# forestagostinelli/DeepCubeA

Hardware: AMD Instinct MI355X
Metric: A* nodes expanded/sec on cube3, batch 20k (higher is better)
Workload: dtype u8 states / f64 cost keys / f32 heuristic

## Files before the change

deepcubea_amd/csrc/dca_engine.hip:

```cpp
#include <string.h>

#include <new>
#include <vector>

#include "dca_common.h"
#include "dca_tile.h"

namespace dca {

constexpr int NBIN = 4096;
constexpr int kBinsPerThread = NBIN / 1024;
constexpr int kLgNbin = 12;
constexpr int kSub = 2048;
constexpr int kScanBlocks = 256;
constexpr int kCollectBlocks = 512;
constexpr int kRankBlocks = 256;
constexpr uint32_t kTinyBin = 512;
constexpr int kSortCap = 8192;
constexpr int RT = 512;
constexpr int kRegEnt = 16;
constexpr uint32_t kLdsEnt = RT * kRegEnt;
constexpr int kStash = 2560;
constexpr int kSegs = NBIN + 1 + kSub;
constexpr uint32_t kGiantBin = 8192;
constexpr int kMaxLevels = 9;
constexpr unsigned long long kBarrierTimeout = 200000000ull;
constexpr unsigned long long kBarrierTimeoutFirst = 25000000ull;
constexpr uint32_t GBAR_BROKEN = 0x80000000u;
constexpr uint32_t NIL = 0xFFFFFFFFu;
constexpr uint32_t ID_MASK = 0x7FFFFFFFu, ID_SOLVED = 0x80000000u;
constexpr uint64_t EMPTY = ~0ull;
constexpr uint64_t DEAD = ~0ull;
constexpr uint32_t GINF = 0xFFFFFFFFu;
constexpr int kMaxMoves = 4096;

struct Slot {
    uint64_t entry;
    uint32_t g;
    uint32_t head;
};

struct alignas(128) Cnt {
    uint32_t v;
    uint32_t pad[31];
};
struct alignas(128) GRange {
    uint64_t kmin, kmax;
    uint32_t imin, imax;
    uint32_t pad[26];
};
struct alignas(128) Rng {
    uint64_t kmin, kmax;
    uint64_t pad[14];
};
struct IterState {
    uint32_t pool_n;
    uint32_t npop, m, base;
    uint32_t best_id;
    int32_t has_best;
    float best_cost;
};
struct Ctl {
    int32_t done, failed, stop_after, pad0;
    int64_t iters, gen, expanded;
    IterState S[2];
    uint32_t cur_f;
    uint32_t hbin;
    uint32_t front_above;
    uint32_t cur_b;
    uint64_t T;
    uint32_t refill, compact, r_bstar, spill_bin, r_move;
    uint64_t r_kmin;
    uint32_t r_shift;
    uint32_t want, bstar, shift, n_big, n_ord;
    uint32_t giant;
    uint32_t tseg;
    uint32_t pre_b, cn_star;
    uint64_t sel_kmin;
    uint32_t goal_id;
    uint32_t dbg_nord, dbg_maxbin, dbg_giant, dbg_giant_seen, dbg_maxsub;
    Cnt open_n[4];
    Cnt closed_n, back_dead, front_dead, ret_n, ticket_a;
    Cnt gbar;
    GRange grange;
    Rng rng[4];
    alignas(128) unsigned long long goal_best;
    alignas(128) uint32_t first_solved;
};

__device__ __forceinline__ uint64_t key_of_cost(double c) {
    uint64_t b = (uint64_t)__double_as_longlong(c);
    return (b & 0x8000000000000000ull) ? ~b : (b | 0x8000000000000000ull);
}
__device__ __forceinline__ double cost_of_key(uint64_t k) {
    uint64_t b = (k & 0x8000000000000000ull) ? (k & 0x7FFFFFFFFFFFFFFFull) : ~k;
    return __longlong_as_double((long long)b);
}
__device__ __forceinline__ uint32_t select_shift(uint64_t kmin, uint64_t kmax) {
    uint64_t range = kmax - kmin;
    int bits = range ? 64 - __clzll((long long)range) : 0;
    return bits > kLgNbin ? (uint32_t)(bits - kLgNbin) : 0u;
}
__device__ __forceinline__ uint32_t bin_of(uint64_t k, uint64_t kmin, uint32_t shift) {
    if (k <= kmin) return 0u;
    const uint64_t f = (k - kmin) >> shift;
    return f < (uint64_t)NBIN ? (uint32_t)f : (uint32_t)(NBIN - 1);
}
__device__ __forceinline__ bool pair_less(uint64_t ka, uint32_t ia, uint64_t kb, uint32_t ib) {
    return ka < kb || (ka == kb && (ia & ID_MASK) < (ib & ID_MASK));
}

enum {
    P_REFILL_HIST = 0, P_REFILL_SCAN, P_REFILL_MOVE, P_SEL_HIST, P_SEL_SCAN, P_SEL_COLLECT, P_RANK, P_EXPAND,
    P_PROBE,
    P_DECIDE, P_PACK, P_COMMIT, P_RANK_SMALL, P_RANK_BIG, P_RB_LOAD, P_RB_COUNT, P_RB_SCATTER, P_RB_ORDER, P_COUNT
};
constexpr int kProfSlots = 1024;
__device__ int g_back_squeeze_mark;
__device__ int g_first_barrier_gives_up;
__device__ __forceinline__ uint32_t rank_shares(uint32_t cn) {
    return cn <= (uint32_t)(512 * 16) ? (cn + 1023u) / 1024u : 1u;
}

struct Eng {
    int env, dim, D, A, B, sem, oh_dtype, depth;
    double w;
    float wf;
    uint32_t max_nodes, M, tab_cap, tab_mask;
    uint32_t front_cap;
    uint8_t* state;
    int32_t* g;
    uint32_t* parent;
    uint8_t* move;
    uint8_t* solved;
    Slot* tab;
    uint32_t* closed_slots;
    uint64_t* open_key[4];
    uint32_t* open_id[4];
    uint32_t f_keep, f_max;
    uint32_t *hist, *pre, *fill;
    uint32_t* rhist;
    uint32_t* subhist;
    int coop;
    uint32_t* coop_off;
    uint64_t* part;
    uint64_t* tmp_key;
    uint32_t* tmp_id;
    uint16_t* tmp_f;
    uint32_t* tmp_idx;
    uint64_t* ord_key;
    uint32_t* ord_id;
    uint32_t* big_list;
    uint64_t* pop_key;
    uint32_t *pop_id, *pop_g;
    uint32_t *child_slot, *child_next, *child_v0;
    uint8_t *child_flags, *child_multi;
    float* child_h;
    uint8_t* nnet_in;
    uint8_t* onehot;
    uint8_t* root_nnet;
    int32_t* d_moves;
    Ctl* ctl;
    unsigned long long* prof;
    uint32_t* kept_pos;
    uint32_t* pk_n;
    uint32_t* pk_src;
    uint8_t* pk_nnet;
    uint8_t* pk_onehot;
    const float* pk_h;
    uint32_t pk_stride, inst;
    int pk_dtype;
};

__device__ __forceinline__ const IterState& st_cur(const Ctl* c) { return c->S[c->iters & 1]; }
__device__ __forceinline__ const IterState& st_next(const Ctl* c) { return c->S[(c->iters + 1) & 1]; }

__device__ __forceinline__ void fresh_binning(const Ctl* c, uint32_t buf, uint64_t& kmin, uint32_t& shift) {
    kmin = c->rng[buf].kmin;
    uint64_t kmax = c->rng[buf].kmax;
    const uint64_t T = c->T;
    if (T != ~0ull && T > kmax) kmax = T;
    shift = kmax > kmin ? select_shift(kmin, kmax) : 0u;
}

struct Stamp {
    unsigned long long* p;
    unsigned long long t0;
    __device__ __forceinline__ Stamp(const Eng& E, int kid) : p(nullptr), t0(0) {
        if (E.prof != nullptr && threadIdx.x == 0) {
            p = E.prof + ((size_t)kid * kProfSlots + (blockIdx.x & (kProfSlots - 1))) * 2;
            t0 = wall_clock64();
        }
    }
    __device__ __forceinline__ ~Stamp() {
        if (p) {
            atomicMin(p, t0);
            atomicMax(p + 1, (unsigned long long)wall_clock64());
        }
    }
};

__device__ __forceinline__ void prof_begin(const Eng& E, int kid) {
    if (E.prof != nullptr && threadIdx.x == 0)
        atomicMin(E.prof + ((size_t)kid * kProfSlots + (blockIdx.x & (kProfSlots - 1))) * 2, (unsigned long long)wall_clock64());
}
__device__ __forceinline__ void prof_end(const Eng& E, int kid) {
    if (E.prof != nullptr && threadIdx.x == 0)
        atomicMax(E.prof + ((size_t)kid * kProfSlots + (blockIdx.x & (kProfSlots - 1))) * 2 + 1, (unsigned long long)wall_clock64());
}

__device__ __forceinline__ void open_append(const Eng& E, Ctl* c, uint32_t buf, bool pred, uint64_t key, uint32_t id) {
    unsigned long long mask = __ballot(pred);
    if (mask == 0) return;
    int lane = threadIdx.x & 63;
    int leader = __ffsll((long long)mask) - 1;
    uint32_t cnt = (uint32_t)__popcll(mask);
    uint32_t basep = 0;
    uint64_t kmn = pred ? key : ~0ull, kmx = pred ? key : 0ull;
    for (int o = 32; o > 0; o >>= 1) {
        uint64_t a = __shfl_xor(kmn, o), b = __shfl_xor(kmx, o);
        kmn = a < kmn ? a : kmn;
        kmx = b > kmx ? b : kmx;
    }
    if (lane == leader) {
        basep = atomicAdd(&c->open_n[buf].v, cnt);
        atomicMin((unsigned long long*)&c->rng[buf].kmin, (unsigned long long)kmn);
        atomicMax((unsigned long long*)&c->rng[buf].kmax, (unsigned long long)kmx);
    }
    basep = __shfl(basep, leader);
    if (pred) {
        uint32_t pos = basep + (uint32_t)__popcll(mask & ((1ull << lane) - 1ull));
        if (pos < (buf < 2 ? E.front_cap : E.max_nodes)) {
            E.open_key[buf][pos] = key;
            E.open_id[buf][pos] = id;
        } else {
            c->failed = 1;
        }
    }
}

struct Pos2 {
    uint32_t a, b;
};
template <int NT>
__device__ __forceinline__ Pos2 block_reserve2(uint32_t cntA, uint32_t cntB, uint32_t* ctrA, uint32_t* ctrB,
                                               uint32_t* sh) {
    constexpr int NW = NT / 64;
    const int lane = threadIdx.x & 63, wv = threadIdx.x >> 6;
    uint32_t ia = cntA, ib = cntB;
    for (int o = 1; o < 64; o <<= 1) {
        uint32_t va = __shfl_up(ia, o), vb = __shfl_up(ib, o);
        if (lane >= o) {
            ia += va;
            ib += vb;
        }
    }
    if (lane == 63) {
        sh[wv] = ia;
        sh[NW + wv] = ib;
    }
    __syncthreads();
    if (threadIdx.x == 0) {
        uint32_t aa = 0, ab = 0;
        for (int w = 0; w < NW; w++) {
            uint32_t ta = sh[w], tb = sh[NW + w];
            sh[w] = aa;
            sh[NW + w] = ab;
            aa += ta;
            ab += tb;
        }
        sh[2 * NW] = aa ? atomicAdd(ctrA, aa) : 0u;
        sh[2 * NW + 1] = ab ? atomicAdd(ctrB, ab) : 0u;
    }
    __syncthreads();
    Pos2 p{sh[2 * NW] + sh[wv] + ia - cntA, sh[2 * NW + 1] + sh[NW + wv] + ib - cntB};
    __syncthreads();
    return p;
}

struct Pos3 {
    uint32_t a, b, c;
};
template <int NT>
__device__ __forceinline__ Pos3 block_reserve3(uint32_t cntA, uint32_t cntB, uint32_t cntC, uint32_t* ctrA,
                                               uint32_t* ctrB, uint32_t* ctrC, uint32_t* sh ) {
    constexpr int NW = NT / 64;
    const int lane = threadIdx.x & 63, wv = threadIdx.x >> 6;
    uint32_t ia = cntA, ib = cntB, ic = cntC;
    for (int o = 1; o < 64; o <<= 1) {
        uint32_t va = __shfl_up(ia, o), vb = __shfl_up(ib, o), vc = __shfl_up(ic, o);
        if (lane >= o) {
            ia += va;
            ib += vb;
            ic += vc;
        }
    }
    if (lane == 63) {
        sh[wv] = ia;
        sh[NW + wv] = ib;
        sh[2 * NW + wv] = ic;
    }
    __syncthreads();
    if (threadIdx.x == 0) {
        uint32_t aa = 0, ab = 0, ac = 0;
        for (int w = 0; w < NW; w++) {
            uint32_t ta = sh[w], tb = sh[NW + w], tc = sh[2 * NW + w];
            sh[w] = aa;
            sh[NW + w] = ab;
            sh[2 * NW + w] = ac;
            aa += ta;
            ab += tb;
            ac += tc;
        }
        sh[3 * NW] = aa ? atomicAdd(ctrA, aa) : 0u;
        sh[3 * NW + 1] = ab ? atomicAdd(ctrB, ab) : 0u;
        sh[3 * NW + 2] = ac ? atomicAdd(ctrC, ac) : 0u;
    }
    __syncthreads();
    Pos3 p{sh[3 * NW] + sh[wv] + ia - cntA, sh[3 * NW + 1] + sh[NW + wv] + ib - cntB,
           sh[3 * NW + 2] + sh[2 * NW + wv] + ic - cntC};
    __syncthreads();
    return p;
}

template <int NT, int K>
__device__ __forceinline__ void block_reserveK(const uint32_t (&cnt)[K], uint32_t* const (&ctr)[K], uint32_t (&pos)[K],
                                               uint32_t* sh ) {
    constexpr int NW = NT / 64;
    const int lane = threadIdx.x & 63, wv = threadIdx.x >> 6;
    uint32_t inc[K];
#pragma unroll
    for (int k = 0; k < K; k++) inc[k] = cnt[k];
    for (int o = 1; o < 64; o <<= 1) {
#pragma unroll
        for (int k = 0; k < K; k++) {
            uint32_t v = __shfl_up(inc[k], o);
            if (lane >= o) inc[k] += v;
        }
    }
    if (lane == 63) {
#pragma unroll
        for (int k = 0; k < K; k++) sh[k * NW + wv] = inc[k];
    }
    __syncthreads();
    if (threadIdx.x < K) {
        const int k = threadIdx.x;
        uint32_t acc = 0;
        for (int w = 0; w < NW; w++) {
            uint32_t tv = sh[k * NW + w];
            sh[k * NW + w] = acc;
            acc += tv;
        }
        sh[K * NW + k] = acc ? atomicAdd(ctr[k], acc) : 0u;
    }
    __syncthreads();
#pragma unroll
    for (int k = 0; k < K; k++) pos[k] = sh[K * NW + k] + sh[k * NW + wv] + inc[k] - cnt[k];
    __syncthreads();
}

__device__ __forceinline__ void fold_range(Ctl* c, uint32_t buf, uint64_t kmn, uint64_t kmx) {
    for (int o = 32; o > 0; o >>= 1) {
        uint64_t a = __shfl_xor(kmn, o), b = __shfl_xor(kmx, o);
        kmn = a < kmn ? a : kmn;
        kmx = b > kmx ? b : kmx;
    }
    if ((threadIdx.x & 63) == 0) {
        if (kmn < c->rng[buf].kmin) atomicMin((unsigned long long*)&c->rng[buf].kmin, (unsigned long long)kmn);
        if (kmx > c->rng[buf].kmax) atomicMax((unsigned long long*)&c->rng[buf].kmax, (unsigned long long)kmx);
    }
}

__device__ __forceinline__ bool clear_by_list(const Ctl* c, uint32_t cap, int force) {
    return !force && (uint64_t)c->closed_n.v * 8ull < (uint64_t)cap;
}
__global__ void k_init_table(Slot* tab, uint32_t cap, const Ctl* c, int force) {
    if (clear_by_list(c, cap, force)) return;
    uint32_t i = blockIdx.x * blockDim.x + threadIdx.x;
    uint32_t stride = gridDim.x * blockDim.x;
    for (; i < cap; i += stride) {
        tab[i].entry = EMPTY;
        tab[i].g = GINF;
        tab[i].head = 0;
    }
}
__global__ void k_clear_table_list(Slot* tab, uint32_t cap, const uint32_t* __restrict__ slots, const Ctl* c, int force) {
    if (!clear_by_list(c, cap, force)) return;
    const uint32_t n = c->closed_n.v;
    for (uint32_t i = blockIdx.x * blockDim.x + threadIdx.x; i < n; i += gridDim.x * blockDim.x) {
        const uint32_t sl = slots[i];
        if (sl < cap) {
            tab[sl].entry = EMPTY;
            tab[sl].g = GINF;
            tab[sl].head = 0;
        }
    }
}

__global__ void k_reset(Eng E) {
    if (threadIdx.x != 0 || blockIdx.x != 0) return;
    Ctl* c = E.ctl;
    memset(c, 0, sizeof(Ctl));
    const uint8_t* s = E.state;
    uint64_t h = hash_init(E.D);
    bool ok = true;
    for (int k = 0; k < E.D; k += 8) {
        uint64_t w = 0;
        for (int j = 0; j < 8 && k + j < E.D; j++) {
            uint32_t b = s[k + j];
            uint32_t goal = goal_byte(E.env, E.D, k + j);
            ok &= (b == goal);
            w |= (uint64_t)b << (8 * j);
            E.root_nnet[k + j] = (uint8_t)(E.env == DCA_ENV_CUBE3 ? (b * 57u) >> 9 : b);
        }
        h = hash_word(h, w);
    }
    h = hash_final(h);
    E.g[0] = 0;
    E.parent[0] = NIL;
    E.move[0] = 0xFF;
    E.solved[0] = ok ? 1 : 0;
    for (int p = 0; p < 2; p++) c->S[p].pool_n = 1;
    c->cur_f = 0;
    c->goal_best = ~0ull;
    c->first_solved = NIL;
    for (int b = 0; b < 4; b++) {
        c->rng[b].kmin = ~0ull;
        c->rng[b].kmax = 0;
    }
    c->cur_b = 2;
    c->T = ~0ull;
    if (E.sem == DCA_SEM_CPP) {
        uint32_t slot = (uint32_t)h & E.tab_mask;
        E.tab[slot].entry = ((h >> 32) << 32) | 0u;
        E.tab[slot].g = 0;
        E.closed_slots[0] = slot;
        c->closed_n.v = 1;
        c->gen = 1;
        uint64_t key = key_of_cost(0.0);
        E.open_key[0][0] = key;
        E.open_id[0][0] = ok ? ID_SOLVED : 0u;
        c->open_n[0].v = 1;
        c->rng[0].kmin = c->rng[0].kmax = key;
    }
}

__global__ void k_root_commit(Eng E, const float* h_root) {
    if (threadIdx.x != 0 || blockIdx.x != 0) return;
    Ctl* c = E.ctl;
    if (E.sem != DCA_SEM_PY || c->open_n[c->cur_f].v != 0) return;
    double hv = fmax((double)h_root[0], 0.0);
    double cost = __dadd_rn(__dmul_rn(E.w, 0.0), __dmul_rn(hv, E.solved[0] ? 0.0 : 1.0));
    uint64_t key = key_of_cost(cost);
    uint32_t b = c->cur_f;
    E.open_key[b][0] = key;
    E.open_id[b][0] = E.solved[0] ? ID_SOLVED : 0u;
    c->open_n[b].v = 1;
    c->rng[b].kmin = c->rng[b].kmax = key;
}

constexpr int kRefillPeriod = 16;
__device__ __forceinline__ uint32_t front_keep(const Eng& E) {
    const uint32_t floor_ = (uint32_t)(kRefillPeriod + 1) * (uint32_t)E.B;
    return E.f_keep > floor_ ? E.f_keep : floor_;
}
__device__ __forceinline__ bool need_refill(const Eng& E, const Ctl* c) {
    return c->open_n[c->cur_b].v != c->back_dead.v &&
           c->open_n[c->cur_f].v - c->front_dead.v - c->front_above < (uint32_t)(kRefillPeriod + 1) * (uint32_t)E.B;
}

__global__ __launch_bounds__(256) void k_refill_hist(const Eng* __restrict__ engs) {
    const Eng& E = engs[blockIdx.y];
    Ctl* c = E.ctl;
    if (c->done || !need_refill(E, c)) return;
    Stamp stamp(E, P_REFILL_HIST);
    __shared__ uint32_t lh[NBIN];
    for (int i = threadIdx.x; i < NBIN; i += 256) lh[i] = 0;
    __syncthreads();
    const uint32_t b = c->cur_b, n = c->open_n[b].v;
    const uint64_t kmin = c->rng[b].kmin;
    const uint32_t shift = select_shift(kmin, c->rng[b].kmax);
    const uint64_t* __restrict__ keys = E.open_key[b];
    for (uint32_t i = blockIdx.x * 256 + threadIdx.x; i < n; i += gridDim.x * 256) {
        uint64_t k = keys[i];
        if (k == DEAD) continue;
        uint64_t f = (k - kmin) >> shift;
        atomicAdd(&lh[f < NBIN ? (uint32_t)f : NBIN - 1], 1u);
    }
    __syncthreads();
    for (int i = threadIdx.x; i < NBIN; i += 256)
        if (lh[i]) atomicAdd(&E.rhist[i], lh[i]);
}

__device__ __forceinline__ void scan_vals(const uint32_t (&v)[kBinsPerThread], uint32_t* pre, uint32_t* wsum) {
    const int t = threadIdx.x, lane = t & 63, wv = t >> 6;
    uint32_t s = 0;
#pragma unroll
    for (int k = 0; k < kBinsPerThread; k++) s += v[k];
    uint32_t incl = s;
    for (int o = 1; o < 64; o <<= 1) {
        uint32_t u = __shfl_up(incl, o);
        if (lane >= o) incl += u;
    }
    if (lane == 63) wsum[wv] = incl;
    __syncthreads();
    if (t < 16) {
        uint32_t u = wsum[t], acc = u;
        for (int o = 1; o < 16; o <<= 1) {
            uint32_t x = __shfl_up(acc, o, 16);
            if (t >= o) acc += x;
        }
        wsum[t] = acc - u;
    }
    __syncthreads();
    uint32_t run = incl - s + wsum[wv];
#pragma unroll
    for (int k = 0; k < kBinsPerThread; k++) {
        pre[kBinsPerThread * t + k] = run;
        run += v[k];
    }
    if (t == 1023) pre[NBIN] = run;
    __syncthreads();
}

__device__ __forceinline__ void scan_bins(uint32_t* __restrict__ hist, bool zero, uint32_t* pre, uint32_t* wsum) {
    const int t = threadIdx.x, lane = t & 63, wv = t >> 6;
    uint32_t v[kBinsPerThread], s = 0;
#pragma unroll
    for (int k = 0; k < kBinsPerThread; k++) {
        v[k] = hist[kBinsPerThread * t + k];
        if (zero) hist[kBinsPerThread * t + k] = 0;
        s += v[k];
    }
    uint32_t incl = s;
    for (int o = 1; o < 64; o <<= 1) {
        uint32_t u = __shfl_up(incl, o);
        if (lane >= o) incl += u;
    }
    if (lane == 63) wsum[wv] = incl;
    __syncthreads();
    if (t < 16) {
        uint32_t u = wsum[t], acc = u;
        for (int o = 1; o < 16; o <<= 1) {
            uint32_t x = __shfl_up(acc, o, 16);
            if (t >= o) acc += x;
        }
        wsum[t] = acc - u;
    }
    __syncthreads();
    uint32_t run = incl - s + wsum[wv];
#pragma unroll
    for (int k = 0; k < kBinsPerThread; k++) {
        pre[kBinsPerThread * t + k] = run;
        run += v[k];
    }
    if (t == 1023) pre[NBIN] = run;
    __syncthreads();
}

__global__ __launch_bounds__(1024) void k_refill_scan(const Eng* __restrict__ engs) {
    const Eng& E = engs[blockIdx.y];
    Ctl* c = E.ctl;
    if (c->done) return;
    Stamp stamp(E, P_REFILL_SCAN);
    for (int k = 0; k < kBinsPerThread; k++) E.hist[kBinsPerThread * threadIdx.x + k] = 0;
    if (threadIdx.x == 0) c->open_n[c->cur_f ^ 1].v = 0;
    if (!need_refill(E, c)) {
        if (threadIdx.x == 0) {
            const uint32_t b = c->cur_b, phys = c->open_n[b].v, dead = c->back_dead.v;
            const uint32_t mark = g_back_squeeze_mark > 0 ? (uint32_t)(((uint64_t)E.max_nodes * (uint32_t)g_back_squeeze_mark) >> 10)
                                                          : (E.max_nodes / 8) * 7;
            const bool squeeze = dead != 0 && phys > mark;
            c->refill = squeeze ? 1u : 0u;
            c->compact = squeeze ? 1u : 0u;
            c->r_move = 0;
            if (squeeze) {
                c->open_n[b ^ 1].v = 0;
                c->rng[b ^ 1].kmin = c->rng[b].kmin;
                c->rng[b ^ 1].kmax = c->rng[b].kmax;
            }
        }
        return;
    }
    __shared__ uint32_t pre[NBIN + 1];
    __shared__ uint32_t wsum[16];
    scan_bins(E.rhist, true, pre, wsum);
    const int t = threadIdx.x;
    const uint32_t b = c->cur_b, n = c->open_n[b].v - c->back_dead.v;
    const uint32_t target = n < front_keep(E) ? n : front_keep(E);
    for (int k = 0; k < kBinsPerThread; k++) {
        int bin = kBinsPerThread * t + k;
        if (pre[bin] < target && target <= pre[bin + 1]) c->r_bstar = (uint32_t)bin;
    }
    __syncthreads();
    if (t == 0) {
        const uint64_t kmin = c->rng[b].kmin;
        const uint32_t shift = select_shift(kmin, c->rng[b].kmax);
        c->refill = 1;
        c->r_move = 1;
        c->r_kmin = kmin;
        c->r_shift = shift;
        uint64_t top = (c->r_bstar >= NBIN - 1) ? ~0ull : kmin + (((uint64_t)c->r_bstar + 1) << shift) - 1;
        if (top < kmin) top = ~0ull;
        c->T = top;
        if (top != ~0ull) c->rng[b].kmin = top + 1;
        const uint32_t phys = c->open_n[b].v, dead = c->back_dead.v;
        c->compact = ((dead > phys / 2 && phys > 4096) || (dead != 0 && phys > (E.max_nodes / 8) * 7)) ? 1u : 0u;
        if (c->compact) {
            c->open_n[b ^ 1].v = 0;
            c->rng[b ^ 1].kmin = c->rng[b].kmin;
            c->rng[b ^ 1].kmax = c->rng[b].kmax;
        }
    }
}

__global__ __launch_bounds__(256) void k_refill_move(const Eng* __restrict__ engs) {
    const Eng& E = engs[blockIdx.y];
    Ctl* c = E.ctl;
    if (c->done || !c->refill) return;
    Stamp stamp(E, P_REFILL_MOVE);
    __shared__ uint32_t sh[2 * 4 + 2];
    const uint32_t sb = c->cur_b, fb = c->cur_f, db = sb ^ 1;
    const bool compact = c->compact != 0;
    const uint32_t n = c->open_n[sb].v;
    const uint64_t kmin = c->r_kmin;
    const uint32_t shift = c->r_shift, bstar = c->r_bstar;
    const bool move = c->r_move != 0;
    uint64_t* __restrict__ keys = E.open_key[sb];
    const uint32_t* __restrict__ ids = E.open_id[sb];
    constexpr uint32_t ITEMS = 8, TILE = 256 * ITEMS;
    uint64_t fmn = ~0ull, fmx = 0;
    uint32_t moved = 0;
    const uint32_t ntiles = (n + TILE - 1) / TILE;
    for (uint32_t tile = blockIdx.x; tile < ntiles; tile += gridDim.x) {
        uint64_t k[ITEMS];
        uint32_t tof = 0, stay = 0, cf = 0, cs = 0;
#pragma unroll
        for (uint32_t i = 0; i < ITEMS; i++) {
            uint32_t idx = tile * TILE + i * 256 + threadIdx.x;
            k[i] = keys[idx < n ? idx : n - 1];
            if (idx >= n) k[i] = DEAD;
            uint64_t f = (k[i] - kmin) >> shift;
            bool alive = k[i] != DEAD;
            bool front = alive && move && (f < NBIN ? (uint32_t)f : NBIN - 1) <= bstar;
            tof |= (front ? 1u : 0u) << i;
            stay |= ((alive && !front && compact) ? 1u : 0u) << i;
            cf += front ? 1u : 0u;
            cs += (alive && !front && compact) ? 1u : 0u;
        }
        Pos2 p = block_reserve2<256>(cf, cs, &c->open_n[fb].v, &c->open_n[db].v, sh);
#pragma unroll
        for (uint32_t i = 0; i < ITEMS; i++) {
            uint32_t idx = tile * TILE + i * 256 + threadIdx.x;
            if ((tof >> i) & 1u) {
                if (p.a < E.front_cap) {
                    E.open_key[fb][p.a] = k[i];
                    E.open_id[fb][p.a] = ids[idx];
                }
                if (!compact) keys[idx] = DEAD;
                p.a++;
                moved++;
                fmn = k[i] < fmn ? k[i] : fmn;
                fmx = k[i] > fmx ? k[i] : fmx;
            } else if ((stay >> i) & 1u) {
                E.open_key[db][p.b] = k[i];
                E.open_id[db][p.b] = ids[idx];
                p.b++;
            }
        }
    }
    fold_range(c, fb, fmn, fmx);
    if (!compact) {
        for (int o = 32; o > 0; o >>= 1) moved += __shfl_xor(moved, o);
        if ((threadIdx.x & 63) == 0 && moved) atomicAdd(&c->back_dead.v, moved);
    }
}

__global__ __launch_bounds__(256) void k_front_rebase(const Eng* __restrict__ engs) {
    const Eng& E = engs[blockIdx.y];
    Ctl* c = E.ctl;
    if (c->done) return;
    Stamp stamp(E, P_SEL_HIST);
    __shared__ uint32_t lh[NBIN];
    __shared__ uint32_t sh[2 * 4 + 2];
    for (int i = threadIdx.x; i < NBIN; i += 256) lh[i] = 0;
    __syncthreads();
    const uint32_t b = c->cur_f, nb = b ^ 1, n = c->open_n[b].v;
    const uint32_t bb = (c->refill && c->compact) ? c->cur_b ^ 1u : c->cur_b;
    const uint64_t T = c->T;
    uint64_t kmin;
    uint32_t shift;
    fresh_binning(c, b, kmin, shift);
    const uint64_t* __restrict__ keys = E.open_key[b];
    const uint32_t* __restrict__ ids = E.open_id[b];
    constexpr uint32_t ITEMS = 8, TILE = 256 * ITEMS;
    uint64_t fmn = ~0ull, fmx = 0, bmn = ~0ull, bmx = 0;
    const uint32_t ntiles = (n + TILE - 1) / TILE;
    for (uint32_t tile = blockIdx.x; tile < ntiles; tile += gridDim.x) {
        uint64_t k[ITEMS];
        uint32_t id[ITEMS];
        uint32_t cl = 0, ce = 0;
#pragma unroll
        for (uint32_t i = 0; i < ITEMS; i++) {
            const uint32_t idx = tile * TILE + i * 256 + threadIdx.x, ic = idx < n ? idx : n - 1;
            k[i] = keys[ic];
            id[i] = ids[ic];
            if (idx >= n) k[i] = DEAD;
            cl += (k[i] != DEAD && k[i] <= T) ? 1u : 0u;
            ce += (k[i] != DEAD && k[i] > T) ? 1u : 0u;
        }
        Pos2 p = block_reserve2<256>(cl, ce, &c->open_n[nb].v, &c->open_n[bb].v, sh);
#pragma unroll
        for (uint32_t i = 0; i < ITEMS; i++) {
            if (k[i] != DEAD && k[i] > T) {
                if (p.b < E.max_nodes) {
                    E.open_key[bb][p.b] = k[i];
                    E.open_id[bb][p.b] = id[i];
                } else {
                    c->failed = 1;
                }
                p.b++;
                bmn = k[i] < bmn ? k[i] : bmn;
                bmx = k[i] > bmx ? k[i] : bmx;
                continue;
            }
            const bool lv = k[i] != DEAD;
            if (lv) atomicAdd(&lh[bin_of(k[i], kmin, shift)], 1u);
            if (!lv) continue;
            if (p.a < E.front_cap) {
                E.open_key[nb][p.a] = k[i];
                E.open_id[nb][p.a] = id[i];
            } else {
                c->failed = 1;
            }
            p.a++;
            fmn = k[i] < fmn ? k[i] : fmn;
            fmx = k[i] > fmx ? k[i] : fmx;
        }
    }
    __syncthreads();
    for (int i = threadIdx.x; i < NBIN; i += 256)
        if (lh[i]) atomicAdd(&E.hist[i], lh[i]);
    if (T != ~0ull) fold_range(c, bb, bmn, bmx);
    {
        __shared__ uint64_t red[2][4];
        const int lane = threadIdx.x & 63, wv = threadIdx.x >> 6;
        for (int o = 32; o > 0; o >>= 1) {
            const uint64_t a = __shfl_xor(fmn, o), z = __shfl_xor(fmx, o);
            fmn = a < fmn ? a : fmn;
            fmx = z > fmx ? z : fmx;
        }
        if (lane == 0) {
            red[0][wv] = fmn;
            red[1][wv] = fmx;
        }
        __syncthreads();
        if (threadIdx.x == 0) {
            uint64_t mn = red[0][0], mx = red[1][0];
            for (int w = 1; w < 4; w++) {
                mn = red[0][w] < mn ? red[0][w] : mn;
                mx = red[1][w] > mx ? red[1][w] : mx;
            }
            E.part[blockIdx.x] = mn;
            E.part[kCollectBlocks + blockIdx.x] = mx;
        }
    }
}

__global__ __launch_bounds__(1024) void k_sel_scan(const Eng* __restrict__ engs, int rebased) {
    const Eng& E = engs[blockIdx.y];
    Ctl* c = E.ctl;
    __shared__ uint32_t pre[NBIN + 1];
    __shared__ uint32_t wsum[16];
    __shared__ uint32_t s_spill, s_bstar, s_maxbin, s_giant, s_nbig, s_sp, s_hbin;
    __shared__ uint64_t s_red[2][16];
    const int t = threadIdx.x;
    const uint32_t done = c->done;
    const uint32_t cur0 = c->cur_f, old_shift = c->shift, refill = c->refill, compact = c->compact;
    const uint64_t old_kmin = c->sel_kmin, T0 = c->T;
    const uint32_t on0 = c->open_n[0].v, on1 = c->open_n[1].v, dead0 = c->front_dead.v, above0 = c->front_above;
    const uint64_t r0min = c->rng[0].kmin, r0max = c->rng[0].kmax, r1min = c->rng[1].kmin, r1max = c->rng[1].kmax;
    const uint32_t giant_seen = c->dbg_giant_seen;
    uint32_t hv[kBinsPerThread];
#pragma unroll
    for (int k = 0; k < kBinsPerThread; k++) hv[k] = E.hist[kBinsPerThread * t + k];
    uint64_t mn = ~0ull, mx = 0;
    if (rebased && t < kCollectBlocks) {
        mn = E.part[t];
        mx = E.part[kCollectBlocks + t];
    }
    if (done) return;
    Stamp stamp(E, P_SEL_SCAN);
    uint32_t cb = cur0;
    uint64_t new_kmin = old_kmin;
    uint32_t new_shift = old_shift;
    if (rebased) {
        new_kmin = cur0 ? r1min : r0min;
        uint64_t kmax = cur0 ? r1max : r0max;
        if (T0 != ~0ull && T0 > kmax) kmax = T0;
        new_shift = kmax > new_kmin ? select_shift(new_kmin, kmax) : 0u;
        for (int o = 32; o > 0; o >>= 1) {
            const uint64_t a = __shfl_xor(mn, o), z = __shfl_xor(mx, o);
            mn = a < mn ? a : mn;
            mx = z > mx ? z : mx;
        }
        if ((t & 63) == 0) {
            s_red[0][t >> 6] = mn;
            s_red[1][t >> 6] = mx;
        }
        cb ^= 1;
    }
    if (t == 0) {
        s_maxbin = 0;
        s_giant = 0;
        s_nbig = 0;
        s_spill = NBIN;
        s_bstar = 0;
        s_hbin = NBIN;
    }
    scan_vals(hv, pre, wsum);
    const uint32_t n = rebased ? (cb ? on1 : on0) : (cb ? on1 : on0) - dead0 - above0;
    const uint32_t want = n < (uint32_t)E.B ? n : (uint32_t)E.B;
    const uint32_t hwant = (uint32_t)(kRefillPeriod + 2) * (uint32_t)E.B;
    for (int k = 0; k < kBinsPerThread; k++) {
        int bin = kBinsPerThread * t + k;
        if (pre[bin] < want && want <= pre[bin + 1]) s_bstar = (uint32_t)bin;
        if (rebased && n > E.f_max) {
            const uint32_t keepn = want + front_keep(E);
            if (pre[bin] < keepn && keepn <= pre[bin + 1]) s_spill = (uint32_t)bin;
        }
        if (rebased && pre[bin] < hwant && hwant <= pre[bin + 1]) s_hbin = (uint32_t)bin + 1u;
        E.pre[bin] = pre[bin];
        E.fill[bin] = 0;
    }
    for (int i = NBIN + t; i < kSegs; i += 1024) E.fill[i] = 0;
    if (t == 1023) E.pre[NBIN] = pre[NBIN];
    __syncthreads();
    const bool giant = E.coop && !*E.coop_off && want != 0 && pre[s_bstar + 1] - pre[s_bstar] > kGiantBin;
    if (giant)
        for (int i = t; i < kMaxLevels * kSub; i += 1024) E.subhist[i] = 0;
    for (int k = 0; k < kBinsPerThread; k++) {
        const uint32_t bin = kBinsPerThread * t + k;
        if (bin <= s_bstar && want != 0) {
            const uint32_t cn = pre[bin + 1] - pre[bin];
            if (cn > 256) atomicMax(&s_maxbin, cn);
            if (cn > (uint32_t)kSortCap) atomicAdd(&s_giant, 1u);
            if (cn > kTinyBin && !(giant && bin == s_bstar)) {
                uint32_t G = rank_shares(cn);
                G = G > 8u ? 8u : G;
                const uint32_t at = atomicAdd(&s_nbig, G);
                for (uint32_t g = 0; g < G; g++) E.big_list[at + g] = bin | (g << 16) | (G << 20);
            }
        }
    }
    __syncthreads();
    if (t == 0) {
        if (rebased) {
            uint64_t fmn = ~0ull, fmx = 0;
            for (int w = 0; w < 16; w++) {
                fmn = s_red[0][w] < fmn ? s_red[0][w] : fmn;
                fmx = s_red[1][w] > fmx ? s_red[1][w] : fmx;
            }
            c->cur_f = cb;
            c->rng[cb].kmin = fmn;
            c->rng[cb].kmax = fmx;
            c->hbin = s_hbin;
        }
        if (refill) {
            if (compact) {
                c->cur_b ^= 1;
                c->back_dead.v = 0;
                c->compact = 0;
            }
            c->refill = 0;
        }
        c->want = want;
        c->bstar = s_bstar;
        c->tseg = s_bstar;
        c->pre_b = pre[s_bstar];
        c->cn_star = pre[s_bstar + 1] - pre[s_bstar];
        c->giant = giant ? 1u : 0u;
        c->gbar.v = 0;
        c->grange.kmin = ~0ull;
        c->grange.kmax = 0;
        c->grange.imin = ~0u;
        c->grange.imax = 0;
        c->sel_kmin = new_kmin;
        c->shift = new_shift;
        uint32_t sp = s_spill;
        if (sp < NBIN - 1) {
            const uint64_t top = new_kmin + (((uint64_t)sp + 1) << new_shift) - 1;
            if (top >= new_kmin && top < T0) c->T = top;  else sp = NBIN;
        } else {
            sp = NBIN;
        }
        if (rebased) c->front_above = sp < NBIN ? pre[NBIN] - pre[sp + 1] : 0u;
        c->spill_bin = sp;
        s_sp = sp;
        c->goal_best = ~0ull;
        c->first_solved = NIL;
        if (want == 0) {
            c->failed = 1;
            c->done = 1;
        }
        c->n_big = s_nbig;
        c->n_ord = want ? pre[s_bstar + 1] : 0;
        c->ret_n.v = 0;
        c->dbg_maxsub = 0;
        c->front_dead.v = (rebased ? 0u : dead0) + want;
        c->dbg_nord = want ? pre[s_bstar + 1] : 0;
        c->dbg_maxbin = s_maxbin;
        c->dbg_giant = s_giant;
        c->dbg_giant_seen = giant_seen + s_giant;
    }
    __syncthreads();
    {
        const uint32_t bstar = s_bstar, sp = s_sp;
        for (int k = 0; k < kBinsPerThread; k++) {
            const uint32_t bin = kBinsPerThread * t + k;
            if (want == 0) break;
            if (bin < bstar || bin > sp)
                E.hist[bin] = 0;
            else if (bin == bstar)
                E.hist[bin] = pre[bin + 1] - want;
        }
    }
}

typedef unsigned __int128 u128;
__device__ __forceinline__ u128 comp_of(uint64_t key, uint32_t id) { return ((u128)key << 32) | (u128)(id & ID_MASK); }
__device__ __forceinline__ int clz128(u128 v) {
    uint64_t hi = (uint64_t)(v >> 64), lo = (uint64_t)v;
    return hi ? __clzll((long long)hi) : 64 + (lo ? __clzll((long long)lo) : 64);
}

constexpr int kStashG = 1536;
struct CollectLds {
    uint32_t pre[NBIN + 4];
    uint32_t lcnt[NBIN];
    union {
        struct {
            uint64_t st_key[kStash];
            uint32_t st_idx[kStash];
            uint16_t st_f[kStash];
            uint16_t nzf[kStash];
        } n;
        struct {
            uint32_t lcnt_ext[kSegs - NBIN + 3];
            uint32_t subpre[kSub + 4];
            uint64_t st_key[kStashG];
            uint32_t st_idx[kStashG];
            uint16_t st_f[kStashG];
            uint16_t nzf[kStashG];
        } g;
    } u;
    uint64_t red64[2][4];
    uint32_t red32[2][4];
    uint32_t wsum[4];
    uint32_t st_n, nz_n, ok, tsub, nb, bstar;
};
static_assert(sizeof(CollectLds) <= 80 * 1024, "two workgroups of k_sel_collect must fit one CU's LDS");
static_assert(offsetof(CollectLds, u) == offsetof(CollectLds, lcnt) + sizeof(uint32_t) * NBIN, "lcnt must run on into lcnt_ext");
static_assert(sizeof(uint64_t) * kStashG >= sizeof(uint32_t) * kSub, "sub-bin counters alias the giant stash");

struct SelParams {
    uint32_t b, n;
    uint64_t kmin;
    uint32_t shift;
    uint32_t want, bstar, pre_b, cn_star;
    bool giant;
};

enum { BAR_FAIL = 0, BAR_PASS = 1, BAR_BROKEN = 2 };
__device__ __forceinline__ int collect_grid_barrier(const Eng& E, Ctl* c, CollectLds& L, uint32_t target, bool first) {
    asm volatile("s_waitcnt vmcnt(0)" ::: "memory");
    __syncthreads();
    if (threadIdx.x == 0) {
        __builtin_amdgcn_fence(__ATOMIC_RELEASE, "agent");
        asm volatile("s_waitcnt vmcnt(0)" ::: "memory");
        uint32_t v = __hip_atomic_fetch_add(&c->gbar.v, 1u, __ATOMIC_RELAXED, __HIP_MEMORY_SCOPE_AGENT) + 1u;
        int res = BAR_PASS;
        const unsigned long long t0 = wall_clock64();
        const unsigned long long limit = first ? (g_first_barrier_gives_up ? 0ull : kBarrierTimeoutFirst) : kBarrierTimeout;
        for (;;) {
            if (v & GBAR_BROKEN) {
                res = first ? BAR_BROKEN : BAR_FAIL;
                break;
            }
            if (v >= target) break;
            __builtin_amdgcn_s_sleep(4);
            if (__hip_atomic_load(&c->failed, __ATOMIC_RELAXED, __HIP_MEMORY_SCOPE_AGENT) != 0) {
                res = BAR_FAIL;
                break;
            }
            if (wall_clock64() - t0 > limit) {
                if (!first) {
                    res = BAR_FAIL;
                    break;
                }
                uint32_t expect = v;
                if (__hip_atomic_compare_exchange_strong(&c->gbar.v, &expect, v | GBAR_BROKEN, __ATOMIC_RELAXED, __ATOMIC_RELAXED,
                                                         __HIP_MEMORY_SCOPE_AGENT)) {
                    res = BAR_BROKEN;
                    break;
                }
                v = expect;
                continue;
            }
            v = __hip_atomic_load(&c->gbar.v, __ATOMIC_RELAXED, __HIP_MEMORY_SCOPE_AGENT);
        }
        __builtin_amdgcn_fence(__ATOMIC_ACQUIRE, "agent");
        if (res == BAR_FAIL) {
            __hip_atomic_store(&c->failed, 1, __ATOMIC_RELAXED, __HIP_MEMORY_SCOPE_AGENT);
            __hip_atomic_store(&c->done, 1, __ATOMIC_RELAXED, __HIP_MEMORY_SCOPE_AGENT);
        } else if (res == BAR_BROKEN) {
            __hip_atomic_store(E.coop_off, 1u, __ATOMIC_RELAXED, __HIP_MEMORY_SCOPE_AGENT);
        }
        L.ok = (uint32_t)res;
    }
    __syncthreads();
    return (int)L.ok;
}

__device__ __noinline__ int collect_giant(const Eng& E, Ctl* c, CollectLds& L, const SelParams P) {
    const uint32_t t = threadIdx.x, lane = t & 63, wv = t >> 6;
    const uint32_t n = P.n;
    const uint64_t bkmin = P.kmin;
    const uint32_t shift = P.shift, bstar = P.bstar, want = P.want;
    const uint32_t pre_b = P.pre_b;
    uint64_t* __restrict__ keys = E.open_key[P.b];
    const uint32_t* __restrict__ ids = E.open_id[P.b];
    constexpr uint32_t ITEMS = 8, TILE = 256 * ITEMS;
    const uint32_t ntiles = (n + TILE - 1) / TILE;
    uint32_t phase = 0;
    {
        uint64_t kmn = ~0ull, kmx = 0;
        uint32_t imn = ~0u, imx = 0;
        for (uint32_t tile = blockIdx.x; tile < ntiles; tile += gridDim.x) {
            uint64_t k[ITEMS];
            uint32_t id[ITEMS];
#pragma unroll
            for (uint32_t i = 0; i < ITEMS; i++) {
                const uint32_t idx = tile * TILE + i * 256 + t, ic = idx < n ? idx : n - 1;
                k[i] = keys[ic];
                id[i] = ids[ic] & ID_MASK;
                if (idx >= n) k[i] = DEAD;
            }
#pragma unroll
            for (uint32_t i = 0; i < ITEMS; i++) {
                const bool in = k[i] != DEAD && bin_of(k[i], bkmin, shift) == bstar;
                kmn = in && k[i] < kmn ? k[i] : kmn;
                kmx = in && k[i] > kmx ? k[i] : kmx;
                imn = in && id[i] < imn ? id[i] : imn;
                imx = in && id[i] > imx ? id[i] : imx;
            }
        }
        for (int o = 32; o > 0; o >>= 1) {
            const uint64_t a = __shfl_xor(kmn, o), z = __shfl_xor(kmx, o);
            const uint32_t x = __shfl_xor(imn, o), y = __shfl_xor(imx, o);
            kmn = a < kmn ? a : kmn;
            kmx = z > kmx ? z : kmx;
            imn = x < imn ? x : imn;
            imx = y > imx ? y : imx;
        }
        if (lane == 0) {
            L.red64[0][wv] = kmn;
            L.red64[1][wv] = kmx;
            L.red32[0][wv] = imn;
            L.red32[1][wv] = imx;
        }
        __syncthreads();
        if (t == 0) {
            for (int w = 1; w < 4; w++) {
                kmn = L.red64[0][w] < kmn ? L.red64[0][w] : kmn;
                kmx = L.red64[1][w] > kmx ? L.red64[1][w] : kmx;
                imn = L.red32[0][w] < imn ? L.red32[0][w] : imn;
                imx = L.red32[1][w] > imx ? L.red32[1][w] : imx;
            }
            if (kmn <= kmx) {
                atomicMin((unsigned long long*)&c->grange.kmin, (unsigned long long)kmn);
                atomicMax((unsigned long long*)&c->grange.kmax, (unsigned long long)kmx);
                atomicMin(&c->grange.imin, imn);
                atomicMax(&c->grange.imax, imx);
            }
        }
    }
    if (const int r = collect_grid_barrier(E, c, L, ++phase * gridDim.x, true); r != BAR_PASS) return r;
    const uint64_t gkmin = __hip_atomic_load(&c->grange.kmin, __ATOMIC_RELAXED, __HIP_MEMORY_SCOPE_AGENT);
    const uint64_t gkmax = __hip_atomic_load(&c->grange.kmax, __ATOMIC_RELAXED, __HIP_MEMORY_SCOPE_AGENT);
    const uint32_t gimin = __hip_atomic_load(&c->grange.imin, __ATOMIC_RELAXED, __HIP_MEMORY_SCOPE_AGENT);
    const uint32_t gimax = __hip_atomic_load(&c->grange.imax, __ATOMIC_RELAXED, __HIP_MEMORY_SCOPE_AGENT);
    u128 V0 = ((u128)gkmin << 32) + (u128)gimin;
    u128 span = ((u128)(gkmax - gkmin) << 32) + (u128)(gimax - gimin);
    uint32_t need = want - pre_b, below = 0, shc = 0, tsub = 0;
    uint32_t* lh = reinterpret_cast<uint32_t*>(L.u.g.st_key);
    uint32_t* subpre = L.u.g.subpre;
    for (int lvl = 0;; lvl++) {
        const uint32_t bits = span ? (uint32_t)(128 - clz128(span)) : 0u;
        shc = bits > 11u ? bits - 11u : 0u;
        for (uint32_t i = t; i < (uint32_t)kSub; i += 256) lh[i] = 0;
        __syncthreads();
        for (uint32_t tile = blockIdx.x; tile < ntiles; tile += gridDim.x) {
            uint64_t k[ITEMS];
            uint32_t id[ITEMS];
#pragma unroll
            for (uint32_t i = 0; i < ITEMS; i++) {
                const uint32_t idx = tile * TILE + i * 256 + t, ic = idx < n ? idx : n - 1;
                k[i] = keys[ic];
                id[i] = ids[ic];
                if (idx >= n) k[i] = DEAD;
            }
#pragma unroll
            for (uint32_t i = 0; i < ITEMS; i++) {
                if (k[i] == DEAD || bin_of(k[i], bkmin, shift) != bstar) continue;
                const u128 v = comp_of(k[i], id[i]);
                if (v < V0 || v - V0 > span) continue;
                atomicAdd(&lh[(uint32_t)((v - V0) >> shc)], 1u);
            }
        }
        __syncthreads();
        uint32_t* gh = E.subhist + (size_t)lvl * kSub;
        for (uint32_t i = t; i < (uint32_t)kSub; i += 256)
            if (lh[i]) atomicAdd(&gh[i], lh[i]);
        if (collect_grid_barrier(E, c, L, ++phase * gridDim.x, false) != BAR_PASS) return BAR_FAIL;
        constexpr int PER = kSub / 256;
        uint32_t v[PER], sum = 0;
#pragma unroll
        for (int k = 0; k < PER; k++) {
            v[k] = __hip_atomic_load(&gh[PER * t + k], __ATOMIC_RELAXED, __HIP_MEMORY_SCOPE_AGENT);
            sum += v[k];
        }
        uint32_t incl = sum;
        for (int o = 1; o < 64; o <<= 1) {
            const uint32_t u = __shfl_up(incl, o);
            if (lane >= (uint32_t)o) incl += u;
        }
        if (lane == 63) L.wsum[wv] = incl;
        if (t == 0) L.tsub = ~0u;
        __syncthreads();
        uint32_t run = incl - sum;
        for (uint32_t w = 0; w < wv; w++) run += L.wsum[w];
#pragma unroll
        for (int k = 0; k < PER; k++) {
            subpre[PER * t + k] = run;
            if (run < need && need <= run + v[k]) L.tsub = PER * t + k;
            run += v[k];
        }
        if (t == 255) subpre[kSub] = run;
        __syncthreads();
        tsub = L.tsub;
        if (tsub == ~0u) {
            if (t == 0) c->failed = 1, c->done = 1;
            return BAR_FAIL;
        }
        const uint32_t cn = subpre[tsub + 1] - subpre[tsub];
        if (cn <= kGiantBin || shc == 0 || lvl + 1 >= kMaxLevels) break;
        below += subpre[tsub];
        need -= subpre[tsub];
        V0 += (u128)tsub << shc;
        span = ((u128)1 << shc) - 1;
        __syncthreads();
    }
    const uint32_t seg0 = bstar + 1u;
    if (blockIdx.x == 0) {
        if (t == 0) {
            L.nb = c->n_big;
            E.pre[bstar + 1] = pre_b + below;
            c->tseg = seg0 + tsub;
            c->n_ord = pre_b + below + subpre[tsub + 1];
            c->dbg_nord = pre_b + below + subpre[tsub + 1];
        }
        __syncthreads();
        for (uint32_t sg = t; sg <= tsub + 1u; sg += 256) {
            const uint32_t cn = sg == 0 ? below : subpre[sg] - subpre[sg - 1];
            if (sg > 0) E.pre[seg0 + sg] = pre_b + below + subpre[sg];
            if (cn > kTinyBin) {
                uint32_t G = rank_shares(cn);
                G = G > 8u ? 8u : G;
                const uint32_t at = atomicAdd(&L.nb, G);
                for (uint32_t g = 0; g < G; g++) E.big_list[at + g] = (bstar + sg) | (g << 16) | (G << 20);
            }
        }
        __syncthreads();
        if (t == 0) c->n_big = L.nb;
    }
    uint32_t* lcnt = L.lcnt;
    for (uint32_t i = t; i < (uint32_t)(kSegs + 3); i += 256) lcnt[i] = 0;
    if (t == 0) {
        L.st_n = 0;
        L.nz_n = 0;
    }
    __syncthreads();
    uint64_t* st_key = L.u.g.st_key;
    uint32_t* st_idx = L.u.g.st_idx;
    uint16_t *st_f = L.u.g.st_f, *nzf = L.u.g.nzf;
    auto seg_base = [&](uint32_t f) -> uint32_t {
        return f < bstar ? L.pre[f] : f == bstar ? pre_b : pre_b + below + subpre[f - seg0];
    };
    auto seg_end = [&](uint32_t f) -> uint32_t {
        return f < bstar ? L.pre[f + 1] : f == bstar ? pre_b + below : pre_b + below + subpre[f - seg0 + 1];
    };
    auto flush = [&]() {
        const uint32_t ns = L.st_n < (uint32_t)kStashG ? L.st_n : (uint32_t)kStashG;
        const uint32_t nz = L.nz_n;
        for (uint32_t i = t; i < nz; i += 256) {
            const uint32_t f = nzf[i];
            lcnt[f] = atomicAdd(&E.fill[f], lcnt[f]);
        }
        __syncthreads();
        for (uint32_t p = t; p < ns; p += 256) {
            const uint32_t f = st_f[p];
            const uint32_t id = ids[st_idx[p]];
            const uint32_t pos = seg_base(f) + atomicAdd(&lcnt[f], 1u);
            if (pos < seg_end(f)) {
                E.tmp_key[pos] = st_key[p];
                E.tmp_id[pos] = id;
                E.tmp_f[pos] = (uint16_t)f;
                E.tmp_idx[pos] = st_idx[p];
            } else {
                c->failed = 1;
            }
        }
        __syncthreads();
        for (uint32_t i = t; i < nz; i += 256) lcnt[nzf[i]] = 0;
        __syncthreads();
        if (t == 0) {
            L.st_n = 0;
            L.nz_n = 0;
        }
        __syncthreads();
    };
    constexpr uint32_t ITEMS_D = 4, TILE_D = 256 * ITEMS_D;
    const uint32_t ntiles_d = (n + TILE_D - 1) / TILE_D;
    for (uint32_t tile2 = blockIdx.x; tile2 < ntiles; tile2 += gridDim.x) {
        for (uint32_t half = 0; half < 2; half++) {
            const uint32_t tile = tile2 * 2 + half;
            if (tile < ntiles_d) {
                uint64_t k[ITEMS_D];
                uint32_t id[ITEMS_D];
#pragma unroll
                for (uint32_t i = 0; i < ITEMS_D; i++) {
                    const uint32_t idx = tile * TILE_D + i * 256 + t, ic = idx < n ? idx : n - 1;
                    k[i] = keys[ic];
                    id[i] = ids[ic];
                    if (idx >= n) k[i] = DEAD;
                }
#pragma unroll
                for (uint32_t i = 0; i < ITEMS_D; i++) {
                    if (k[i] == DEAD) continue;
                    uint32_t f = bin_of(k[i], bkmin, shift);
                    if (f > bstar) continue;
                    if (f == bstar) {
                        const u128 v = comp_of(k[i], id[i]);
                        if (v >= V0) {
                            if (v - V0 > span) continue;
                            const uint32_t sub = (uint32_t)((v - V0) >> shc);
                            if (sub > tsub) continue;
                            f = seg0 + sub;
                        }
                    }
                    const uint32_t idx = tile * TILE_D + i * 256 + t;
                    const uint32_t p = atomicAdd(&L.st_n, 1u);
                    keys[idx] = DEAD;
                    if (p < (uint32_t)kStashG) {
                        st_key[p] = k[i];
                        st_idx[p] = idx;
                        st_f[p] = (uint16_t)f;
                        if (atomicAdd(&lcnt[f], 1u) == 0u) nzf[atomicAdd(&L.nz_n, 1u)] = (uint16_t)f;
                    } else {
                        const uint32_t pos = seg_base(f) + atomicAdd(&E.fill[f], 1u);
                        if (pos < seg_end(f)) {
                            E.tmp_key[pos] = k[i];
                            E.tmp_id[pos] = id[i];
                            E.tmp_f[pos] = (uint16_t)f;
                            E.tmp_idx[pos] = idx;
                        } else {
                            c->failed = 1;
                        }
                    }
                }
            }
            __syncthreads();
            if (L.st_n + TILE_D > (uint32_t)kStashG) flush();
        }
    }
    __syncthreads();
    flush();
    return BAR_PASS;
}

template <bool FUSED>
__global__ __launch_bounds__(256) void k_sel_collect(const Eng* __restrict__ engs) {
    const Eng& E = engs[blockIdx.y];
    Ctl* c = E.ctl;
    if (c->done) return;
    Stamp stamp(E, P_SEL_COLLECT);
    extern __shared__ __attribute__((aligned(16))) uint8_t collect_lds[];
    CollectLds& L = *reinterpret_cast<CollectLds*>(collect_lds);
    const uint32_t t = threadIdx.x;
    SelParams P;
    {
        const uint32_t b = c->cur_f, on0 = c->open_n[0].v, on1 = c->open_n[1].v;
        P.b = b;
        P.n = b ? on1 : on0;
        P.kmin = c->sel_kmin;
        P.shift = c->shift;
        P.want = c->want;
    }
    if constexpr (FUSED) {
        constexpr int PER = NBIN / 256;
        const uint32_t lane = t & 63, wv = t >> 6;
        uint32_t v[PER], sum = 0;
        {
            const uint4* h4 = reinterpret_cast<const uint4*>(E.hist + PER * t);
#pragma unroll
            for (int q = 0; q < PER / 4; q++) {
                const uint4 x = h4[q];
                v[4 * q] = x.x;
                v[4 * q + 1] = x.y;
                v[4 * q + 2] = x.z;
                v[4 * q + 3] = x.w;
            }
#pragma unroll
            for (int k = 0; k < PER; k++) sum += v[k];
        }
        uint32_t incl = sum;
        for (int o = 1; o < 64; o <<= 1) {
            const uint32_t u = __shfl_up(incl, o);
            if (lane >= (uint32_t)o) incl += u;
        }
        if (lane == 63) L.wsum[wv] = incl;
        if (t == 0) L.bstar = 0;
        __syncthreads();
        uint32_t run = incl - sum;
        for (uint32_t w = 0; w < wv; w++) run += L.wsum[w];
        const uint32_t want = P.want;
#pragma unroll
        for (int k = 0; k < PER; k++) {
            L.pre[PER * t + k] = run;
            if (run < want && want <= run + v[k]) L.bstar = PER * t + k;
            run += v[k];
        }
        if (t == 255) L.pre[NBIN] = run;
        __syncthreads();
        if (want == 0) {
            if (blockIdx.x == 0 && t == 0) {
                c->failed = 1;
                c->done = 1;
            }
            return;
        }
        P.bstar = L.bstar;
        P.pre_b = L.pre[P.bstar];
        P.cn_star = L.pre[P.bstar + 1] - P.pre_b;
        P.giant = E.coop && !*E.coop_off && P.cn_star > kGiantBin;
        if (blockIdx.x == 0) {
            for (uint32_t i = t; i <= (uint32_t)NBIN; i += 256) E.pre[i] = L.pre[i];
            if (t == 0) {
                L.nb = 0;
                L.st_n = 0;
                L.nz_n = 0;
            }
            __syncthreads();
            for (uint32_t bin = t; bin <= P.bstar; bin += 256) {
                const uint32_t cn = L.pre[bin + 1] - L.pre[bin];
                if (cn > 256) atomicMax(&L.st_n, cn);
                if (cn > (uint32_t)kSortCap) atomicAdd(&L.nz_n, 1u);
                if (cn > kTinyBin && !(P.giant && bin == P.bstar)) {
                    uint32_t G = rank_shares(cn);
                    G = G > 8u ? 8u : G;
                    const uint32_t at = atomicAdd(&L.nb, G);
                    for (uint32_t g = 0; g < G; g++) E.big_list[at + g] = bin | (g << 16) | (G << 20);
                }
            }
            __syncthreads();
            if (t == 0) {
                c->bstar = P.bstar;
                c->tseg = P.bstar;
                c->giant = P.giant ? 1u : 0u;
                c->pre_b = P.pre_b;
                c->cn_star = P.cn_star;
                c->spill_bin = NBIN;
                c->n_big = L.nb;
                c->n_ord = L.pre[P.bstar + 1];
                c->front_dead.v += want;
                c->dbg_nord = L.pre[P.bstar + 1];
                c->dbg_maxbin = L.st_n;
                c->dbg_giant = L.nz_n;
                c->dbg_giant_seen += L.nz_n;
                c->dbg_maxsub = 0;
            }
            __syncthreads();
        }
    } else {
        P.bstar = c->bstar;
        P.giant = c->giant != 0;
        P.pre_b = c->pre_b;
        P.cn_star = c->cn_star;
        if (P.want == 0) return;
        for (uint32_t i = t; i <= P.bstar + 1u; i += 256) L.pre[i] = E.pre[i];
        __syncthreads();
    }
    if (P.giant) {
        if (collect_giant(E, c, L, P) != BAR_BROKEN) return;
        if (blockIdx.x == 0 && t == 0) {
            const uint32_t cn = P.cn_star;
            uint32_t G = rank_shares(cn);
            G = G > 8u ? 8u : G;
            const uint32_t at = c->n_big;
            if (cn > kTinyBin) {
                for (uint32_t g = 0; g < G; g++) E.big_list[at + g] = P.bstar | (g << 16) | (G << 20);
                c->n_big = at + G;
            }
            c->giant = 0;
        }
        P.giant = false;
        __syncthreads();
    }
    const uint32_t n = P.n;
    const uint64_t kmin = P.kmin;
    const uint32_t shift = P.shift, bstar = P.bstar;
    uint64_t* __restrict__ keys = E.open_key[P.b];
    const uint32_t* __restrict__ ids = E.open_id[P.b];
    constexpr uint32_t ITEMS = 8, TILE = 256 * ITEMS;
    const uint32_t ntiles = (n + TILE - 1) / TILE;
    uint64_t* st_key = L.u.n.st_key;
    uint32_t* st_idx = L.u.n.st_idx;
    uint16_t *st_f = L.u.n.st_f, *nzf = L.u.n.nzf;
    for (int i = t; i < NBIN; i += 256) L.lcnt[i] = 0;
    if (t == 0) {
        L.st_n = 0;
        L.nz_n = 0;
    }
    __syncthreads();
    auto flush = [&]() {
        const uint32_t ns = L.st_n < (uint32_t)kStash ? L.st_n : (uint32_t)kStash;
        const uint32_t nz = L.nz_n;
        for (uint32_t i = t; i < nz; i += 256) {
            const uint32_t f = nzf[i];
            L.lcnt[f] = atomicAdd(&E.fill[f], L.lcnt[f]);
        }
        __syncthreads();
        for (uint32_t p = t; p < ns; p += 256) {
            const uint32_t f = st_f[p];
            const uint32_t id = ids[st_idx[p]];
            const uint32_t pos = L.pre[f] + atomicAdd(&L.lcnt[f], 1u);
            if (pos < L.pre[f + 1]) {
                E.tmp_key[pos] = st_key[p];
                E.tmp_id[pos] = id;
                E.tmp_f[pos] = (uint16_t)f;
                E.tmp_idx[pos] = st_idx[p];
            } else {
                c->failed = 1;
            }
        }
        __syncthreads();
        for (uint32_t i = t; i < nz; i += 256) L.lcnt[nzf[i]] = 0;
        __syncthreads();
        if (t == 0) {
            L.st_n = 0;
            L.nz_n = 0;
        }
        __syncthreads();
    };
    for (uint32_t tile = blockIdx.x; tile < ntiles; tile += gridDim.x) {
        uint64_t k[ITEMS];
        uint32_t dest = 0;
#pragma unroll
        for (uint32_t i = 0; i < ITEMS; i++) {
            const uint32_t idx = tile * TILE + i * 256 + t, ic = idx < n ? idx : n - 1;
            k[i] = keys[ic];
            if (idx >= n) k[i] = DEAD;
        }
#pragma unroll
        for (uint32_t i = 0; i < ITEMS; i++) {
            const uint32_t f = bin_of(k[i], kmin, shift);
            const uint32_t d = (k[i] != DEAD && f <= bstar) ? 1u : 0u;
            dest |= d << (2 * i);
        }
        if (dest & 0x5555u & ~(dest >> 1)) {
#pragma unroll
            for (uint32_t i = 0; i < ITEMS; i++) {
                if (((dest >> (2 * i)) & 3u) != 1u) continue;
                const uint32_t idx = tile * TILE + i * 256 + t;
                const uint32_t f = bin_of(k[i], kmin, shift);
                const uint32_t p = atomicAdd(&L.st_n, 1u);
                keys[idx] = DEAD;
                if (p < kStash) {
                    st_key[p] = k[i];
                    st_idx[p] = idx;
                    st_f[p] = (uint16_t)f;
                    if (atomicAdd(&L.lcnt[f], 1u) == 0u) nzf[atomicAdd(&L.nz_n, 1u)] = (uint16_t)f;
                } else {
                    const uint32_t pos = L.pre[f] + atomicAdd(&E.fill[f], 1u);
                    if (pos < L.pre[f + 1]) {
                        E.tmp_key[pos] = k[i];
                        E.tmp_id[pos] = ids[idx];
                        E.tmp_f[pos] = (uint16_t)f;
                        E.tmp_idx[pos] = idx;
                    } else {
                        c->failed = 1;
                    }
                }
            }
        }
        __syncthreads();
        if (L.st_n + TILE > (uint32_t)kStash) flush();
    }
    __syncthreads();
    flush();
}


constexpr int kRankStack = 512;
constexpr uint32_t kDirectMax = 512;
constexpr uint32_t kSubMax = 512;

struct RankItem {
    uint32_t off, n, need, src;
    uint32_t g, G;
    uint32_t nopush;
};
struct RankShared {
    uint32_t cnt[kSub + 64];
    uint32_t off[kSub + 1];
    uint32_t wsum[16];
    uint64_t red_lo[32], red_hi[32];
    uint64_t vmin_hi, vmin_lo;
    uint64_t kmin, kspan;
    uint32_t imin, ispan;
    uint32_t bits, tsub, sp, fail;
    uint32_t ret_base, ret_cnt;
    RankItem stack[kRankStack];
};

__device__ __forceinline__ void emit_pop(const Eng& E, Ctl* c, uint32_t rank, uint64_t key, uint32_t id) {
    E.pop_key[rank] = key;
    E.pop_id[rank] = id;
    if (id & ID_SOLVED) {
        if (E.sem == DCA_SEM_PY)
            atomicMin(&c->goal_best, ((unsigned long long)(uint32_t)E.g[id & ID_MASK] << 32) | rank);
        else
            atomicMin(&c->first_solved, rank);
    }
}
__device__ __forceinline__ void emit_ranked(const Eng& E, Ctl* c, uint32_t nf, bool live, uint32_t rank, uint32_t want,
                                            uint64_t key, uint32_t id) {
    if (live && rank < want) emit_pop(E, c, rank, key, id);
    const bool back = live && rank >= want;
    const unsigned long long mask = __ballot(back);
    if (mask == 0) return;
    const int lane = threadIdx.x & 63;
    const int leader = __ffsll((long long)mask) - 1;
    uint32_t basep = 0;
    if (lane == leader) basep = atomicAdd(&c->ret_n.v, (uint32_t)__popcll(mask));
    basep = __shfl(basep, leader);
    if (back) {
        const uint32_t slot = E.tmp_idx[basep + (uint32_t)__popcll(mask & ((1ull << lane) - 1ull))];
        E.open_key[nf][slot] = key;
        E.open_id[nf][slot] = id;
    }
}
__device__ __forceinline__ void ret_begin(Ctl* c, RankShared& S, uint32_t nf, uint32_t count) {
    __syncthreads();
    if (threadIdx.x == 0) {
        S.ret_base = count ? atomicAdd(&c->ret_n.v, count) : 0u;
        S.ret_cnt = 0;
    }
    __syncthreads();
}
struct RetAcc {};
__device__ __forceinline__ void ret_put(const Eng& E, Ctl* c, RankShared& S, uint32_t nf, bool pred, uint64_t key,
                                        uint32_t id, RetAcc& acc) {
    const unsigned long long mask = __ballot(pred);
    if (mask == 0) return;
    const int lane = threadIdx.x & 63;
    const int leader = __ffsll((long long)mask) - 1;
    uint32_t basep = 0;
    if (lane == leader) basep = atomicAdd(&S.ret_cnt, (uint32_t)__popcll(mask));
    basep = __shfl(basep, leader);
    if (pred) {
        const uint32_t slot = E.tmp_idx[S.ret_base + basep + (uint32_t)__popcll(mask & ((1ull << lane) - 1ull))];
        E.open_key[nf][slot] = key;
        E.open_id[nf][slot] = id;
    }
}
__device__ __forceinline__ void ret_end(Ctl* c, uint32_t nf, RetAcc acc) {}
template <int NJ>
__device__ __forceinline__ void ret_put_many(const Eng& E, RankShared& S, uint32_t nf, uint32_t n_ord, uint32_t preds,
                                             const uint64_t* key, const uint32_t* id) {
    const uint32_t cnt = (uint32_t)__popc(preds);
    const int lane = threadIdx.x & 63;
    uint32_t incl = cnt;
    for (int o = 1; o < 64; o <<= 1) {
        const uint32_t u = __shfl_up(incl, o);
        if (lane >= o) incl += u;
    }
    const uint32_t total = __shfl(incl, 63);
    if (total == 0) return;
    uint32_t basep = 0;
    if (lane == 63) basep = atomicAdd(&S.ret_cnt, total);
    basep = __shfl(basep, 63);
    uint32_t r = S.ret_base + basep + incl - cnt;
    uint32_t slot[NJ];
#pragma unroll
    for (int j = 0; j < NJ; j++) {
        slot[j] = E.tmp_idx[r < n_ord ? r : n_ord - 1];
        r += (preds >> j) & 1u;
    }
#pragma unroll
    for (int j = 0; j < NJ; j++)
        if ((preds >> j) & 1u) {
            E.open_key[nf][slot[j]] = key[j];
            E.open_id[nf][slot[j]] = id[j];
        }
}

__device__ __forceinline__ void rank_small_entries(const Eng& E, Ctl* c, RankShared& S, uint64_t* LK, uint32_t* LI,
                                                   uint32_t nf, uint32_t p0, uint32_t n_ord, uint32_t want) {
    const uint32_t t = threadIdx.x;
    const uint32_t plast = (p0 + RT - 1 < n_ord ? p0 + RT - 1 : n_ord - 1);
    const uint32_t f_lo = E.tmp_f[p0], f_hi = E.tmp_f[plast];
    const uint32_t lo = E.pre[f_lo], hi = E.pre[f_hi + 1];
    const bool staged = hi - lo <= kLdsEnt && f_hi - f_lo + 2 <= (uint32_t)kSub;
    if (staged) {
        for (uint32_t i = t; i < hi - lo; i += RT) {
            LK[i] = E.tmp_key[lo + i];
            LI[i] = E.tmp_id[lo + i];
        }
        for (uint32_t i = t; i < f_hi - f_lo + 2; i += RT) S.off[i] = E.pre[f_lo + i];
    }
    __syncthreads();
    const uint32_t p = p0 + t;
    bool live = p < n_ord;
    uint64_t k = 0;
    uint32_t id = 0, rank = 0;
    if (live) {
        const uint32_t f = E.tmp_f[p];
        const uint32_t o = staged ? S.off[f - f_lo] : E.pre[f], e = staged ? S.off[f - f_lo + 1] : E.pre[f + 1];
        if (e - o > kTinyBin) {
            live = false;
        } else if (staged) {
            k = LK[p - lo];
            id = LI[p - lo];
            rank = o;
            for (uint32_t j = o - lo; j < e - lo; j++) rank += pair_less(LK[j], LI[j], k, id) ? 1u : 0u;
        } else {
            k = E.tmp_key[p];
            id = E.tmp_id[p];
            rank = o;
            for (uint32_t j = o; j < e; j++) rank += pair_less(E.tmp_key[j], E.tmp_id[j], k, id) ? 1u : 0u;
        }
    }
    emit_ranked(E, c, nf, live, rank, want, k, id);
    __syncthreads();
}

__device__ __forceinline__ uint32_t sub_of(uint64_t k, uint32_t id, u128 vmin, uint32_t shc, uint32_t nsub) {
    const u128 q = (comp_of(k, id) - vmin) >> shc;
    return q < (u128)nsub ? (uint32_t)q : nsub - 1u;
}


__device__ __forceinline__ void rank_range(RankShared& S, u128 vmin, u128 vmax) {
    const uint32_t t = threadIdx.x, lane = t & 63, wv = t >> 6;
    for (int o = 32; o > 0; o >>= 1) {
        uint64_t ahi = __shfl_xor((uint64_t)(vmin >> 64), o), alo = __shfl_xor((uint64_t)vmin, o);
        uint64_t bhi = __shfl_xor((uint64_t)(vmax >> 64), o), blo = __shfl_xor((uint64_t)vmax, o);
        u128 a = ((u128)ahi << 64) | alo, b = ((u128)bhi << 64) | blo;
        vmin = a < vmin ? a : vmin;
        vmax = b > vmax ? b : vmax;
    }
    if (lane == 0) {
        S.red_hi[wv] = (uint64_t)(vmin >> 64);
        S.red_lo[wv] = (uint64_t)vmin;
        S.red_hi[16 + wv] = (uint64_t)(vmax >> 64);
        S.red_lo[16 + wv] = (uint64_t)vmax;
    }
    for (uint32_t i = t; i < (uint32_t)kSub; i += RT) S.cnt[i] = 0;
    __syncthreads();
    if (t == 0) {
        u128 mn = ~(u128)0, mx = 0;
        for (int k = 0; k < RT / 64; k++) {
            u128 a = ((u128)S.red_hi[k] << 64) | S.red_lo[k], b = ((u128)S.red_hi[16 + k] << 64) | S.red_lo[16 + k];
            mn = a < mn ? a : mn;
            mx = b > mx ? b : mx;
        }
        const u128 range = mx - mn;
        S.bits = range ? (uint32_t)(128 - clz128(range)) : 0u;
        S.vmin_hi = (uint64_t)(mn >> 64);
        S.vmin_lo = (uint64_t)mn;
    }
    __syncthreads();
}

__device__ __forceinline__ void rank_range64(RankShared& S, uint64_t kmn, uint64_t kmx, uint32_t imn, uint32_t imx) {
    const uint32_t t = threadIdx.x, lane = t & 63, wv = t >> 6;
    for (int o = 32; o > 0; o >>= 1) {
        const uint64_t a = __shfl_xor(kmn, o), b = __shfl_xor(kmx, o);
        const uint32_t x = __shfl_xor(imn, o), y = __shfl_xor(imx, o);
        kmn = a < kmn ? a : kmn;
        kmx = b > kmx ? b : kmx;
        imn = x < imn ? x : imn;
        imx = y > imx ? y : imx;
    }
    if (lane == 0) {
        S.red_lo[wv] = kmn;
        S.red_lo[16 + wv] = kmx;
        S.red_hi[wv] = imn;
        S.red_hi[16 + wv] = imx;
    }
    for (uint32_t i = t; i < (uint32_t)kSub; i += RT) S.cnt[i] = 0;
    __syncthreads();
    if (t == 0) {
        uint64_t a = ~0ull, b = 0, x = ~0ull, y = 0;
        for (int k = 0; k < RT / 64; k++) {
            a = S.red_lo[k] < a ? S.red_lo[k] : a;
            b = S.red_lo[16 + k] > b ? S.red_lo[16 + k] : b;
            x = S.red_hi[k] < x ? S.red_hi[k] : x;
            y = S.red_hi[16 + k] > y ? S.red_hi[16 + k] : y;
        }
        S.kmin = a;
        S.kspan = b - a;
        S.imin = (uint32_t)x;
        S.ispan = (uint32_t)(y - x);
    }
    __syncthreads();
}

__device__ __forceinline__ void rank_prefix(RankShared& S, uint32_t nsub, uint32_t need) {
    constexpr int PER = kSub / RT;
    const uint32_t t = threadIdx.x, lane = t & 63, wv = t >> 6;
    uint32_t v[PER], s4 = 0;
#pragma unroll
    for (int k = 0; k < PER; k++) {
        v[k] = PER * t + k < nsub ? S.cnt[PER * t + k] : 0u;
        s4 += v[k];
    }
    uint32_t incl = s4;
    for (int o = 1; o < 64; o <<= 1) {
        uint32_t u = __shfl_up(incl, o);
        if (lane >= (uint32_t)o) incl += u;
    }
    if (lane == 63) S.wsum[wv] = incl;
    __syncthreads();
    uint32_t run = incl - s4;
    for (uint32_t w = 0; w < wv; w++) run += S.wsum[w];
#pragma unroll
    for (int k = 0; k < PER; k++) {
        const uint32_t i = PER * t + k;
        if (i < nsub) {
            S.off[i] = run;
            S.cnt[i] = 0;
            if (run < need && need <= run + v[k]) S.tsub = i;
            if (i + 1 == nsub) S.off[nsub] = run + v[k];
        }
        run += v[k];
    }
    __syncthreads();
}

__device__ __forceinline__ void rank_push(RankShared& S, const RankItem& it, uint32_t tsub, uint32_t need, bool refinable,
                                          uint32_t lo = 0u, uint32_t hi = ~0u) {
    for (uint32_t sb = lo + threadIdx.x; sb <= tsub && sb < hi; sb += RT) {
        const uint32_t s0 = S.off[sb], e0 = S.off[sb + 1];
        if (e0 - s0 > kSubMax && refinable) {
            const uint32_t slot = atomicAdd(&S.sp, 1u);
            if (slot < (uint32_t)kRankStack)
                S.stack[slot] = RankItem{it.off + s0, e0 - s0, sb == tsub ? need - s0 : e0 - s0, it.src ^ 1u, 0u, 1u,
                                         (it.G > 1u || it.nopush) ? 1u : 0u};
            else
                S.fail = 1;
        }
    }
}

__device__ __noinline__ void rank_item(const Eng& E, Ctl* c, RankShared& S, uint64_t* LK, uint32_t* LI, uint32_t nf,
                                       uint32_t want, RankItem it) {
    const uint32_t t = threadIdx.x;
    const uint64_t* __restrict__ K = (it.src ? E.ord_key : E.tmp_key) + it.off;
    const uint32_t* __restrict__ I = (it.src ? E.ord_id : E.tmp_id) + it.off;
    uint64_t* __restrict__ K2 = (it.src ? E.tmp_key : E.ord_key) + it.off;
    uint32_t* __restrict__ I2 = (it.src ? E.tmp_id : E.ord_id) + it.off;
    const uint32_t n = it.n, need = it.need;
    if (n <= kDirectMax) {
        if (t < n) {
            LK[t] = K[t];
            LI[t] = I[t];
        }
        __syncthreads();
        ret_begin(c, S, nf, n - need);
        RetAcc acc{};
        const bool live = t < n;
        uint64_t k = 0;
        uint32_t id = 0, rank = 0;
        if (live) {
            k = LK[t];
            id = LI[t];
            for (uint32_t j = 0; j < n; j++) rank += pair_less(LK[j], LI[j], k, id) ? 1u : 0u;
            if (rank < need) emit_pop(E, c, it.off + rank, k, id);
        }
        ret_put(E, c, S, nf, live && rank >= need, k, id, acc);
        ret_end(c, nf, acc);
        __syncthreads();
        return;
    }
    uint32_t lg = 0;
    while ((8u << lg) <= n && lg < 11) lg++;
    if (lg < 11) lg++;
    if (n <= kLdsEnt) {
        uint64_t ek[kRegEnt];
        uint32_t ei[kRegEnt];
        prof_begin(E, P_RB_LOAD);
#pragma unroll
        for (int j = 0; j < kRegEnt; j++) {
            const uint32_t i = t + (uint32_t)RT * j, ic = i < n ? i : n - 1;
            ek[j] = K[ic];
            ei[j] = I[ic];
        }
        {
            uint64_t kmn = ~0ull, kmx = 0;
            uint32_t imn = ~0u, imx = 0;
#pragma unroll
            for (int j = 0; j < kRegEnt; j++) {
                const uint32_t im = ei[j] & ID_MASK;
                kmn = ek[j] < kmn ? ek[j] : kmn;
                kmx = ek[j] > kmx ? ek[j] : kmx;
                imn = im < imn ? im : imn;
                imx = im > imx ? im : imx;
            }
            rank_range64(S, kmn, kmx, imn, imx);
        }
        prof_end(E, P_RB_LOAD);
        prof_begin(E, P_RB_COUNT);
        const bool idmode = S.kspan == 0;
        const uint64_t kbase = S.kmin, span = idmode ? (uint64_t)S.ispan : S.kspan;
        const uint32_t ibase = S.imin;
        const uint32_t bits = span ? (uint32_t)(64 - __clzll((long long)span)) : 0u;
        if (lg > bits) lg = bits;
        const uint32_t nsub = 1u << lg, shc = bits - lg;
        const bool refinable = (shc > 0 || !idmode) && !it.nopush;
        const uint32_t lo_sub = (uint32_t)((uint64_t)nsub * it.g / it.G), hi_sub = (uint32_t)((uint64_t)nsub * (it.g + 1u) / it.G);
#pragma unroll
        for (int j = 0; j < kRegEnt; j++) {
            ek[j] = idmode ? (uint64_t)((ei[j] & ID_MASK) - ibase) : ek[j] - kbase;
            if (t + (uint32_t)RT * j < n) atomicAdd(&S.cnt[(uint32_t)(ek[j] >> shc)], 1u);
        }
        __syncthreads();
        rank_prefix(S, nsub, need);
        prof_end(E, P_RB_COUNT);
        prof_begin(E, P_RB_SCATTER);
        if (E.prof != nullptr) {
            uint32_t mx = 0;
            for (uint32_t sb = t; sb < nsub; sb += RT) mx = max(mx, S.off[sb + 1] - S.off[sb]);
            if (mx > 16) atomicMax(&c->dbg_maxsub, mx);
        }
        const uint32_t tsub = S.tsub;
        const bool tsub_pushed = S.off[tsub + 1] - S.off[tsub] > kSubMax && refinable;
        const uint32_t in_hi = hi_sub < tsub + 1u ? hi_sub : tsub + 1u;
        const uint32_t ret_lo = lo_sub > tsub + 1u ? lo_sub : tsub + 1u;
        ret_begin(c, S, nf, (ret_lo < hi_sub ? S.off[hi_sub] - S.off[ret_lo] : 0u) +
                                ((tsub >= lo_sub && tsub < hi_sub && !tsub_pushed) ? S.off[tsub + 1] - need : 0u));
        const uint32_t n_ord = c->n_ord;
        {
            uint32_t inm = 0, retm = 0, pos[kRegEnt];
#pragma unroll
            for (int j = 0; j < kRegEnt; j++) {
                const uint32_t sub = (uint32_t)(ek[j] >> shc);
                const bool live = t + (uint32_t)RT * j < n, in = live && sub >= lo_sub && sub < in_hi;
                inm |= (in ? 1u : 0u) << j;
                retm |= (live && sub >= ret_lo && sub < hi_sub ? 1u : 0u) << j;
                pos[j] = S.off[in ? sub : 0u] + atomicAdd(&S.cnt[in ? sub : (uint32_t)kSub + (t & 63u)], in ? 1u : 0u);
            }
#pragma unroll
            for (int j = 0; j < kRegEnt; j++) {
                if ((inm >> j) & 1u) {
                    LK[pos[j]] = ek[j];
                    LI[pos[j]] = ei[j];
                }
                ek[j] = idmode ? kbase : kbase + ek[j];
            }
            ret_put_many<kRegEnt>(E, S, nf, n_ord, retm, ek, ei);
        }
        __syncthreads();
        prof_end(E, P_RB_SCATTER);
        prof_begin(E, P_RB_ORDER);
        const uint32_t p_lo = S.off[lo_sub], p_hi = in_hi > lo_sub ? S.off[in_hi] : p_lo;
        constexpr int U = 4;
        for (uint32_t p0 = p_lo; p0 < p_hi; p0 += RT * U) {
            uint64_t o[U];
            uint32_t id[U], s0[U], cn[U], rank[U], livem = 0, bigm = 0, trip = 0;
#pragma unroll
            for (int u = 0; u < U; u++) {
                const uint32_t p = p0 + (uint32_t)u * RT + t;
                livem |= (p < p_hi ? 1u : 0u) << u;
                o[u] = LK[p < p_hi ? p : p_hi - 1];
                id[u] = LI[p < p_hi ? p : p_hi - 1];
            }
#pragma unroll
            for (int u = 0; u < U; u++) {
                const uint32_t sub = (uint32_t)(o[u] >> shc);
                s0[u] = S.off[sub];
                cn[u] = S.off[sub + 1] - s0[u];
                rank[u] = s0[u];
                if (!((livem >> u) & 1u)) cn[u] = 0;
                if (cn[u] > kSubMax && refinable) {
                    bigm |= 1u << u;
                    cn[u] = 0;
                }
                trip = cn[u] > trip ? cn[u] : trip;
            }
            for (uint32_t jj = 0; jj < trip; jj++) {
#pragma unroll
                for (int u = 0; u < U; u++) {
                    const uint32_t j = s0[u] + (jj < cn[u] ? jj : 0u);
                    const bool less = pair_less(LK[j], LI[j], o[u], id[u]);
                    rank[u] += (jj < cn[u] && less) ? 1u : 0u;
                }
            }
            uint32_t retm = 0;
#pragma unroll
            for (int u = 0; u < U; u++) {
                const uint32_t p = p0 + (uint32_t)u * RT + t;
                o[u] = idmode ? kbase : kbase + o[u];
                if ((bigm >> u) & 1u) {
                    K2[p] = o[u];
                    I2[p] = id[u];
                } else if ((livem >> u) & 1u) {
                    if (rank[u] < need) emit_pop(E, c, it.off + rank[u], o[u], id[u]);
                    else retm |= 1u << u;
                }
            }
            ret_put_many<U>(E, S, nf, n_ord, retm, o, id);
        }
        rank_push(S, it, tsub, need, refinable, lo_sub, in_hi);
        __syncthreads();
        prof_end(E, P_RB_ORDER);
        return;
    }
    {
        u128 vmin = ~(u128)0, vmax = 0;
        for (uint32_t b0 = 0; b0 < n; b0 += kLdsEnt) {
            uint64_t ek[kRegEnt];
            uint32_t ei[kRegEnt];
#pragma unroll
            for (int j = 0; j < kRegEnt; j++) {
                const uint32_t i = b0 + t + (uint32_t)RT * j, ic = i < n ? i : n - 1;
                ek[j] = K[ic];
                ei[j] = I[ic];
            }
#pragma unroll
            for (int j = 0; j < kRegEnt; j++)
                if (b0 + t + (uint32_t)RT * j < n) {
                    const u128 v = comp_of(ek[j], ei[j]);
                    vmin = v < vmin ? v : vmin;
                    vmax = v > vmax ? v : vmax;
                }
        }
        rank_range(S, vmin, vmax);
    }
    const u128 base = ((u128)S.vmin_hi << 64) | S.vmin_lo;
    const uint32_t bits = S.bits;
    if (lg > bits) lg = bits;
    const uint32_t nsub = 1u << lg, shc = bits - lg;
    for (uint32_t b0 = 0; b0 < n; b0 += kLdsEnt) {
        uint64_t ek[kRegEnt];
        uint32_t ei[kRegEnt];
#pragma unroll
        for (int j = 0; j < kRegEnt; j++) {
            const uint32_t i = b0 + t + (uint32_t)RT * j, ic = i < n ? i : n - 1;
            ek[j] = K[ic];
            ei[j] = I[ic];
        }
#pragma unroll
        for (int j = 0; j < kRegEnt; j++)
            if (b0 + t + (uint32_t)RT * j < n) atomicAdd(&S.cnt[sub_of(ek[j], ei[j], base, shc, nsub)], 1u);
    }
    __syncthreads();
    rank_prefix(S, nsub, need);
    const uint32_t tsub = S.tsub;
    const bool tsub_pushed = S.off[tsub + 1] - S.off[tsub] > kSubMax && shc > 0;
    ret_begin(c, S, nf, (n - S.off[tsub + 1]) + (tsub_pushed ? 0u : S.off[tsub + 1] - need));
    RetAcc acc{};
    const uint32_t n_ord_all = c->n_ord;
    for (uint32_t b0 = 0; b0 < n; b0 += kLdsEnt) {
        uint64_t ek[kRegEnt];
        uint32_t ei[kRegEnt];
#pragma unroll
        for (int j = 0; j < kRegEnt; j++) {
            const uint32_t i = b0 + t + (uint32_t)RT * j, ic = i < n ? i : n - 1;
            ek[j] = K[ic];
            ei[j] = I[ic];
        }
        uint32_t retm = 0;
#pragma unroll
        for (int j = 0; j < kRegEnt; j++) {
            const bool live = b0 + t + (uint32_t)RT * j < n;
            uint32_t sub = 0;
            if (live) {
                sub = sub_of(ek[j], ei[j], base, shc, nsub);
                if (sub <= tsub) {
                    const uint32_t p = S.off[sub] + atomicAdd(&S.cnt[sub], 1u);
                    K2[p] = ek[j];
                    I2[p] = ei[j];
                }
            }
            retm |= (live && sub > tsub ? 1u : 0u) << j;
        }
        ret_put_many<kRegEnt>(E, S, nf, n_ord_all, retm, ek, ei);
    }
    __syncthreads();
    const uint32_t m = S.off[tsub + 1];
    for (uint32_t p0 = 0; p0 < m; p0 += RT) {
        const uint32_t p = p0 + t;
        bool live = p < m;
        uint64_t k = 0;
        uint32_t id = 0, rank = 0;
        if (live) {
            k = K2[p];
            id = I2[p];
            const uint32_t sub = sub_of(k, id, base, shc, nsub);
            const uint32_t s0 = S.off[sub], e0 = S.off[sub + 1];
            if (e0 - s0 > kSubMax && shc > 0) {
                live = false;
            } else {
                rank = s0;
                for (uint32_t j = s0; j < e0; j++) rank += pair_less(K2[j], I2[j], k, id) ? 1u : 0u;
                if (rank < need) emit_pop(E, c, it.off + rank, k, id);
            }
        }
        ret_put(E, c, S, nf, live && rank >= need, k, id, acc);
    }
    rank_push(S, it, tsub, need, shc > 0);
    ret_end(c, nf, acc);
    __syncthreads();
}

__global__ __launch_bounds__(RT) void k_rank(const Eng* __restrict__ engs) {
    const Eng& E = engs[blockIdx.y];
    Ctl* c = E.ctl;
    if (c->done) return;
    Stamp stamp(E, P_RANK);
    __shared__ RankShared S;
    extern __shared__ __attribute__((aligned(16))) uint8_t rank_lds[];
    uint64_t* LK = reinterpret_cast<uint64_t*>(rank_lds);
    uint32_t* LI = reinterpret_cast<uint32_t*>(rank_lds + (size_t)kLdsEnt * 8);
    const uint32_t t = threadIdx.x;
    const uint32_t nf = c->cur_f;
    const uint32_t tseg = c->tseg, want = c->want;
    const uint32_t n_big = c->n_big, n_ord = c->n_ord;
    if (blockIdx.x == gridDim.x - 1) {
        const uint32_t bstar = c->bstar, pre_b = c->pre_b, cn_star = c->cn_star;
        if (want != 0) {
            for (uint32_t bin = t; bin < bstar; bin += RT) E.hist[bin] = 0;
            if (t == 0) E.hist[bstar] = cn_star - (want - pre_b);
        }
        for (uint32_t i = t; i < (uint32_t)kSegs; i += RT) E.fill[i] = 0;
        if (c->giant)
            for (uint32_t i = t; i < (uint32_t)(kMaxLevels * kSub); i += RT) E.subhist[i] = 0;
    }
    {
        Stamp sub(E, P_RANK_SMALL);
        for (uint32_t p0 = blockIdx.x * RT; p0 < n_ord; p0 += gridDim.x * RT)
            rank_small_entries(E, c, S, LK, LI, nf, p0, n_ord, want);
    }
    Stamp sub2(E, P_RANK_BIG);
    for (uint32_t bi = (blockIdx.x + gridDim.x - 64u) % gridDim.x; bi < n_big; bi += gridDim.x) {
        const uint32_t unit = E.big_list[bi];
        const uint32_t f = unit & 0xFFFFu;
        const uint32_t o = E.pre[f], n = E.pre[f + 1] - o;
        __syncthreads();
        if (t == 0) {
            S.stack[0] = RankItem{o, n, (f == tseg) ? want - o : n, 0u, (unit >> 16) & 15u, unit >> 20, 0u};
            S.sp = 1;
            S.fail = 0;
        }
        for (;;) {
            __syncthreads();
            const uint32_t sp = S.sp;
            if (sp == 0 || sp > (uint32_t)kRankStack) break;
            const RankItem it = S.stack[sp - 1];
            __syncthreads();
            if (t == 0) S.sp = sp - 1;
            __syncthreads();
            rank_item(E, c, S, LK, LI, nf, want, it);
        }
        if (t == 0 && (S.fail || S.sp != 0)) c->failed = 1;
    }
}

__device__ __forceinline__ void close_pop(const Eng& E, Ctl* c, const IterState& S0, uint32_t it, uint32_t want,
                                          uint32_t npop, uint32_t base, bool fail) {
    IterState N = S0;
    if (E.sem == DCA_SEM_PY) {
        const unsigned long long gb = c->goal_best;
        if (gb != ~0ull) {
            c->stop_after = 1;
            c->goal_id = E.pop_id[(uint32_t)(gb & 0xFFFFFFFFull)] & ID_MASK;
        }
    } else {
        const uint32_t fs = c->first_solved;
        if (fs != NIL) {
            const float cst = (float)cost_of_key(E.pop_key[fs]);
            if (E.B == 1) {
                N.best_id = E.pop_id[fs] & ID_MASK;
                N.best_cost = cst;
                N.has_best = 1;
                c->stop_after = 1;
            } else if (!S0.has_best || S0.best_cost > cst) {
                N.best_id = E.pop_id[fs] & ID_MASK;
                N.best_cost = cst;
                N.has_best = 1;
            }
        }
        if (S0.has_best && (float)cost_of_key(E.pop_key[0]) >= N.best_cost) c->stop_after = 1;
    }
    if (fail) {
        c->failed = 1;
        c->done = 1;
        c->front_dead.v -= want;
        return;
    }
    const uint32_t m = npop * (uint32_t)E.A;
    N.npop = npop;
    N.m = m;
    N.base = base;
    N.pool_n = base + m;
    c->S[(it + 1) & 1] = N;
    c->gen += (int64_t)m;
    c->expanded += npop;
}

constexpr uint8_t F_KEEP = 1, F_MIN = 2, F_NEW = 4;

template <int ENV, int DIM>
__device__ __forceinline__ uint32_t child_word_from_parent(uint32_t pw, uint32_t w, uint32_t a, const uint8_t* ltab) {
    using EV = EnvT<ENV, DIM>;
    const int gbase = (int)(threadIdx.x & 63u) & ~15;
    uint32_t out = 0;
    if constexpr (ENV == DCA_ENV_CUBE3) {
#pragma unroll
        for (uint32_t b = 0; b < 4; b++) {
            const uint32_t i = 4 * w + b;
            const uint32_t p = i < (uint32_t)EV::D ? ltab[a * EV::D + i] : 0u;
            const uint32_t v = (uint32_t)__shfl((int)pw, gbase + (int)(p >> 2));
            if (i < (uint32_t)EV::D) out |= ((v >> (8 * (p & 3))) & 0xFFu) << (8 * b);
        }
    } else if constexpr (ENV == DCA_ENV_LIGHTSOUT) {
#pragma unroll
        for (uint32_t b = 0; b < 4; b++) {
            const uint32_t i = 4 * w + b;
            if (i < (uint32_t)EV::D) {
                const uint32_t v = (pw >> (8 * b)) & 0xFFu;
                out |= (lightsout_flip(DIM, (int)a, (int)i) ? ((v + 1u) & 1u) : v) << (8 * b);
            }
        }
    } else {
        uint32_t z = 0xFFFFu;
#pragma unroll
        for (int b = 3; b >= 0; b--)
            if (4 * w + b < (uint32_t)EV::D && ((pw >> (8 * b)) & 0xFFu) == 0u) z = 4 * w + b;
        for (int o = 8; o > 0; o >>= 1) {
            const uint32_t y = (uint32_t)__shfl_xor((int)z, o);
            z = y < z ? y : z;
        }
        z = z < (uint32_t)EV::D ? z : 0u;
        const uint32_t sw = (uint32_t)npuzzle_swap(DIM, (int)z, (int)a);
#pragma unroll
        for (uint32_t b = 0; b < 4; b++) {
            const uint32_t i = 4 * w + b;
            const uint32_t src = i < (uint32_t)EV::D ? ((i == z) ? sw : i) : 0u;
            const uint32_t v = (uint32_t)__shfl((int)pw, gbase + (int)(src >> 2));
            if (i < (uint32_t)EV::D) out |= ((i == sw) ? 0u : ((v >> (8 * (src & 3))) & 0xFFu)) << (8 * b);
        }
    }
    return out;
}

constexpr int kEngTile = 16;
template <int ENV, int DIM, int OH>
__global__ __launch_bounds__(kThreads) void k_expand(const Eng* __restrict__ engs, int heur_id, int write_nn) {
    const Eng& E = engs[blockIdx.y];
    using EV = EnvT<ENV, DIM>;
    using TL = Tile<ENV, DIM, kEngTile>;
    constexpr int kTileParents = kEngTile;
    constexpr int TP = kEngTile;
    Ctl* c = E.ctl;
    if (c->done) return;
    Stamp stamp(E, P_EXPAND);
    extern __shared__ __attribute__((aligned(16))) uint8_t smem[];
    uint8_t* lpar = smem;
    uint8_t* ltab = smem + TL::PAR_BYTES;
    uint8_t* lst = smem + TL::LDS_BYTES;
    __shared__ uint32_t l_pid[TP], l_g[TP];
    __shared__ uint32_t l_qn, l_qcc[kThreads], l_qrep[kThreads], l_qres[kThreads];
    __shared__ uint32_t l_ohq;
    static_assert((EV::D + 3) / 4 < 16, "no spare lane per row for the parent's path cost");
    const uint32_t it = (uint32_t)c->iters;
    const IterState S0 = c->S[it & 1];
    const uint32_t want = c->want;
    uint32_t npop = want;
    if (E.sem == DCA_SEM_CPP) {
        const uint32_t fs = c->first_solved;
        if (fs != NIL) npop = fs + 1;
    }
    const uint32_t base = (S0.pool_n + 15u) & ~15u;
    const bool fail = (uint64_t)base + (uint64_t)npop * (uint64_t)EV::A > (uint64_t)E.max_nodes;
    const uint32_t cur_new = c->cur_f;
    if (blockIdx.x == 0 && threadIdx.x == 0) close_pop(E, c, S0, it, want, npop, base, fail);
    if (fail) return;
    const uint32_t r0 = blockIdx.x * kTileParents;
    if (E.sem == DCA_SEM_CPP && r0 + kTileParents > npop) {
        uint32_t r = r0 + threadIdx.x;
        bool back = threadIdx.x < kTileParents && r >= npop && r < want;
        open_append(E, c, cur_new, back, back ? E.pop_key[r] : 0, back ? E.pop_id[r] : 0);
        if (back) atomicAdd(&E.hist[bin_of(E.pop_key[r], c->sel_kmin, c->shift)], 1u);
    }
    if (r0 >= npop) return;
    const uint32_t np = min((uint32_t)kTileParents, npop - r0);
    if (OH != 0 && threadIdx.x == 0) l_ohq = 0;
    {
        constexpr int WPR = (EV::D + 3) / 4;
        static_assert(WPR <= 16, "row wider than 64 bytes");
        const uint32_t w = threadIdx.x & 15;
#pragma unroll
        for (uint32_t r = threadIdx.x >> 4; r < (uint32_t)TP; r += 16) {
        if (r < np && w == WPR) {
            const uint32_t pid = E.pop_id[r0 + r] & ID_MASK;
            l_pid[r] = pid;
            l_g[r] = (uint32_t)E.g[pid];
        }
        if (r < np && w < WPR) {
            const uint8_t* row = E.state + (size_t)(E.pop_id[r0 + r] & ID_MASK) * EV::D;
            uint32_t v = 0;
            if (4 * w + 4 <= EV::D) {
                __builtin_memcpy(&v, row + 4 * w, 4);
            } else {
                for (int b = 0; 4 * w + b < EV::D; b++) v |= (uint32_t)row[4 * w + b] << (8 * b);
            }
#pragma unroll
            for (int b = 0; b < 4; b++)
                if (4 * w + b < EV::D) lpar[r * EV::D + 4 * w + b] = (uint8_t)(v >> (8 * b));
        }
        }
    }
    if constexpr (ENV == DCA_ENV_CUBE3) stage_tables<ENV, DIM>(ltab, lpar, np);
    __syncthreads();
    if constexpr (ENV != DCA_ENV_CUBE3) {
        stage_tables<ENV, DIM>(ltab, lpar, np);
        __syncthreads();
    }
    TL t{lpar, ltab};
    const uint32_t nchild = np * EV::A;
    const uint32_t j0 = r0 * EV::A;

    auto oh_emit = [&]() {
        if constexpr (OH != 0) {
            constexpr uint32_t ROW = EV::D * EV::DEPTH;
            constexpr uint32_t EPC = 16 / OH;
            const uint32_t te = nchild * ROW;
            const uint32_t one16 = E.oh_dtype == DCA_DT_F16 ? 0x3C00u : 0x3F80u;
            uint8_t* goh = E.onehot + (size_t)j0 * ROW * OH;
            const uint32_t nch = (te + EPC - 1) / EPC;
            auto staged_nnet = [&](uint32_t i) -> uint32_t {
                const uint32_t b = lst[i];
                return ENV == DCA_ENV_CUBE3 ? (b * 57u) >> 9 : b;
            };
            for (;;) {
                uint32_t piece = 0;
                if ((threadIdx.x & 63u) == 0) piece = atomicAdd(&l_ohq, 1u);
                piece = (uint32_t)__builtin_amdgcn_readfirstlane((int)piece);
                if (piece * 64u >= nch) break;
                const uint32_t q = piece * 64u + (threadIdx.x & 63u);
                if (q >= nch) continue;
                uint32_t e0 = q * EPC;
                if constexpr (ENV == DCA_ENV_CUBE3 && OH == 4) {
                    if (e0 + EPC <= te) {
                        const uint32_t P0 = (q << 1) / 3u, phase = (q << 1) - 3u * P0;
                        uint32_t w[4];
                        cube3_onehot32_chunk(phase, staged_nnet(P0), phase == 2u ? staged_nnet(P0 + 1u) : 0u, w);
                        store16(goh + (size_t)e0 * OH, w, true);
                        continue;
                    }
                }
                if constexpr (ENV == DCA_ENV_CUBE3 && OH == 2) {
                    if (e0 + EPC <= te) {
                        const uint32_t P0 = (q << 2) / 3u, phase = (q << 2) - 3u * P0;
                        uint32_t w[4];
                        cube3_onehot16_chunk(phase, staged_nnet(P0), staged_nnet(P0 + 1u), one16, w);
                        store16(goh + (size_t)e0 * OH, w, true);
                        continue;
                    }
                }
                uint32_t cch = e0 / ROW, e = e0 - cch * ROW;
                uint32_t pos = e / EV::DEPTH, col = e - pos * EV::DEPTH;
                uint32_t r = cch / EV::A, a = cch - r * EV::A;
                uint32_t nb = staged_nnet(cch * EV::D + pos);
                uint32_t w[4] = {0, 0, 0, 0};
#pragma unroll
                for (uint32_t k = 0; k < EPC; k++) {
                    bool hot = (nb == col) && (e0 + k < te);
                    if constexpr (OH == 4)
                        w[k] = hot ? 0x3F800000u : 0u;
                    else
                        w[k >> 1] |= (hot ? one16 : 0u) << (16 * (k & 1));
                    if (++col == EV::DEPTH) {
                        col = 0;
                        if (++pos == EV::D) {
                            pos = 0;
                            if (++a == EV::A) {
                                a = 0;
                                ++r;
                            }
                        }
                        nb = staged_nnet((r * EV::A + a) * EV::D + pos);
                    }
                }
                uint8_t* dst = goh + (size_t)e0 * OH;
                if (e0 + EPC <= te) {
                    store16(dst, w, true);
                } else {
                    for (uint32_t k = 0; e0 + k < te; k++) {
                        if constexpr (OH == 4)
                            reinterpret_cast<uint32_t*>(dst)[k] = w[k];
                        else
                            reinterpret_cast<uint16_t*>(dst)[k] = (uint16_t)(w[k >> 1] >> (16 * (k & 1)));
                    }
                }
            }
        }
    };

    if (threadIdx.x == 0) l_qn = 0;
    for (uint32_t cc0 = 0; cc0 < nchild; cc0 += kThreads) {
        const uint32_t cc = cc0 + threadIdx.x;
        const bool cvalid = cc < nchild;
        uint64_t h = 0;
        uint64_t roww[(EV::D + 7) / 8];
        if (cvalid) {
        uint32_t r = cc / EV::A, a = cc - r * EV::A;
        uint64_t sum = 0;
        h = hash_init(EV::D);
        uint32_t manh = 0;
        bool ok = true;
#pragma unroll
        for (int k = 0; k < EV::D; k += 8) {
            uint64_t w = 0;
#pragma unroll
            for (int j = 0; j < 8; j++) {
                if (k + j < EV::D) {
                    uint32_t b = t.child_byte(r, a, k + j);
                    uint32_t goal = goal_byte(ENV, EV::D, k + j);
                    ok &= (b == goal);
                    w |= (uint64_t)b << (8 * j);
                    sum += (uint64_t)b * (uint64_t)(7 * (k + j) + 3);
                    if constexpr (ENV == DCA_ENV_NPUZZLE) manh += manhattan_term(DIM, (uint32_t)(k + j), b);
                }
            }
            h = hash_word(h, w);
            roww[k >> 3] = w;
            uint8_t* dst = lst + cc * EV::D + k;
#pragma unroll
            for (int j = 0; j < 8; j += 2) {
                if (k + j + 1 < EV::D && (EV::D % 2) == 0) {
                    *reinterpret_cast<uint16_t*>(dst + j) = (uint16_t)(w >> (8 * j));
                } else {
                    if (k + j < EV::D) dst[j] = (uint8_t)(w >> (8 * j));
                    if (k + j + 1 < EV::D) dst[j + 1] = (uint8_t)(w >> (8 * j + 8));
                }
            }
        }
        h = hash_final(h);
        const uint32_t j = j0 + cc, id = base + j, pid = l_pid[r];
        const uint32_t gp = l_g[r];
        if (a == 0) E.pop_g[r0 + r] = gp;
        E.g[id] = (int32_t)(gp + 1u);
        E.parent[id] = pid;
        E.move[id] = (uint8_t)a;
        E.solved[id] = ok ? 1 : 0;
        if (heur_id >= 0) E.child_h[j] = heur_from(heur_id, sum, h, manh);
        }
        {
            constexpr int NWD = (EV::D + 3) / 4;
            const uint32_t j = j0 + cc, id = base + j;
            const uint64_t tag = h >> 32;
            bool active = cvalid, inserted = false, paused = false;
            uint32_t slot = (uint32_t)h & E.tab_mask, v0 = GINF, rep_id = 0, probes = 0, qi = 0;
            __syncthreads();
            for (;;) {
                if (active && !paused) {
                    for (;;) {
                        const uint4 sl = *reinterpret_cast<const uint4*>(&E.tab[slot]);
                        uint64_t e = ((uint64_t)sl.y << 32) | sl.x;
                        v0 = sl.z;
                        if (e == EMPTY) {
                            const uint64_t old = atomicCAS((unsigned long long*)&E.tab[slot].entry, (unsigned long long)EMPTY,
                                                           (unsigned long long)((tag << 32) | id));
                            if (old == EMPTY) {
                                inserted = true;
                                active = false;
                                break;
                            }
                            e = old;
                        }
                        if ((e >> 32) == tag) {
                            const uint32_t rep = (uint32_t)e;
                            if (rep >= base) {
                                qi = atomicAdd(&l_qn, 1u);
                                l_qcc[qi] = cc;
                                l_qrep[qi] = rep;
                                paused = true;
                                break;
                            }
                            const uint8_t* rrow = E.state + (size_t)rep * EV::D;
                            uint32_t diff = 0;
#pragma unroll
                            for (int k = 0; k < NWD; k++) {
                                uint32_t v = 0;
                                if (4 * k + 4 <= EV::D) {
                                    __builtin_memcpy(&v, rrow + 4 * k, 4);
                                } else {
                                    for (int b = 0; 4 * k + b < EV::D; b++) v |= (uint32_t)rrow[4 * k + b] << (8 * b);
                                }
                                diff |= v ^ (uint32_t)(roww[k >> 1] >> (32 * (k & 1)));
                            }
                            if (diff == 0) {
                                rep_id = rep;
                                active = false;
                                break;
                            }
                        }
                        slot = (slot + 1) & E.tab_mask;
                        if (++probes > E.tab_mask) {
                            c->failed = 1;
                            active = false;
                            break;
                        }
                    }
                }
                __syncthreads();
                const uint32_t nq = l_qn;
                if (nq == 0) break;
                for (uint32_t q0 = 0; q0 < nq; q0 += kThreads / 16) {
                    const uint32_t item = q0 + (threadIdx.x >> 4), w = threadIdx.x & 15u;
                    const bool iv = item < nq;
                    const uint32_t itc = iv ? item : 0u;
                    const uint32_t rrel = l_qrep[itc] - base;
                    const uint32_t rk = rrel / (uint32_t)EV::A, a2 = rrel - rk * (uint32_t)EV::A;
                    const uint32_t ppid = E.pop_id[rk] & ID_MASK;
                    const uint8_t* prow = E.state + (size_t)ppid * EV::D;
                    uint32_t pw = 0;
                    if (w < (uint32_t)NWD) {
                        if (4 * w + 4 <= (uint32_t)EV::D) {
                            __builtin_memcpy(&pw, prow + 4 * w, 4);
                        } else {
                            for (uint32_t b = 0; 4 * w + b < (uint32_t)EV::D; b++) pw |= (uint32_t)prow[4 * w + b] << (8 * b);
                        }
                    }
                    const uint32_t cw = child_word_from_parent<ENV, DIM>(pw, w, a2, ltab);
                    const uint8_t* mrow = lst + l_qcc[itc] * EV::D;
                    uint32_t mv = 0;
                    for (uint32_t b = 0; b < 4 && 4 * w + b < (uint32_t)EV::D; b++) mv |= (uint32_t)mrow[4 * w + b] << (8 * b);
                    uint32_t diff = w < (uint32_t)NWD ? (cw ^ mv) : 0u;
                    for (int o = 8; o > 0; o >>= 1) diff |= (uint32_t)__shfl_xor((int)diff, o);
                    if (iv && w == 0) l_qres[item] = diff == 0 ? 1u : 0u;
                }
                __syncthreads();
                if (paused) {
                    paused = false;
                    if (l_qres[qi]) {
                        rep_id = l_qrep[qi];
                        active = false;
                    } else {
                        slot = (slot + 1) & E.tab_mask;
                        probes++;
                    }
                }
                __syncthreads();
                if (threadIdx.x == 0) l_qn = 0;
                __syncthreads();
            }
            if (cvalid) {
                uint32_t prev = NIL;
                if (!inserted) {
                    const uint32_t old_head = atomicExch(&E.tab[slot].head, id);
                    if (old_head >= base)
                        prev = old_head - base;
                    else if (rep_id >= base)
                        prev = rep_id - base;
                }
                E.child_next[j] = prev;
                E.child_slot[j] = slot;
                E.child_v0[j] = v0;
                E.child_flags[j] = inserted ? F_NEW : 0;
                if (prev != NIL) {
                    E.child_multi[j] = 1;
                    E.child_multi[prev] = 1;
                }
            }
        }
    }

    __syncthreads();
    if (!write_nn) {
        const uint32_t tb = nchild * EV::D;
        uint8_t* gpool = E.state + ((size_t)base + j0) * EV::D;
        const uint32_t nfull = tb >> 4;
        for (uint32_t q = threadIdx.x; q < nfull; q += kThreads)
            reinterpret_cast<uint4*>(gpool)[q] = reinterpret_cast<const uint4*>(lst)[q];
        for (uint32_t bq = (nfull << 4) + threadIdx.x; bq < tb; bq += kThreads) gpool[bq] = lst[bq];
    } else {
        const uint32_t tb = nchild * EV::D;
        uint8_t* gpool = E.state + ((size_t)base + j0) * EV::D;
        uint8_t* gnn = E.nnet_in + (size_t)j0 * EV::D;
        const uint32_t nfull = tb >> 4;
        for (uint32_t q = threadIdx.x; q < nfull; q += kThreads) {
            const uint4 v = reinterpret_cast<const uint4*>(lst)[q];
            reinterpret_cast<uint4*>(gpool)[q] = v;
            if constexpr (ENV == DCA_ENV_CUBE3) {
                auto div9 = [](uint32_t x) {
                    uint32_t lo = (((x & 0x00FF00FFu) * 57u) >> 9) & 0x00070007u;
                    uint32_t hi = ((((x >> 8) & 0x00FF00FFu) * 57u) >> 9) & 0x00070007u;
                    return lo | (hi << 8);
                };
                reinterpret_cast<uint4*>(gnn)[q] = make_uint4(div9(v.x), div9(v.y), div9(v.z), div9(v.w));
            } else {
                reinterpret_cast<uint4*>(gnn)[q] = v;
            }
        }
        for (uint32_t bq = (nfull << 4) + threadIdx.x; bq < tb; bq += kThreads) {
            const uint32_t b = lst[bq];
            gpool[bq] = (uint8_t)b;
            gnn[bq] = (uint8_t)(ENV == DCA_ENV_CUBE3 ? (b * 57u) >> 9 : b);
        }
    }

    oh_emit();
}

struct Dec {
    bool keep, is_min;
    uint32_t first;
};
__device__ __forceinline__ Dec decide_child(const Eng& E, uint32_t base, uint32_t m, uint32_t j, uint32_t slot,
                                            uint32_t v0, uint32_t gj, bool multi) {
    if (!multi) return Dec{gj < v0, true, j};
    bool dominated = false;
    uint32_t gmin = GINF, pmin = NIL, first = j;
    const uint32_t A = (uint32_t)E.A;
    uint32_t steps = 0;
    for (uint32_t k = E.tab[slot].head - base; k < m && steps <= m; k = E.child_next[k], steps++) {
        const uint32_t gk = E.pop_g[k / A] + 1u;
        dominated |= (k < j && gk <= gj);
        if (gk < gmin || (gk == gmin && k < pmin)) {
            gmin = gk;
            pmin = k;
        }
        first = k < first ? k : first;
    }
    return Dec{(gj < v0) && !dominated, j == pmin, first};
}

__device__ __forceinline__ void fix_representative(const Eng& E, uint32_t base, uint32_t slot, uint32_t id) {
    const uint64_t e = E.tab[slot].entry;
    if ((uint32_t)e >= base && (uint32_t)e != id) E.tab[slot].entry = (e & 0xFFFFFFFF00000000ull) | id;
}

__global__ __launch_bounds__(256) void k_decide(const Eng* __restrict__ engs) {
    const Eng& E = engs[blockIdx.y];
    Ctl* c = E.ctl;
    if (c->done) return;
    Stamp stamp(E, P_DECIDE);
    const uint32_t j = blockIdx.x * 256 + threadIdx.x;
    const IterState& S1 = st_next(c);
    const uint32_t m = S1.m, base = S1.base;
    if (j >= m) return;
    const uint32_t slot = E.child_slot[j];
    const bool multi = E.child_multi[j] != 0;
    const uint32_t gj = E.pop_g[j / (uint32_t)E.A] + 1u;
    const Dec d = decide_child(E, base, m, j, slot, E.child_v0[j], gj, multi);
    E.child_flags[j] = (E.child_flags[j] & F_NEW) | (d.keep ? F_KEEP : 0) | (d.is_min ? F_MIN : 0);
    if (multi && j == d.first) fix_representative(E, base, slot, base + j);
}

template <int ENV, int DIM, int OH>
__global__ __launch_bounds__(256) void k_pack(const Eng* __restrict__ engs) {
    const Eng& E = engs[blockIdx.y];
    using EV = EnvT<ENV, DIM>;
    Ctl* c = E.ctl;
    if (c->done) {
        if (blockIdx.x == 0 && threadIdx.x == 0) {
            atomicAdd(&E.pk_n[1], 1u);
            if (c->failed) atomicAdd(&E.pk_n[2], 1u);
        }
        return;
    }
    Stamp stamp(E, P_PACK);
    const uint32_t m = st_next(c).m, base = st_next(c).base;
    if (blockIdx.x * 256 >= m) return;
    __shared__ uint32_t sh[6];
    __shared__ uint32_t lsrc[256];
    __shared__ __attribute__((aligned(16))) uint8_t lrow[256 * EV::D];
    const uint32_t j = blockIdx.x * 256 + threadIdx.x;
    const bool keep = j < m && (E.child_flags[j] & F_KEEP);
    const int lane = threadIdx.x & 63, wv = threadIdx.x >> 6;
    const unsigned long long mask = __ballot(keep);
    if (lane == 0) sh[wv] = (uint32_t)__popcll(mask);
    __syncthreads();
    if (threadIdx.x == 0) {
        uint32_t tot = 0;
        for (int w = 0; w < 4; w++) {
            uint32_t t = sh[w];
            sh[w] = tot;
            tot += t;
        }
        sh[4] = tot;
        sh[5] = tot ? atomicAdd(E.pk_n, tot) : 0u;
    }
    __syncthreads();
    const uint32_t total = sh[4], gbase = sh[5];
    const uint32_t lr = sh[wv] + (uint32_t)__popcll(mask & ((1ull << lane) - 1ull));
    if (j < m) E.kept_pos[j] = keep ? gbase + lr : NIL;
    if (keep) lsrc[lr] = j;
    __syncthreads();
    if (total == 0) return;
    if (threadIdx.x < total) E.pk_src[gbase + threadIdx.x] = E.inst * E.M + lsrc[threadIdx.x];
    const uint32_t tb = total * EV::D;
    for (uint32_t q = threadIdx.x; q < tb; q += 256) {
        const uint32_t r = q / EV::D, b = q - r * EV::D;
        const uint32_t v = E.state[(size_t)(base + lsrc[r]) * EV::D + b];
        lrow[q] = (uint8_t)(ENV == DCA_ENV_CUBE3 ? (v * 57u) >> 9 : v);
    }
    __syncthreads();
    uint8_t* gnn = E.pk_nnet + (size_t)gbase * EV::D;
    for (uint32_t q = threadIdx.x; q < tb; q += 256) gnn[q] = lrow[q];
    if constexpr (OH != 0) {
        constexpr uint32_t ROW = EV::D * EV::DEPTH, EPC = 16 / OH;
        const uint32_t cpr = E.pk_stride / EPC;
        const uint32_t one16 = E.pk_dtype == DCA_DT_F16 ? 0x3C00u : 0x3F80u;
        uint4* goh = reinterpret_cast<uint4*>(E.pk_onehot + (size_t)gbase * E.pk_stride * OH);
        const uint32_t nch = total * cpr;
        for (uint32_t q = threadIdx.x; q < nch; q += 256) {
            const uint32_t r = q / cpr, e0 = (q - r * cpr) * EPC;
            uint32_t pos = e0 / EV::DEPTH, col = e0 - pos * EV::DEPTH;
            uint32_t nb = pos < (uint32_t)EV::D ? lrow[r * EV::D + pos] : 0xFFFFu;
            uint32_t w[4] = {0, 0, 0, 0};
#pragma unroll
            for (uint32_t k = 0; k < EPC; k++) {
                const bool hot = (e0 + k < ROW) && nb == col;
                if constexpr (OH == 4)
                    w[k] = hot ? 0x3F800000u : 0u;
                else
                    w[k >> 1] |= (hot ? one16 : 0u) << (16 * (k & 1));
                if (++col == EV::DEPTH) {
                    col = 0;
                    ++pos;
                    nb = pos < (uint32_t)EV::D ? lrow[r * EV::D + pos] : 0xFFFFu;
                }
            }
            goh[q] = make_uint4(w[0], w[1], w[2], w[3]);
        }
    }
}

__device__ __forceinline__ void commit_ticket(const Eng& E, Ctl* c) {
    __syncthreads();
    if (threadIdx.x == 0) {
        uint32_t t = atomicAdd(&c->ticket_a.v, 1u);
        if (t == gridDim.x - 1) {
            c->ticket_a.v = 0;
            c->iters += 1;
            if (c->stop_after || c->failed) {
                c->done = 1;
            } else {
                const uint32_t fb = c->cur_f;
                const uint32_t live = __hip_atomic_load(&c->open_n[fb].v, __ATOMIC_RELAXED, __HIP_MEMORY_SCOPE_AGENT) -
                                      __hip_atomic_load(&c->front_dead.v, __ATOMIC_RELAXED, __HIP_MEMORY_SCOPE_AGENT) - c->front_above;
                c->want = live < (uint32_t)E.B ? live : (uint32_t)E.B;
                c->ret_n.v = 0;
                c->goal_best = ~0ull;
                c->first_solved = NIL;
                c->gbar.v = 0;
                c->grange.kmin = ~0ull;
                c->grange.kmax = 0;
                c->grange.imin = ~0u;
                c->grange.imax = 0;
            }
        }
    }
}

template <bool FUSED>
__global__ __launch_bounds__(1024) void k_commit(const Eng* __restrict__ engs, int packed) {
    const Eng& E = engs[blockIdx.y];
    Ctl* c = E.ctl;
    if (c->done) return;
    Stamp stamp(E, P_COMMIT);
    __shared__ uint32_t sh[3 * 16 + 3];
    __shared__ uint32_t lh[NBIN];
    __shared__ uint64_t red[4][16];
    const IterState& S1 = st_next(c);
    const uint32_t m = S1.m, base = S1.base;
    const uint32_t fb = c->cur_f, bb = c->cur_b;
    const uint64_t T = c->T;
    const uint32_t j = blockIdx.x * 1024 + threadIdx.x;
    if (blockIdx.x * 1024 >= m) {
        commit_ticket(E, c);
        return;
    }
    uint64_t rng_snap;
    {
        const uint32_t sl = threadIdx.x < 4 ? threadIdx.x : 0u;
        const uint32_t sbuf = sl < 2 ? fb : bb;
        const uint64_t* sp = (sl & 1) ? &c->rng[sbuf].kmax : &c->rng[sbuf].kmin;
        asm volatile("global_load_dwordx2 %0, %1, off" : "=v"(rng_snap) : "v"(sp) : "memory");
    }
    for (int k = 0; k < kBinsPerThread; k++) lh[kBinsPerThread * threadIdx.x + k] = 0;
    const uint64_t bin_kmin = c->sel_kmin;
    const uint32_t bin_shift = c->shift;
    __syncthreads();
    const bool live = j < m;
    const uint32_t id = base + j;
    bool keep = false, is_new = false;
    uint32_t gj = 0, my_slot = 0;
    float h_early = 0.f;
    uint8_t solved_early = 0;
    if (live) {
        if (!packed) h_early = E.child_h[j];
        solved_early = E.solved[id];
        const uint8_t fl = E.child_flags[j];
        is_new = (fl & F_NEW) != 0;
        gj = E.pop_g[j / (uint32_t)E.A] + 1u;
        const uint32_t slot = E.child_slot[j];
        my_slot = slot;
        bool is_min;
        uint32_t first = j;
        bool multi = false;
        if constexpr (FUSED) {
            multi = E.child_multi[j] != 0;
            const Dec d = decide_child(E, base, m, j, slot, E.child_v0[j], gj, multi);
            keep = d.keep;
            is_min = d.is_min;
            first = d.first;
        } else {
            keep = (fl & F_KEEP) != 0;
            is_min = (fl & F_MIN) != 0;
        }
        if (keep && is_min) {
            E.tab[slot].g = gj;
            if (E.sem == DCA_SEM_CPP) {
                uint32_t rep = (uint32_t)E.tab[slot].entry;
                if (FUSED && rep >= base) rep = base + first;
                if (rep != id) {
                    E.g[rep] = (int32_t)gj;
                    E.parent[rep] = E.parent[id];
                    E.move[rep] = E.move[id];
                }
            }
        }
        if (FUSED && multi && j == first) fix_representative(E, base, slot, id);
        E.child_multi[j] = 0;
    }
    uint64_t key = 0;
    uint32_t pid_flag = 0;
    if (keep) {
        const float hraw = packed ? E.pk_h[E.kept_pos[j]] : h_early;
        const float hv = fmaxf(hraw, 0.0f);
        const bool ns = solved_early == 0;
        pid_flag = ns ? 0u : ID_SOLVED;
        double cost;
        if (E.sem == DCA_SEM_PY) {
            cost = __dadd_rn(__dmul_rn(E.w, (double)gj), __dmul_rn((double)hv, ns ? 1.0 : 0.0));
        } else {
            cost = (double)__fadd_rn(__fmul_rn(hv, ns ? 1.0f : 0.0f), __fmul_rn(E.wf, (float)gj));
        }
        key = key_of_cost(cost);
    }
    const bool tof = keep && key <= T, tob = keep && key > T;
    const uint32_t hbin = c->hbin;
    if (tof) {
        const uint32_t f = bin_of(key, bin_kmin, bin_shift);
        if (f < hbin) atomicAdd(&lh[f], 1u);
    }
    const uint32_t cnt[3] = {tof ? 1u : 0u, tob ? 1u : 0u, is_new ? 1u : 0u};
    uint32_t* const ctr[3] = {&c->open_n[fb].v, &c->open_n[bb].v, &c->closed_n.v};
    uint32_t pos[3];
    block_reserveK<1024, 3>(cnt, ctr, pos, sh);
    static_assert(kBinsPerThread % 2 == 0, "bins are flushed in aligned pairs");
    if (kBinsPerThread * threadIdx.x < hbin) {
#pragma unroll
        for (int k = 0; k < kBinsPerThread; k += 2) {
            const uint32_t v0 = lh[kBinsPerThread * threadIdx.x + k], v1 = lh[kBinsPerThread * threadIdx.x + k + 1];
            if (v0 | v1)
                atomicAdd(reinterpret_cast<unsigned long long*>(&E.hist[kBinsPerThread * threadIdx.x + k]),
                          (unsigned long long)v0 | ((unsigned long long)v1 << 32));
        }
    }
    if (is_new && pos[2] < E.max_nodes) E.closed_slots[pos[2]] = my_slot;
    if (tof) {
        if (pos[0] < E.front_cap) {
            E.open_key[fb][pos[0]] = key;
            E.open_id[fb][pos[0]] = id | pid_flag;
        } else {
            c->failed = 1;
        }
    } else if (tob) {
        if (pos[1] < E.max_nodes) {
            E.open_key[bb][pos[1]] = key;
            E.open_id[bb][pos[1]] = id | pid_flag;
        } else {
            c->failed = 1;
        }
    }
    {
        uint64_t fmn = tof ? key : ~0ull, fmx = tof ? key : 0ull, bmn = tob ? key : ~0ull, bmx = tob ? key : 0ull;
        for (int o = 32; o > 0; o >>= 1) {
            const uint64_t a = __shfl_xor(fmn, o), z = __shfl_xor(fmx, o), x = __shfl_xor(bmn, o), y = __shfl_xor(bmx, o);
            fmn = a < fmn ? a : fmn;
            fmx = z > fmx ? z : fmx;
            bmn = x < bmn ? x : bmn;
            bmx = y > bmx ? y : bmx;
        }
        const int lane = threadIdx.x & 63, wv = threadIdx.x >> 6;
        if (lane == 0) {
            red[0][wv] = fmn;
            red[1][wv] = fmx;
            red[2][wv] = bmn;
            red[3][wv] = bmx;
        }
        __syncthreads();
        if (threadIdx.x < 4) {
            const int q = threadIdx.x;
            uint64_t v = red[q][0];
            for (int w = 1; w < 16; w++) v = (q & 1) ? (red[q][w] > v ? red[q][w] : v) : (red[q][w] < v ? red[q][w] : v);
            const uint32_t buf = q < 2 ? fb : bb;
            asm volatile("" : "+v"(rng_snap));
            if (q & 1) {
                if (v > rng_snap) atomicMax((unsigned long long*)&c->rng[buf].kmax, (unsigned long long)v);
            } else {
                if (v < rng_snap) atomicMin((unsigned long long*)&c->rng[buf].kmin, (unsigned long long)v);
            }
        }
    }
    commit_ticket(E, c);
}

__global__ void k_set_weights(Eng* __restrict__ engs, const double* __restrict__ w, int n) {
    const int i = blockIdx.x * blockDim.x + threadIdx.x;
    if (i < n) {
        const double v = w[i] >= 0.0 ? w[i] : 0.0;
        engs[i].w = v;
        engs[i].wf = (float)v;
    }
}

__global__ __launch_bounds__(256) void k_gather_popped(const Eng* __restrict__ engs, uint8_t* __restrict__ out_states,
                                                       uint8_t* __restrict__ out_flags) {
    const Eng& E = engs[blockIdx.y];
    const Ctl* c = E.ctl;
    const uint32_t B = (uint32_t)E.B, D = (uint32_t)E.D;
    const uint32_t npop = c->done ? 0u : st_next(c).npop;
    for (uint32_t r = blockIdx.x; r < B; r += gridDim.x) {
        uint8_t* dst = out_states + ((size_t)blockIdx.y * B + r) * D;
        if (r < npop) {
            const uint32_t idf = E.pop_id[r];
            const uint8_t* src = E.state + (size_t)(idf & ID_MASK) * D;
            for (uint32_t b = threadIdx.x; b < D; b += blockDim.x) dst[b] = src[b];
            if (threadIdx.x == 0) out_flags[(size_t)blockIdx.y * B + r] = (idf & ID_SOLVED) ? 2 : 1;
        } else {
            for (uint32_t b = threadIdx.x; b < D; b += blockDim.x) dst[b] = 0;
            if (threadIdx.x == 0) out_flags[(size_t)blockIdx.y * B + r] = 0;
        }
    }
}

__global__ void k_solution(Eng E, int32_t* out , double* path_cost) {
    if (threadIdx.x != 0 || blockIdx.x != 0) return;
    Ctl* c = E.ctl;
    out[0] = -1;
    *path_cost = 0.0;
    uint32_t n;
    if (E.sem == DCA_SEM_PY) {
        if (c->goal_best == ~0ull && !(c->done && c->stop_after)) return;
        n = c->goal_id;
        *path_cost = (double)E.g[n];
    } else {
        if (!st_cur(c).has_best) return;
        n = st_cur(c).best_id;
    }
    int len = 0;
    while ((E.sem == DCA_SEM_PY ? E.parent[n] != NIL : E.g[n] > 0) && len < kMaxMoves - 1) {
        out[1 + len++] = E.move[n];
        n = E.parent[n];
    }
    for (int i = 0; i < len / 2; i++) {
        int32_t tmp = out[1 + i];
        out[1 + i] = out[len - i];
        out[len - i] = tmp;
    }
    out[0] = len;
    if (E.sem == DCA_SEM_CPP) *path_cost = (double)len;
}


}


using namespace dca;

constexpr int kMaxInstances = 64;
constexpr int kGraphSlots = 48, kGraphChunk = 64;

struct dca_engine {
    int K;
    Eng E[kMaxInstances];
    Eng* d_engs;
    uint8_t* nnet_all;
    uint8_t* onehot_all;
    float* h_all;
    Ctl* h_ctl;
    int32_t* h_moves;
    double* d_cost;
    double* h_cost;
    uint8_t* h_stage;
    uint32_t* pk_n;
    uint32_t* h_pk_n;
    uint8_t *pk_nnet, *pk_onehot;
    uint32_t* pk_src;
    float* pk_h;
    int64_t pk_rows;
    int phase;
    bool w_dev;
    uint8_t tab_cleared[kMaxInstances];
    unsigned collect_blocks;
    long collect_resident;
    struct GraphSlot {
        unsigned long long mask;
        int n;
        hipGraph_t graph;
        hipGraphExec_t exec;
    } gslot[kGraphSlots];
    int gslot_next;
    int graph_heur;
    long host_iter;
    unsigned long long* d_prof;
    unsigned long long* h_prof;
    void* allocs[kMaxInstances * 48 + 16];
    int nalloc;
};

namespace {

template <typename T>
int dev_alloc(dca_engine* e, T** p, size_t count) {
    if (e->nalloc >= (int)(sizeof(e->allocs) / sizeof(e->allocs[0]))) {
        set_error("allocation table full");
        return DCA_E_NOMEM;
    }
    void* q = nullptr;
    hipError_t err = hipMalloc(&q, count * sizeof(T) + 256);
    if (err != hipSuccess) {
        set_error("hipMalloc(%zu bytes) failed: %s", count * sizeof(T), hipGetErrorString(err));
        return DCA_E_NOMEM;
    }
    e->allocs[e->nalloc++] = q;
    *p = reinterpret_cast<T*>(q);
    return 0;
}

constexpr int kScanGrid = kScanBlocks;
constexpr int kRampIters = 8;
static inline bool rebase_due(long host_iter) { return host_iter < kRampIters || host_iter % kRefillPeriod == 0; }
static int h_giant_path_off;

inline dim3 gxy(unsigned x, const dca_engine* e) { return dim3(x, (unsigned)e->K); }

template <int ENV, int DIM>
int launch_expand_env(const dca_engine* e, int heur_id, bool want_oh, bool want_nn, hipStream_t s) {
    using TL = Tile<ENV, DIM, kEngTile>;
    const Eng& E = e->E[0];
    dim3 g = gxy((E.B + kEngTile - 1) / kEngTile, e), b(kThreads);
    const size_t lds = TL::LDS_BYTES + ((kEngTile * EnvT<ENV, DIM>::A * EnvT<ENV, DIM>::D + 15) / 16) * 16 + 64;
    const int wnn = want_nn && heur_id < 0 ? 1 : 0;
    if (E.onehot == nullptr || !want_oh)
        hipLaunchKernelGGL((k_expand<ENV, DIM, 0>), g, b, lds, s, e->d_engs, heur_id, wnn);
    else if (E.oh_dtype == DCA_DT_F32)
        hipLaunchKernelGGL((k_expand<ENV, DIM, 4>), g, b, lds, s, e->d_engs, heur_id, wnn);
    else
        hipLaunchKernelGGL((k_expand<ENV, DIM, 2>), g, b, lds, s, e->d_engs, heur_id, wnn);
    return launch_check("k_expand");
}

int launch_expand(const dca_engine* e, int heur_id, bool want_oh, bool want_nn, hipStream_t s) {
    const Eng& E = e->E[0];
    if (E.env == DCA_ENV_CUBE3) return launch_expand_env<DCA_ENV_CUBE3, 0>(e, heur_id, want_oh, want_nn, s);
    if (E.env == DCA_ENV_LIGHTSOUT) return launch_expand_env<DCA_ENV_LIGHTSOUT, 7>(e, heur_id, want_oh, want_nn, s);
    switch (E.dim) {
        case 4: return launch_expand_env<DCA_ENV_NPUZZLE, 4>(e, heur_id, want_oh, want_nn, s);
        case 5: return launch_expand_env<DCA_ENV_NPUZZLE, 5>(e, heur_id, want_oh, want_nn, s);
        case 6: return launch_expand_env<DCA_ENV_NPUZZLE, 6>(e, heur_id, want_oh, want_nn, s);
        case 7: return launch_expand_env<DCA_ENV_NPUZZLE, 7>(e, heur_id, want_oh, want_nn, s);
    }
    return DCA_E_BADARG;
}

template <int ENV, int DIM>
int launch_pack_env(const dca_engine* e, hipStream_t s) {
    const Eng& E = e->E[0];
    const dim3 g = gxy((E.M + 255) / 256, e), b(256);
    if (E.pk_onehot == nullptr)
        hipLaunchKernelGGL((k_pack<ENV, DIM, 0>), g, b, 0, s, e->d_engs);
    else if (E.pk_dtype == DCA_DT_F32)
        hipLaunchKernelGGL((k_pack<ENV, DIM, 4>), g, b, 0, s, e->d_engs);
    else
        hipLaunchKernelGGL((k_pack<ENV, DIM, 2>), g, b, 0, s, e->d_engs);
    return launch_check("k_pack");
}

int launch_pack(const dca_engine* e, hipStream_t s) {
    const Eng& E = e->E[0];
    if (E.env == DCA_ENV_CUBE3) return launch_pack_env<DCA_ENV_CUBE3, 0>(e, s);
    if (E.env == DCA_ENV_LIGHTSOUT) return launch_pack_env<DCA_ENV_LIGHTSOUT, 7>(e, s);
    switch (E.dim) {
        case 4: return launch_pack_env<DCA_ENV_NPUZZLE, 4>(e, s);
        case 5: return launch_pack_env<DCA_ENV_NPUZZLE, 5>(e, s);
        case 6: return launch_pack_env<DCA_ENV_NPUZZLE, 6>(e, s);
        case 7: return launch_pack_env<DCA_ENV_NPUZZLE, 7>(e, s);
    }
    return DCA_E_BADARG;
}

constexpr size_t kRankLdsBytes = (size_t)kLdsEnt * 12;

int enqueue_first_half(dca_engine* e, int heur_id, bool with_refill, hipStream_t s, bool want_oh = true, bool want_nn = true) {
    const Eng* d = e->d_engs;
    if (with_refill) {
        hipLaunchKernelGGL(k_refill_hist, gxy(kScanGrid, e), dim3(256), 0, s, d);
        hipLaunchKernelGGL(k_refill_scan, gxy(1, e), dim3(1024), 0, s, d);
        hipLaunchKernelGGL(k_refill_move, gxy(kScanGrid, e), dim3(256), 0, s, d);
        hipLaunchKernelGGL(k_front_rebase, gxy(kCollectBlocks, e), dim3(256), 0, s, d);
        hipLaunchKernelGGL(k_sel_scan, gxy(1, e), dim3(1024), 0, s, d, 1);
        hipLaunchKernelGGL(k_sel_collect<false>, gxy(e->collect_blocks, e), dim3(256), sizeof(CollectLds), s, d);
    } else {
        hipLaunchKernelGGL(k_sel_collect<true>, gxy(e->collect_blocks, e), dim3(256), sizeof(CollectLds), s, d);
    }
    hipLaunchKernelGGL(k_rank, gxy(kRankBlocks, e), dim3(RT), kRankLdsBytes, s, d);
    if (int rc = launch_check("select kernels")) return rc;
    return launch_expand(e, heur_id, want_oh, want_nn, s);
}

int enqueue_commit(dca_engine* e, bool packed, hipStream_t s) {
    const Eng& E = e->E[0];
    const dim3 g = gxy((E.M + 1023) / 1024, e);
    if (packed)
        hipLaunchKernelGGL(k_commit<false>, g, dim3(1024), 0, s, e->d_engs, 1);
    else
        hipLaunchKernelGGL(k_commit<true>, g, dim3(1024), 0, s, e->d_engs, 0);
    return launch_check("k_commit");
}

void drop_graph_slot(dca_engine::GraphSlot& g) {
    if (g.exec) (void)hipGraphExecDestroy(g.exec);
    if (g.graph) (void)hipGraphDestroy(g.graph);
    g.exec = nullptr;
    g.graph = nullptr;
    g.n = 0;
    g.mask = 0;
}

void drop_graphs(dca_engine* e) {
    for (int g = 0; g < kGraphSlots; g++) drop_graph_slot(e->gslot[g]);
    e->gslot_next = 0;
}

int pull_dev_weights(dca_engine* e) {
    if (!e->w_dev) return 0;
    DCA_HIP(hipDeviceSynchronize());
    std::vector<Eng> tmp((size_t)e->K);
    DCA_HIP(hipMemcpy(tmp.data(), e->d_engs, sizeof(Eng) * (size_t)e->K, hipMemcpyDeviceToHost));
    for (int i = 0; i < e->K; i++) {
        e->E[i].w = tmp[(size_t)i].w;
        e->E[i].wf = tmp[(size_t)i].wf;
    }
    e->w_dev = false;
    return 0;
}

int upload_engs(dca_engine* e) {
    if (int rc = pull_dev_weights(e)) return rc;
    DCA_HIP(hipMemcpy(e->d_engs, e->E, sizeof(Eng) * (size_t)e->K, hipMemcpyHostToDevice));
    return 0;
}

int fetch_ctl(dca_engine* e, int inst, hipStream_t s) {
    DCA_HIP(hipMemcpyAsync(e->h_ctl, e->E[inst].ctl, sizeof(Ctl), hipMemcpyDeviceToHost, s));
    DCA_HIP(hipStreamSynchronize(s));
    return 0;
}

#define DCA_INST(e, i)                                                        \
    do {                                                                      \
        DCA_ARG((e) != nullptr);                                              \
        if ((i) < 0 || (i) >= (e)->K) {                                       \
            set_error("instance %d out of range (engine has %d)", (i), (e)->K); \
            return DCA_E_BADARG;                                              \
        }                                                                     \
    } while (0)

}

extern "C" {

int dca_engine_create_multi(dca_engine** out, int env, int dim, double weight, int batch_size, int64_t max_nodes,
                            int semantics, int onehot_dtype, int num_instances) {
    DCA_ARG(out != nullptr);
    *out = nullptr;
    DCA_ARG(env == DCA_ENV_CUBE3 || (env == DCA_ENV_NPUZZLE && dim >= 4 && dim <= 7) || (env == DCA_ENV_LIGHTSOUT && dim == 7));
    DCA_ARG(batch_size >= 1 && batch_size <= (1 << 22));
    DCA_ARG(semantics == DCA_SEM_PY || semantics == DCA_SEM_CPP);
    DCA_ARG(onehot_dtype >= -1 && onehot_dtype <= DCA_DT_BF16);
    DCA_ARG(weight >= 0.0);
    DCA_ARG(num_instances >= 1 && num_instances <= kMaxInstances);
    const int D = env == DCA_ENV_CUBE3 ? 54 : dim * dim;
    const int A = env == DCA_ENV_CUBE3 ? 12 : env == DCA_ENV_LIGHTSOUT ? D : 4;
    const int depth = env == DCA_ENV_NPUZZLE ? D : 6;
    const int64_t Mll = (int64_t)batch_size * A;
    DCA_ARG(max_nodes >= Mll + 16 && max_nodes <= 0x7FFFFF00ll);
    uint64_t cap = 1024;
    while (cap < 2ull * (uint64_t)max_nodes) cap <<= 1;
    if (cap > 0x80000000ull) {
        set_error("max_nodes too large for a 32-bit slot index");
        return DCA_E_BADARG;
    }
    dca_engine* e = new (std::nothrow) dca_engine();
    if (!e) return DCA_E_NOMEM;
    memset(e, 0, sizeof(*e));
    e->K = num_instances;
    {
        int dev = 0, cus = 256;
        (void)hipGetDevice(&dev);
        if (hipDeviceGetAttribute(&cus, hipDeviceAttributeMultiprocessorCount, dev) != hipSuccess || cus <= 0) cus = 256;
        e->collect_blocks = (unsigned)(2 * cus < kCollectBlocks ? 2 * cus : kCollectBlocks);
        if (num_instances > 1) {
            const unsigned per = e->collect_blocks / (unsigned)num_instances;
            e->collect_blocks = per < 8u ? 8u : per;
        }
    }
    const size_t K = (size_t)num_instances;
    const size_t N = (size_t)max_nodes, M = (size_t)Mll, Bz = (size_t)batch_size + 64;
    int rc = 0;
    rc = dev_alloc(e, &e->nnet_all, K * M * D + 64);
    if (!rc) rc = dev_alloc(e, &e->h_all, K * M);
    if (!rc && onehot_dtype >= 0) rc = dev_alloc(e, &e->onehot_all, K * M * D * depth * (onehot_dtype == DCA_DT_F32 ? 4 : 2) + 64);
    if (!rc) rc = dev_alloc(e, &e->d_engs, K);
    if (!rc) rc = dev_alloc(e, &e->d_cost, 1);
    for (size_t i = 0; i < K && !rc; i++) {
        Eng& E = e->E[i];
        E.env = env;
        E.dim = dim;
        E.D = D;
        E.A = A;
        E.B = batch_size;
        E.sem = semantics;
        E.oh_dtype = onehot_dtype;
        E.depth = depth;
        E.w = weight;
        E.wf = (float)weight;
        E.max_nodes = (uint32_t)max_nodes;
        E.M = (uint32_t)Mll;
        E.coop = (num_instances == 1 && h_giant_path_off == 0) ? 1 : 0;
        E.f_keep = (uint32_t)(32 * batch_size > 65536 ? 32 * batch_size : 65536);
        E.f_max = 3 * E.f_keep;
        E.tab_cap = (uint32_t)cap;
        E.tab_mask = (uint32_t)(cap - 1);
        E.nnet_in = e->nnet_all + i * M * D;
        E.child_h = e->h_all + i * M;
        E.onehot = e->onehot_all ? e->onehot_all + i * M * D * depth * (onehot_dtype == DCA_DT_F32 ? 4 : 2) : nullptr;
#define ALLOC(field, count) \
    if (!rc) rc = dev_alloc(e, &E.field, (count))
        ALLOC(state, N * D + 64);
        ALLOC(g, N);
        ALLOC(parent, N);
        ALLOC(move, N);
        ALLOC(solved, N);
        ALLOC(tab, (size_t)cap);
        ALLOC(closed_slots, N);
        ALLOC(coop_off, 16);
        E.front_cap = (uint32_t)(N + (size_t)(2 * kRefillPeriod) * Bz);
        for (int b = 0; b < 4; b++) {
            ALLOC(open_key[b], b < 2 ? (size_t)E.front_cap : N);
            ALLOC(open_id[b], b < 2 ? (size_t)E.front_cap : N);
        }
        ALLOC(hist, NBIN);
        ALLOC(rhist, NBIN);
        ALLOC(pre, kSegs + 16);
        ALLOC(fill, kSegs + 8);
        ALLOC(subhist, (size_t)kMaxLevels * kSub);
        ALLOC(part, 4 * 1024);
        ALLOC(tmp_key, N);
        ALLOC(tmp_id, N);
        ALLOC(tmp_f, N);
        ALLOC(tmp_idx, N);
        ALLOC(ord_key, N);
        ALLOC(ord_id, N);
        ALLOC(big_list, 8 * kSegs);
        ALLOC(pop_key, Bz);
        ALLOC(pop_id, Bz);
        ALLOC(pop_g, Bz);
        ALLOC(child_slot, M);
        ALLOC(child_next, M);
        ALLOC(child_flags, M);
        ALLOC(child_v0, M);
        ALLOC(child_multi, M);
        ALLOC(root_nnet, 64);
        ALLOC(d_moves, kMaxMoves);
        ALLOC(ctl, 1);
#undef ALLOC
        if (!rc) {
            (void)hipMemset(E.hist, 0, NBIN * sizeof(uint32_t));
            (void)hipMemset(E.rhist, 0, NBIN * sizeof(uint32_t));
            (void)hipMemset(E.fill, 0, (kSegs + 8) * sizeof(uint32_t));
            (void)hipMemset(E.subhist, 0, (size_t)kMaxLevels * kSub * sizeof(uint32_t));
            (void)hipMemset(E.child_multi, 0, M);
            (void)hipMemset(E.coop_off, 0, 16 * sizeof(uint32_t));
            (void)hipMemset(E.ctl, 0, sizeof(Ctl));
        }
    }
    if (!rc) {
        hipError_t err = hipHostMalloc((void**)&e->h_ctl, sizeof(Ctl) + kMaxMoves * sizeof(int32_t) + 512);
        if (err != hipSuccess) rc = hip_fail(err, "hipHostMalloc");
    }
    if (!rc) {
        hipError_t err = hipFuncSetAttribute(reinterpret_cast<const void*>(k_sel_collect<false>),
                                             hipFuncAttributeMaxDynamicSharedMemorySize, (int)sizeof(CollectLds));
        if (err == hipSuccess)
            err = hipFuncSetAttribute(reinterpret_cast<const void*>(k_sel_collect<true>),
                                      hipFuncAttributeMaxDynamicSharedMemorySize, (int)sizeof(CollectLds));
        if (err != hipSuccess) rc = hip_fail(err, "hipFuncSetAttribute(k_sel_collect)");
        if (err == hipSuccess) {
            int per_cu_a = 0, per_cu_b = 0, dev = 0, cus = 0;
            (void)hipGetDevice(&dev);
            (void)hipDeviceGetAttribute(&cus, hipDeviceAttributeMultiprocessorCount, dev);
            hipError_t oa = hipOccupancyMaxActiveBlocksPerMultiprocessor(&per_cu_a, k_sel_collect<false>, 256, sizeof(CollectLds));
            hipError_t ob = hipOccupancyMaxActiveBlocksPerMultiprocessor(&per_cu_b, k_sel_collect<true>, 256, sizeof(CollectLds));
            const int per_cu = per_cu_a < per_cu_b ? per_cu_a : per_cu_b;
            e->collect_resident = (oa == hipSuccess && ob == hipSuccess && cus > 0) ? (long)per_cu * cus : -1;
            if (e->collect_resident >= 0 && e->collect_resident < (long)e->collect_blocks) {
                for (size_t i = 0; i < K; i++) e->E[i].coop = 0;
            }
            (void)hipGetLastError();
        }
    }
    if (!rc) {
        hipError_t err = hipFuncSetAttribute(reinterpret_cast<const void*>(k_rank),
                                             hipFuncAttributeMaxDynamicSharedMemorySize, (int)kRankLdsBytes);
        if (err != hipSuccess) rc = hip_fail(err, "hipFuncSetAttribute(k_rank)");
    }
    if (rc) {
        dca_engine_destroy(e);
        return rc;
    }
    e->h_moves = reinterpret_cast<int32_t*>(reinterpret_cast<uint8_t*>(e->h_ctl) + ((sizeof(Ctl) + 15) & ~15ul));
    e->h_cost = reinterpret_cast<double*>(e->h_moves + kMaxMoves);
    e->h_stage = reinterpret_cast<uint8_t*>(e->h_cost + 1);
    (void)hipMemset(e->nnet_all, 0, K * M * D);
    if (int urc = upload_engs(e)) {
        dca_engine_destroy(e);
        return urc;
    }
    for (size_t i = 0; i < K; i++) {
        int32_t one = 1;
        (void)hipMemcpy(&e->E[i].ctl->done, &one, sizeof(one), hipMemcpyHostToDevice);
    }
    *out = e;
    return 0;
}

int dca_engine_create(dca_engine** out, int env, int dim, double weight, int batch_size, int64_t max_nodes,
                      int semantics, int onehot_dtype) {
    return dca_engine_create_multi(out, env, dim, weight, batch_size, max_nodes, semantics, onehot_dtype, 1);
}

int dca_engine_num_instances(dca_engine* e) { return e ? e->K : 0; }

void dca_engine_destroy(dca_engine* e) {
    if (!e) return;
    drop_graphs(e);
    for (int i = 0; i < e->nalloc; i++) (void)hipFree(e->allocs[i]);
    if (e->h_ctl) (void)hipHostFree(e->h_ctl);
    if (e->h_pk_n) (void)hipHostFree(e->h_pk_n);
    if (e->h_prof) (void)hipHostFree(e->h_prof);
    delete e;
}

int dca_engine_reset_instance(dca_engine* e, int inst, const uint8_t* root, void* stream) {
    DCA_INST(e, inst);
    DCA_ARG(root != nullptr);
    hipStream_t s = (hipStream_t)stream;
    Eng& E = e->E[inst];
    for (int i = 0; i < E.D; i++) DCA_ARG(root[i] < (E.env == DCA_ENV_CUBE3 ? 54 : E.env == DCA_ENV_LIGHTSOUT ? 2 : E.D));
    DCA_HIP(hipStreamSynchronize(s));
    memcpy(e->h_stage, root, (size_t)E.D);
    DCA_HIP(hipMemcpyAsync(E.state, e->h_stage, (size_t)E.D, hipMemcpyHostToDevice, s));
    {
        if (e->phase != 0)
            for (int i = 0; i < e->K; i++) e->tab_cleared[i] = 0;
        const int force = e->tab_cleared[inst] == 0 ? 1 : 0;
        hipLaunchKernelGGL(k_init_table, dim3(4096), dim3(256), 0, s, E.tab, E.tab_cap, E.ctl, force);
        hipLaunchKernelGGL(k_clear_table_list, dim3(1024), dim3(256), 0, s, E.tab, E.tab_cap, E.closed_slots, E.ctl, force);
        e->tab_cleared[inst] = 1;
    }
    hipLaunchKernelGGL(k_reset, dim3(1), dim3(64), 0, s, E);
    DCA_HIP(hipMemsetAsync(E.child_multi, 0, (size_t)E.M, s));
    e->phase = 0;
    e->host_iter = 0;
    return launch_check("k_reset");
}
int dca_engine_reset(dca_engine* e, const uint8_t* root, void* stream) {
    return dca_engine_reset_instance(e, 0, root, stream);
}

int dca_engine_root_commit_instance(dca_engine* e, int inst, const float* h_root, void* stream) {
    DCA_INST(e, inst);
    if (e->E[inst].sem != DCA_SEM_PY) return 0;
    DCA_ARG(h_root != nullptr);
    hipLaunchKernelGGL(k_root_commit, dim3(1), dim3(64), 0, (hipStream_t)stream, e->E[inst], h_root);
    return launch_check("k_root_commit");
}
int dca_engine_root_commit(dca_engine* e, const float* h_root, void* stream) {
    return dca_engine_root_commit_instance(e, 0, h_root, stream);
}

int dca_engine_root_nnet_in_instance(dca_engine* e, int inst, const uint8_t** nnet_in) {
    DCA_INST(e, inst);
    DCA_ARG(nnet_in != nullptr);
    *nnet_in = e->E[inst].root_nnet;
    return 0;
}
int dca_engine_root_nnet_in(dca_engine* e, const uint8_t** nnet_in) {
    return dca_engine_root_nnet_in_instance(e, 0, nnet_in);
}

int dca_engine_pop_expand(dca_engine* e, const uint8_t** nnet_in, const void** onehot, int64_t* m_capacity,
                          void* stream) {
    DCA_ARG(e != nullptr);
    if (e->phase != 0) {
        set_error("dca_engine_pop_expand called twice without dca_engine_commit");
        return DCA_E_STATE;
    }
    if (int rc = enqueue_first_half(e, -1, rebase_due(e->host_iter++), (hipStream_t)stream)) return rc;
    if (nnet_in) *nnet_in = e->nnet_all;
    if (onehot) *onehot = e->onehot_all;
    if (m_capacity) *m_capacity = (int64_t)e->E[0].M * e->K;
    e->phase = 1;
    return 0;
}

int dca_engine_commit(dca_engine* e, const float* h, void* stream) {
    DCA_ARG(e != nullptr && h != nullptr);
    if (e->phase != 1) {
        set_error("dca_engine_commit without a preceding dca_engine_pop_expand");
        return DCA_E_STATE;
    }
    hipStream_t s = (hipStream_t)stream;
    DCA_HIP(hipMemcpyAsync(e->h_all, h, (size_t)e->E[0].M * e->K * sizeof(float), hipMemcpyDeviceToDevice, s));
    e->phase = 0;
    return enqueue_commit(e, false, s);
}


int dca_engine_enable_packed(dca_engine* e, int onehot_dtype, int64_t onehot_row_stride) {
    DCA_ARG(e != nullptr && onehot_dtype >= -1 && onehot_dtype <= DCA_DT_BF16);
    if (e->pk_n != nullptr) {
        set_error("dca_engine_enable_packed called twice");
        return DCA_E_STATE;
    }
    const Eng& E0 = e->E[0];
    const int64_t row = (int64_t)E0.D * E0.depth;
    const int esz = onehot_dtype == DCA_DT_F32 ? 4 : 2;
    if (onehot_dtype >= 0) DCA_ARG(onehot_row_stride >= row && (onehot_row_stride * esz) % 16 == 0 && onehot_row_stride < (1 << 20));
    const size_t rows = (((size_t)E0.M * e->K + 1023) / 1024) * 1024;
    if (int rc = dev_alloc(e, &e->pk_n, 64)) return rc;
    if (int rc = dev_alloc(e, &e->pk_src, rows)) return rc;
    if (int rc = dev_alloc(e, &e->pk_nnet, rows * E0.D)) return rc;
    if (int rc = dev_alloc(e, &e->pk_h, rows)) return rc;
    DCA_HIP(hipMemset(e->pk_nnet, 0, rows * E0.D));
    if (onehot_dtype >= 0) {
        if (int rc = dev_alloc(e, &e->pk_onehot, rows * (size_t)onehot_row_stride * esz)) return rc;
        DCA_HIP(hipMemset(e->pk_onehot, 0, rows * (size_t)onehot_row_stride * esz));
    }
    DCA_HIP(hipHostMalloc((void**)&e->h_pk_n, 64, hipHostMallocDefault));
    for (int i = 0; i < e->K; i++) {
        Eng& E = e->E[i];
        if (int rc = dev_alloc(e, &E.kept_pos, (size_t)E.M)) return rc;
        E.pk_n = e->pk_n;
        E.pk_src = e->pk_src;
        E.pk_nnet = e->pk_nnet;
        E.pk_onehot = e->pk_onehot;
        E.pk_h = e->pk_h;
        E.pk_stride = (uint32_t)(onehot_dtype >= 0 ? onehot_row_stride : 0);
        E.pk_dtype = onehot_dtype;
        E.inst = (uint32_t)i;
    }
    return upload_engs(e);
}

int dca_engine_pop_expand_packed(dca_engine* e, const uint8_t** nnet_in, const void** onehot, const uint32_t** src,
                                 int64_t* rows, void* stream) {
    DCA_ARG(e != nullptr && rows != nullptr);
    if (e->pk_n == nullptr) {
        set_error("dca_engine_pop_expand_packed before dca_engine_enable_packed");
        return DCA_E_STATE;
    }
    if (e->phase != 0) {
        set_error("dca_engine_pop_expand_packed called twice without dca_engine_commit_packed");
        return DCA_E_STATE;
    }
    hipStream_t s = (hipStream_t)stream;
    DCA_HIP(hipMemsetAsync(e->pk_n, 0, 4 * sizeof(uint32_t), s));
    if (int rc = enqueue_first_half(e, -1, rebase_due(e->host_iter++), s, false, false)) return rc;
    hipLaunchKernelGGL(k_decide, gxy((e->E[0].M + 255) / 256, e), dim3(256), 0, s, e->d_engs);
    if (int rc = launch_check("k_decide")) return rc;
    if (int rc = launch_pack(e, s)) return rc;
    DCA_HIP(hipMemcpyAsync(e->h_pk_n, e->pk_n, 4 * sizeof(uint32_t), hipMemcpyDeviceToHost, s));
    DCA_HIP(hipStreamSynchronize(s));
    e->pk_rows = (int64_t)*e->h_pk_n;
    *rows = e->pk_rows;
    if (nnet_in) *nnet_in = e->pk_nnet;
    if (onehot) *onehot = e->pk_onehot;
    if (src) *src = e->pk_src;
    e->phase = 2;
    return 0;
}

int dca_engine_packed_state(dca_engine* e, int* instances_done, int* instances_failed) {
    DCA_ARG(e != nullptr);
    if (e->h_pk_n == nullptr) {
        set_error("dca_engine_packed_state before dca_engine_enable_packed");
        return DCA_E_STATE;
    }
    if (instances_done) *instances_done = (int)e->h_pk_n[1];
    if (instances_failed) *instances_failed = (int)e->h_pk_n[2];
    return 0;
}

int dca_engine_commit_packed(dca_engine* e, const float* h, void* stream) {
    DCA_ARG(e != nullptr);
    if (e->phase != 2) {
        set_error("dca_engine_commit_packed without a preceding dca_engine_pop_expand_packed");
        return DCA_E_STATE;
    }
    DCA_ARG(h != nullptr || e->pk_rows == 0);
    hipStream_t s = (hipStream_t)stream;
    if (e->pk_rows > 0)
        DCA_HIP(hipMemcpyAsync(e->pk_h, h, (size_t)e->pk_rows * sizeof(float), hipMemcpyDeviceToDevice, s));
    e->phase = 0;
    return enqueue_commit(e, true, s);
}

static void plan_chunk(long host_iter, int remaining, int* n_out, unsigned long long* mask_out) {
    int n = remaining;
    if (host_iter < kRampIters) {
        n = n < (int)(kRampIters - host_iter) ? n : (int)(kRampIters - host_iter);
    } else {
        const int to_boundary = (int)(kRefillPeriod - host_iter % kRefillPeriod) % kRefillPeriod;
        if (to_boundary > 0 && n > to_boundary)
            n = to_boundary;
        else if (to_boundary == 0 && n > kRefillPeriod)
            n = (n < kGraphChunk ? n : kGraphChunk) / kRefillPeriod * kRefillPeriod;
    }
    unsigned long long mask = 0;
    for (int it = 0; it < n; it++)
        if (rebase_due(host_iter + it)) mask |= 1ull << it;
    *n_out = n;
    *mask_out = mask;
}

int dca_engine_plan_chunk(int64_t host_iter, int remaining, int* n, uint64_t* rebase_mask) {
    DCA_ARG(host_iter >= 0 && remaining >= 1 && n != nullptr && rebase_mask != nullptr);
    unsigned long long m = 0;
    plan_chunk((long)host_iter, remaining, n, &m);
    *rebase_mask = (uint64_t)m;
    return 0;
}

int dca_engine_run_builtin(dca_engine* e, int heur_id, int iters, int use_graph, void* stream) {
    DCA_ARG(e != nullptr && heur_id >= 0 && heur_id <= DCA_HEUR_MANHATTAN && iters >= 0);
    if (e->phase != 0) {
        set_error("dca_engine_run_builtin between pop_expand and commit");
        return DCA_E_STATE;
    }
    hipStream_t s = (hipStream_t)stream;
    if (!use_graph) {
        for (int i = 0; i < iters; i++) {
            if (int rc = enqueue_first_half(e, heur_id, rebase_due(e->host_iter++), s)) return rc;
            if (int rc = enqueue_commit(e, false, s)) return rc;
        }
        return 0;
    }
    if (e->graph_heur != heur_id) {
        drop_graphs(e);
        e->graph_heur = heur_id;
    }
    for (int i = 0; i < iters;) {
        int n = 0;
        unsigned long long mask = 0;
        plan_chunk(e->host_iter, iters - i, &n, &mask);
        dca_engine::GraphSlot* g = nullptr;
        for (int q = 0; q < kGraphSlots && !g; q++)
            if (e->gslot[q].exec && e->gslot[q].n == n && e->gslot[q].mask == mask) g = &e->gslot[q];
        if (!g) {
            for (int q = 0; q < kGraphSlots && !g; q++)
                if (!e->gslot[q].exec) g = &e->gslot[q];
            if (!g) {
                g = &e->gslot[e->gslot_next];
                e->gslot_next = (e->gslot_next + 1) % kGraphSlots;
                drop_graph_slot(*g);
            }
            hipStream_t cs;
            DCA_HIP(hipStreamCreateWithFlags(&cs, hipStreamNonBlocking));
            hipError_t err = hipStreamBeginCapture(cs, hipStreamCaptureModeThreadLocal);
            int rc = 0;
            if (err == hipSuccess) {
                for (int it = 0; it < n && !rc; it++) {
                    rc = enqueue_first_half(e, heur_id, (mask >> it) & 1ull, cs);
                    if (!rc) rc = enqueue_commit(e, false, cs);
                }
                err = hipStreamEndCapture(cs, &g->graph);
            }
            (void)hipStreamDestroy(cs);
            if (err != hipSuccess) {
                drop_graph_slot(*g);
                return hip_fail(err, "hipStream capture");
            }
            if (rc) {
                drop_graph_slot(*g);
                return rc;
            }
            if (hipError_t ierr = hipGraphInstantiate(&g->exec, g->graph, nullptr, nullptr, 0); ierr != hipSuccess) {
                drop_graph_slot(*g);
                return hip_fail(ierr, "hipGraphInstantiate");
            }
            g->n = n;
            g->mask = mask;
        }
        DCA_HIP(hipGraphLaunch(g->exec, s));
        e->host_iter += n;
        i += n;
    }
    return 0;
}

int dca_engine_profile_builtin(dca_engine* e, int heur_id, int iters, int use_graph, float* span_ms, float* gap_ms,
                               void* stream) {
    DCA_ARG(e != nullptr && span_ms != nullptr && heur_id >= 0 && heur_id <= DCA_HEUR_MANHATTAN && iters >= 0);
    if (e->phase != 0) {
        set_error("dca_engine_profile_builtin between pop_expand and commit");
        return DCA_E_STATE;
    }
    hipStream_t s = (hipStream_t)stream;
    constexpr size_t kWords = (size_t)P_COUNT * kProfSlots * 2;
    if (e->d_prof == nullptr) {
        if (int rc = dev_alloc(e, &e->d_prof, kWords)) return rc;
        DCA_HIP(hipHostMalloc((void**)&e->h_prof, kWords * sizeof(unsigned long long), hipHostMallocDefault));
    }
    int rate_khz = 100000;
    (void)hipDeviceGetAttribute(&rate_khz, hipDeviceAttributeWallClockRate, 0);
    if (rate_khz <= 0) rate_khz = 100000;
    for (int k = 0; k < DCA_PROF_SLOTS; k++) {
        span_ms[k] = 0.f;
        if (gap_ms) gap_ms[k] = 0.f;
    }
    DCA_HIP(hipStreamSynchronize(s));
    for (int i = 0; i < e->K; i++) e->E[i].prof = e->d_prof;
    if (int rc = upload_engs(e)) return rc;
    int rc = 0;
    for (int it = 0; it < iters && !rc; it++) {
        for (size_t w = 0; w < kWords; w += 2) {
            e->h_prof[w] = ~0ull;
            e->h_prof[w + 1] = 0ull;
        }
        if (hipMemcpyAsync(e->d_prof, e->h_prof, kWords * sizeof(unsigned long long), hipMemcpyHostToDevice, s) != hipSuccess)
            rc = hip_fail(hipGetLastError(), "hipMemcpyAsync(prof)");
        if (!rc) rc = dca_engine_run_builtin(e, heur_id, 1, use_graph, stream);
        if (!rc && hipMemcpyAsync(e->h_prof, e->d_prof, kWords * sizeof(unsigned long long), hipMemcpyDeviceToHost, s) != hipSuccess)
            rc = hip_fail(hipGetLastError(), "hipMemcpyAsync(prof)");
        if (!rc && hipStreamSynchronize(s) != hipSuccess) rc = hip_fail(hipGetLastError(), "hipStreamSynchronize");
        unsigned long long prev_end = 0;
        for (int k = 0; k < P_COUNT && !rc; k++) {
            unsigned long long t0 = ~0ull, t1 = 0;
            for (int b = 0; b < kProfSlots; b++) {
                const unsigned long long a = e->h_prof[((size_t)k * kProfSlots + b) * 2], z = e->h_prof[((size_t)k * kProfSlots + b) * 2 + 1];
                if (a != ~0ull && a < t0) t0 = a;
                if (z > t1) t1 = z;
            }
            if (t0 == ~0ull || t1 < t0) continue;
            span_ms[k] += (float)((double)(t1 - t0) / (double)rate_khz);
            if (gap_ms && prev_end != 0 && t0 > prev_end) gap_ms[k] += (float)((double)(t0 - prev_end) / (double)rate_khz);
            prev_end = t1;
        }
    }
    for (int i = 0; i < e->K; i++) e->E[i].prof = nullptr;
    if (int urc = upload_engs(e)) return urc;
    return rc;
}

int dca_debug_tune(int knob, int value) {
    if (knob != 2 && knob != 5 && knob != 10) {
        set_error("dca_debug_tune: knob %d does not exist (the hooks are 2, 5 and 10)", knob);
        return DCA_E_BADARG;
    }
    if (knob == 5) {
        h_giant_path_off = value;
        return 0;
    }
    if (knob == 2)
        DCA_HIP(hipMemcpyToSymbol(HIP_SYMBOL(g_back_squeeze_mark), &value, sizeof(int), 0, hipMemcpyHostToDevice));
    else
        DCA_HIP(hipMemcpyToSymbol(HIP_SYMBOL(g_first_barrier_gives_up), &value, sizeof(int), 0, hipMemcpyHostToDevice));
    return 0;
}

int dca_engine_set_weight_instance(dca_engine* e, int inst, double weight) {
    DCA_INST(e, inst);
    DCA_ARG(weight >= 0.0);
    if (e->phase != 0) {
        set_error("dca_engine_set_weight_instance between pop_expand and commit");
        return DCA_E_STATE;
    }
    if (int rc = pull_dev_weights(e)) return rc;
    e->E[inst].w = weight;
    e->E[inst].wf = (float)weight;
    DCA_HIP(hipDeviceSynchronize());
    return upload_engs(e);
}

int dca_engine_set_weights(dca_engine* e, const double* weights, int n) {
    DCA_ARG(e != nullptr && weights != nullptr && n >= 1 && n <= e->K);
    if (e->phase != 0) {
        set_error("dca_engine_set_weights between pop_expand and commit");
        return DCA_E_STATE;
    }
    for (int i = 0; i < n; i++) DCA_ARG(weights[i] >= 0.0);
    if (int rc = pull_dev_weights(e)) return rc;
    for (int i = 0; i < n; i++) {
        e->E[i].w = weights[i];
        e->E[i].wf = (float)weights[i];
    }
    DCA_HIP(hipDeviceSynchronize());
    return upload_engs(e);
}

int dca_engine_park_instance(dca_engine* e, int inst, void* stream) {
    DCA_INST(e, inst);
    if (e->phase != 0) {
        set_error("dca_engine_park_instance between pop_expand and commit");
        return DCA_E_STATE;
    }
    const int32_t one = 1;
    DCA_HIP(hipStreamSynchronize((hipStream_t)stream));
    DCA_HIP(hipMemcpy(&e->E[inst].ctl->done, &one, sizeof(one), hipMemcpyHostToDevice));
    return 0;
}

int dca_engine_reset_many(dca_engine* e, const uint8_t* roots_dev, int n, void* stream) {
    DCA_ARG(e != nullptr && roots_dev != nullptr && n >= 0 && n <= e->K);
    hipStream_t s = (hipStream_t)stream;
    if (e->phase != 0)
        for (int i = 0; i < e->K; i++) e->tab_cleared[i] = 0;
    for (int i = 0; i < e->K; i++) {
        Eng& E = e->E[i];
        if (i >= n) {
            DCA_HIP(hipMemsetD32Async((hipDeviceptr_t)&E.ctl->done, 1, 1, s));
            continue;
        }
        DCA_HIP(hipMemcpyAsync(E.state, roots_dev + (size_t)i * (size_t)E.D, (size_t)E.D, hipMemcpyDeviceToDevice, s));
        const int force = e->tab_cleared[i] == 0 ? 1 : 0;
        const unsigned g_all = (unsigned)std::min<uint64_t>(4096, ((uint64_t)E.tab_cap + 255) / 256);
        const unsigned g_list = (unsigned)std::min<uint64_t>(1024, ((uint64_t)E.tab_cap / 8 + 255) / 256);
        hipLaunchKernelGGL(k_init_table, dim3(g_all), dim3(256), 0, s, E.tab, E.tab_cap, E.ctl, force);
        hipLaunchKernelGGL(k_clear_table_list, dim3(g_list ? g_list : 1), dim3(256), 0, s, E.tab, E.tab_cap, E.closed_slots, E.ctl, force);
        e->tab_cleared[i] = 1;
        hipLaunchKernelGGL(k_reset, dim3(1), dim3(64), 0, s, E);
        DCA_HIP(hipMemsetAsync(E.child_multi, 0, (size_t)E.M, s));
    }
    e->phase = 0;
    e->host_iter = 0;
    return launch_check("k_reset (many)");
}

int dca_engine_root_commit_many(dca_engine* e, const float* h_roots_dev, int n, void* stream) {
    DCA_ARG(e != nullptr && n >= 0 && n <= e->K);
    if (e->E[0].sem != DCA_SEM_PY) return 0;
    DCA_ARG(h_roots_dev != nullptr || n == 0);
    for (int i = 0; i < n; i++) hipLaunchKernelGGL(k_root_commit, dim3(1), dim3(64), 0, (hipStream_t)stream, e->E[i], h_roots_dev + i);
    return launch_check("k_root_commit (many)");
}

int dca_engine_set_weights_dev(dca_engine* e, const double* weights_dev, int n, void* stream) {
    DCA_ARG(e != nullptr && weights_dev != nullptr && n >= 1 && n <= e->K);
    if (e->phase != 0) {
        set_error("dca_engine_set_weights_dev between pop_expand and commit");
        return DCA_E_STATE;
    }
    hipLaunchKernelGGL(k_set_weights, dim3((unsigned)((n + 63) / 64)), dim3(64), 0, (hipStream_t)stream, e->d_engs, weights_dev, n);
    e->w_dev = true;
    return launch_check("k_set_weights");
}

int dca_engine_last_popped(dca_engine* e, uint8_t* states, uint8_t* flags, void* stream) {
    DCA_ARG(e != nullptr && states != nullptr && flags != nullptr);
    if (e->phase == 0) {
        set_error("dca_engine_last_popped outside an iteration (call it between pop_expand and commit)");
        return DCA_E_STATE;
    }
    const Eng& E = e->E[0];
    const unsigned gx = (unsigned)(E.B < 1024 ? E.B : 1024);
    hipLaunchKernelGGL(k_gather_popped, gxy(gx, e), dim3(64), 0, (hipStream_t)stream, e->d_engs, states, flags);
    return launch_check("k_gather_popped");
}

int dca_engine_info(dca_engine* e, int64_t* out, void* stream) {
    DCA_ARG(e != nullptr && out != nullptr);
    uint32_t off = 0;
    DCA_HIP(hipStreamSynchronize((hipStream_t)stream));
    DCA_HIP(hipMemcpy(&off, e->E[0].coop_off, sizeof(off), hipMemcpyDeviceToHost));
    out[0] = (int64_t)e->collect_blocks;
    out[1] = (int64_t)e->collect_resident;
    out[2] = (int64_t)e->E[0].coop;
    out[3] = (int64_t)e->E[0].tab_cap * (int64_t)sizeof(Slot);
    out[4] = (int64_t)off;
    out[5] = out[6] = out[7] = 0;
    return 0;
}

int dca_engine_set_tiers(dca_engine* e, int64_t front_keep, int64_t front_max) {
    DCA_ARG(e != nullptr && front_keep >= 1 && front_max >= front_keep && front_max < (1ll << 31));
    for (int i = 0; i < e->K; i++) {
        e->E[i].f_keep = (uint32_t)front_keep;
        e->E[i].f_max = (uint32_t)front_max;
    }
    drop_graphs(e);
    return upload_engs(e);
}

int dca_engine_status_instance(dca_engine* e, int inst, dca_status* out, void* stream) {
    DCA_INST(e, inst);
    DCA_ARG(out != nullptr);
    if (int rc = fetch_ctl(e, inst, (hipStream_t)stream)) return rc;
    const Ctl& c = *e->h_ctl;
    const IterState& S = c.S[(c.iters + (e->phase != 0 ? 1 : 0)) & 1];
    out->done = c.done;
    out->failed = c.failed;
    out->iterations = c.iters;
    out->nodes_generated = c.gen;
    out->nodes_expanded = c.expanded;
    out->open_size = (int64_t)c.open_n[c.cur_f].v - (int64_t)c.front_dead.v + (int64_t)c.open_n[c.cur_b].v - (int64_t)c.back_dead.v;
    out->closed_size = c.closed_n.v;
    out->pool_size = S.pool_n;
    out->best_cost = S.has_best ? (double)S.best_cost : __builtin_nan("");
    return 0;
}
int dca_engine_status(dca_engine* e, dca_status* out, void* stream) {
    return dca_engine_status_instance(e, 0, out, stream);
}

int dca_engine_debug(dca_engine* e, double* out, void* stream) {
    DCA_ARG(e != nullptr && out != nullptr);
    if (int rc = fetch_ctl(e, 0, (hipStream_t)stream)) return rc;
    const Ctl& c = *e->h_ctl;
    auto cost = [](uint64_t k) {
        uint64_t b = (k & 0x8000000000000000ull) ? (k & 0x7FFFFFFFFFFFFFFFull) : ~k;
        double d;
        memcpy(&d, &b, 8);
        return d;
    };
    const IterState& S = c.S[(c.iters + (e->phase != 0 ? 1 : 0)) & 1];
    out[0] = (double)c.open_n[c.cur_f].v - (double)c.front_dead.v;
    out[1] = (double)c.open_n[c.cur_b].v - (double)c.back_dead.v;
    out[2] = cost(c.rng[c.cur_f].kmin);
    out[3] = cost(c.rng[c.cur_f].kmax);
    out[4] = cost(c.rng[c.cur_b].kmin);
    out[5] = cost(c.rng[c.cur_b].kmax);
    out[6] = cost(c.T);
    out[7] = c.want;
    out[8] = c.bstar;
    out[9] = c.dbg_nord;
    out[10] = c.dbg_maxbin;
    out[11] = c.dbg_giant_seen;
    out[12] = c.dbg_maxsub;
    out[13] = c.spill_bin;
    out[14] = S.npop;
    out[15] = S.m;
    return 0;
}

int dca_engine_last_children(dca_engine* e, const uint8_t** states, int64_t* m_live, void* stream) {
    DCA_ARG(e != nullptr && states != nullptr && m_live != nullptr);
    if (int rc = fetch_ctl(e, 0, (hipStream_t)stream)) return rc;
    const IterState& S = e->h_ctl->S[(e->h_ctl->iters + (e->phase != 0 ? 1 : 0)) & 1];
    *states = e->E[0].state + (size_t)S.base * e->E[0].D;
    *m_live = S.m;
    return 0;
}

int dca_engine_solution_instance(dca_engine* e, int inst, int32_t* moves, int cap, int* len, double* path_cost,
                                 void* stream) {
    DCA_INST(e, inst);
    DCA_ARG(len != nullptr && cap >= 0 && (cap == 0 || moves != nullptr));
    hipStream_t s = (hipStream_t)stream;
    const Eng& E = e->E[inst];
    hipLaunchKernelGGL(k_solution, dim3(1), dim3(64), 0, s, E, E.d_moves, e->d_cost);
    if (int rc = launch_check("k_solution")) return rc;
    DCA_HIP(hipMemcpyAsync(e->h_moves, E.d_moves, kMaxMoves * sizeof(int32_t), hipMemcpyDeviceToHost, s));
    DCA_HIP(hipMemcpyAsync(e->h_cost, e->d_cost, sizeof(double), hipMemcpyDeviceToHost, s));
    DCA_HIP(hipStreamSynchronize(s));
    int n = e->h_moves[0];
    if (n < 0) {
        set_error("no solution recorded (search not finished)");
        return DCA_E_NOTFOUND;
    }
    *len = n;
    if (path_cost) *path_cost = *e->h_cost;
    for (int i = 0; i < n && i < cap; i++) moves[i] = e->h_moves[1 + i];
    return 0;
}
int dca_engine_solution(dca_engine* e, int32_t* moves, int cap, int* len, double* path_cost, void* stream) {
    return dca_engine_solution_instance(e, 0, moves, cap, len, path_cost, stream);
}

}
```

Before: 94.73 million.

## Type engine device pointers as global address space to avoid flat memory ops

Result: faster. 101.1 million (median of 6 runs) (+6.8%).

```diff
diff --git a/deepcubea_amd/csrc/dca_engine.hip b/deepcubea_amd/csrc/dca_engine.hip
--- a/deepcubea_amd/csrc/dca_engine.hip
+++ b/deepcubea_amd/csrc/dca_engine.hip
@@ -122,60 +122,118 @@
     return cn <= (uint32_t)(512 * 16) ? (cn + 1023u) / 1024u : 1u;
 }
 
-struct Eng {
+#if defined(__HIP_DEVICE_COMPILE__)
+#define DCA_GLOBAL __attribute__((address_space(1)))
+#else
+#define DCA_GLOBAL
+#endif
+template <class T>
+using gp = T DCA_GLOBAL*;
+template <class T>
+using gr = T DCA_GLOBAL&;
+typedef uint32_t __attribute__((aligned(1), may_alias)) unaligned_u32;
+__device__ __forceinline__ uint32_t load_word(gp<const uint8_t> p) { return *(gp<const unaligned_u32>)p; }
+template <class T, bool DEV>
+struct EngPtr {
+    typedef T* type;
+};
+template <class T>
+struct EngPtr<T, true> {
+    typedef gp<T> type;
+};
+template <class T>
+__device__ __forceinline__ T* generic(gp<T> p) {
+    return (T*)p;
+}
+using ::atomicAdd;
+using ::atomicCAS;
+using ::atomicExch;
+using ::atomicMax;
+using ::atomicMin;
+template <class T, class V>
+__device__ __forceinline__ T atomicAdd(gp<T> p, V v) {
+    return ::atomicAdd(generic(p), (T)v);
+}
+template <class T, class V>
+__device__ __forceinline__ T atomicMin(gp<T> p, V v) {
+    return ::atomicMin(generic(p), (T)v);
+}
+template <class T, class V>
+__device__ __forceinline__ T atomicMax(gp<T> p, V v) {
+    return ::atomicMax(generic(p), (T)v);
+}
+template <class T, class V>
+__device__ __forceinline__ T atomicExch(gp<T> p, V v) {
+    return ::atomicExch(generic(p), (T)v);
+}
+template <class T, class U, class V>
+__device__ __forceinline__ T atomicCAS(gp<T> p, U cmp, V v) {
+    return ::atomicCAS(generic(p), (T)cmp, (T)v);
+}
+
+template <bool DEV>
+struct EngT {
+    template <class T>
+    using P = typename EngPtr<T, DEV>::type;
     int env, dim, D, A, B, sem, oh_dtype, depth;
     double w;
     float wf;
     uint32_t max_nodes, M, tab_cap, tab_mask;
     uint32_t front_cap;
-    uint8_t* state;
-    int32_t* g;
-    uint32_t* parent;
-    uint8_t* move;
-    uint8_t* solved;
-    Slot* tab;
-    uint32_t* closed_slots;
-    uint64_t* open_key[4];
-    uint32_t* open_id[4];
+    P<uint8_t> state;
+    P<int32_t> g;
+    P<uint32_t> parent;
+    P<uint8_t> move;
+    P<uint8_t> solved;
+    P<Slot> tab;
+    P<uint32_t> closed_slots;
+    P<uint64_t> open_key[4];
+    P<uint32_t> open_id[4];
     uint32_t f_keep, f_max;
-    uint32_t *hist, *pre, *fill;
-    uint32_t* rhist;
-    uint32_t* subhist;
+    P<uint32_t> hist, pre, fill;
+    P<uint32_t> rhist;
+    P<uint32_t> subhist;
     int coop;
-    uint32_t* coop_off;
-    uint64_t* part;
-    uint64_t* tmp_key;
-    uint32_t* tmp_id;
-    uint16_t* tmp_f;
-    uint32_t* tmp_idx;
-    uint64_t* ord_key;
-    uint32_t* ord_id;
-    uint32_t* big_list;
-    uint64_t* pop_key;
-    uint32_t *pop_id, *pop_g;
-    uint32_t *child_slot, *child_next, *child_v0;
-    uint8_t *child_flags, *child_multi;
-    float* child_h;
-    uint8_t* nnet_in;
-    uint8_t* onehot;
-    uint8_t* root_nnet;
-    int32_t* d_moves;
-    Ctl* ctl;
-    unsigned long long* prof;
-    uint32_t* kept_pos;
-    uint32_t* pk_n;
-    uint32_t* pk_src;
-    uint8_t* pk_nnet;
-    uint8_t* pk_onehot;
-    const float* pk_h;
+    P<uint32_t> coop_off;
+    P<uint64_t> part;
+    P<uint64_t> tmp_key;
+    P<uint32_t> tmp_id;
+    P<uint16_t> tmp_f;
+    P<uint32_t> tmp_idx;
+    P<uint64_t> ord_key;
+    P<uint32_t> ord_id;
+    P<uint32_t> big_list;
+    P<uint64_t> pop_key;
+    P<uint32_t> pop_id, pop_g;
+    P<uint32_t> child_slot, child_next, child_v0;
+    P<uint8_t> child_flags, child_multi;
+    P<float> child_h;
+    P<uint8_t> nnet_in;
+    P<uint8_t> onehot;
+    P<uint8_t> root_nnet;
+    P<int32_t> d_moves;
+    P<Ctl> ctl;
+    P<unsigned long long> prof;
+    P<uint32_t> kept_pos;
+    P<uint32_t> pk_n;
+    P<uint32_t> pk_src;
+    P<uint8_t> pk_nnet;
+    P<uint8_t> pk_onehot;
+    P<const float> pk_h;
     uint32_t pk_stride, inst;
     int pk_dtype;
 };
-
-__device__ __forceinline__ const IterState& st_cur(const Ctl* c) { return c->S[c->iters & 1]; }
-__device__ __forceinline__ const IterState& st_next(const Ctl* c) { return c->S[(c->iters + 1) & 1]; }
-
-__device__ __forceinline__ void fresh_binning(const Ctl* c, uint32_t buf, uint64_t& kmin, uint32_t& shift) {
+typedef EngT<true> Eng;
+typedef EngT<false> EngH;
+static_assert(sizeof(Eng) == sizeof(EngH) && alignof(Eng) == alignof(EngH), "the two views of an instance descriptor share one layout");
+static_assert(offsetof(Eng, state) == offsetof(EngH, state) && offsetof(Eng, ctl) == offsetof(EngH, ctl) &&
+                  offsetof(Eng, pk_dtype) == offsetof(EngH, pk_dtype),
+              "the two views of an instance descriptor share one layout");
+
+__device__ __forceinline__ gr<const IterState> st_cur(gp<const Ctl> c) { return c->S[c->iters & 1]; }
+__device__ __forceinline__ gr<const IterState> st_next(gp<const Ctl> c) { return c->S[(c->iters + 1) & 1]; }
+
+__device__ __forceinline__ void fresh_binning(gp<const Ctl> c, uint32_t buf, uint64_t& kmin, uint32_t& shift) {
     kmin = c->rng[buf].kmin;
     uint64_t kmax = c->rng[buf].kmax;
     const uint64_t T = c->T;
@@ -209,7 +267,11 @@
         atomicMax(E.prof + ((size_t)kid * kProfSlots + (blockIdx.x & (kProfSlots - 1))) * 2 + 1, (unsigned long long)wall_clock64());
 }
 
-__device__ __forceinline__ void open_append(const Eng& E, Ctl* c, uint32_t buf, bool pred, uint64_t key, uint32_t id) {
+__device__ __forceinline__ bool coop_is_off(const Eng& E) {
+    return __hip_atomic_load(E.coop_off, __ATOMIC_RELAXED, __HIP_MEMORY_SCOPE_AGENT) != 0u;
+}
+
+__device__ __forceinline__ void open_append(const Eng& E, gp<Ctl> c, uint32_t buf, bool pred, uint64_t key, uint32_t id) {
     unsigned long long mask = __ballot(pred);
     if (mask == 0) return;
     int lane = threadIdx.x & 63;
@@ -324,7 +386,7 @@
 }
 
 template <int NT, int K>
-__device__ __forceinline__ void block_reserveK(const uint32_t (&cnt)[K], uint32_t* const (&ctr)[K], uint32_t (&pos)[K],
+__device__ __forceinline__ void block_reserveK(const uint32_t (&cnt)[K], const gp<uint32_t> (&ctr)[K], uint32_t (&pos)[K],
                                                uint32_t* sh ) {
     constexpr int NW = NT / 64;
     const int lane = threadIdx.x & 63, wv = threadIdx.x >> 6;
@@ -359,7 +421,7 @@
     __syncthreads();
 }
 
-__device__ __forceinline__ void fold_range(Ctl* c, uint32_t buf, uint64_t kmn, uint64_t kmx) {
+__device__ __forceinline__ void fold_range(gp<Ctl> c, uint32_t buf, uint64_t kmn, uint64_t kmx) {
     for (int o = 32; o > 0; o >>= 1) {
         uint64_t a = __shfl_xor(kmn, o), b = __shfl_xor(kmx, o);
         kmn = a < kmn ? a : kmn;
@@ -371,11 +433,11 @@
     }
 }
 
-__device__ __forceinline__ bool clear_by_list(const Ctl* c, uint32_t cap, int force) {
+__device__ __forceinline__ bool clear_by_list(gp<const Ctl> c, uint32_t cap, int force) {
     return !force && (uint64_t)c->closed_n.v * 8ull < (uint64_t)cap;
 }
 __global__ void k_init_table(Slot* tab, uint32_t cap, const Ctl* c, int force) {
-    if (clear_by_list(c, cap, force)) return;
+    if (clear_by_list((gp<const Ctl>)c, cap, force)) return;
     uint32_t i = blockIdx.x * blockDim.x + threadIdx.x;
     uint32_t stride = gridDim.x * blockDim.x;
     for (; i < cap; i += stride) {
@@ -385,7 +447,7 @@
     }
 }
 __global__ void k_clear_table_list(Slot* tab, uint32_t cap, const uint32_t* __restrict__ slots, const Ctl* c, int force) {
-    if (!clear_by_list(c, cap, force)) return;
+    if (!clear_by_list((gp<const Ctl>)c, cap, force)) return;
     const uint32_t n = c->closed_n.v;
     for (uint32_t i = blockIdx.x * blockDim.x + threadIdx.x; i < n; i += gridDim.x * blockDim.x) {
         const uint32_t sl = slots[i];
@@ -397,7 +459,7 @@
     }
 }
 
-__global__ void k_reset(Eng E) {
+__global__ void k_reset(EngH E) {
     if (threadIdx.x != 0 || blockIdx.x != 0) return;
     Ctl* c = E.ctl;
     memset(c, 0, sizeof(Ctl));
@@ -445,7 +507,7 @@
     }
 }
 
-__global__ void k_root_commit(Eng E, const float* h_root) {
+__global__ void k_root_commit(EngH E, const float* h_root) {
     if (threadIdx.x != 0 || blockIdx.x != 0) return;
     Ctl* c = E.ctl;
     if (E.sem != DCA_SEM_PY || c->open_n[c->cur_f].v != 0) return;
@@ -464,14 +526,14 @@
     const uint32_t floor_ = (uint32_t)(kRefillPeriod + 1) * (uint32_t)E.B;
     return E.f_keep > floor_ ? E.f_keep : floor_;
 }
-__device__ __forceinline__ bool need_refill(const Eng& E, const Ctl* c) {
+__device__ __forceinline__ bool need_refill(const Eng& E, gp<const Ctl> c) {
     return c->open_n[c->cur_b].v != c->back_dead.v &&
            c->open_n[c->cur_f].v - c->front_dead.v - c->front_above < (uint32_t)(kRefillPeriod + 1) * (uint32_t)E.B;
 }
 
 __global__ __launch_bounds__(256) void k_refill_hist(const Eng* __restrict__ engs) {
     const Eng& E = engs[blockIdx.y];
-    Ctl* c = E.ctl;
+    gp<Ctl> c = E.ctl;
     if (c->done || !need_refill(E, c)) return;
     Stamp stamp(E, P_REFILL_HIST);
     __shared__ uint32_t lh[NBIN];
@@ -480,7 +542,7 @@
     const uint32_t b = c->cur_b, n = c->open_n[b].v;
     const uint64_t kmin = c->rng[b].kmin;
     const uint32_t shift = select_shift(kmin, c->rng[b].kmax);
-    const uint64_t* __restrict__ keys = E.open_key[b];
+    gp<const uint64_t> __restrict__ keys = E.open_key[b];
     for (uint32_t i = blockIdx.x * 256 + threadIdx.x; i < n; i += gridDim.x * 256) {
         uint64_t k = keys[i];
         if (k == DEAD) continue;
@@ -560,7 +622,7 @@
 
 __global__ __launch_bounds__(1024) void k_refill_scan(const Eng* __restrict__ engs) {
     const Eng& E = engs[blockIdx.y];
-    Ctl* c = E.ctl;
+    gp<Ctl> c = E.ctl;
     if (c->done) return;
     Stamp stamp(E, P_REFILL_SCAN);
     for (int k = 0; k < kBinsPerThread; k++) E.hist[kBinsPerThread * threadIdx.x + k] = 0;
@@ -616,7 +678,7 @@
 
 __global__ __launch_bounds__(256) void k_refill_move(const Eng* __restrict__ engs) {
     const Eng& E = engs[blockIdx.y];
-    Ctl* c = E.ctl;
+    gp<Ctl> c = E.ctl;
     if (c->done || !c->refill) return;
     Stamp stamp(E, P_REFILL_MOVE);
     __shared__ uint32_t sh[2 * 4 + 2];
@@ -626,8 +688,8 @@
     const uint64_t kmin = c->r_kmin;
     const uint32_t shift = c->r_shift, bstar = c->r_bstar;
     const bool move = c->r_move != 0;
-    uint64_t* __restrict__ keys = E.open_key[sb];
-    const uint32_t* __restrict__ ids = E.open_id[sb];
+    gp<uint64_t> __restrict__ keys = E.open_key[sb];
+    gp<const uint32_t> __restrict__ ids = E.open_id[sb];
     constexpr uint32_t ITEMS = 8, TILE = 256 * ITEMS;
     uint64_t fmn = ~0ull, fmx = 0;
     uint32_t moved = 0;
@@ -678,7 +740,7 @@
 
 __global__ __launch_bounds__(256) void k_front_rebase(const Eng* __restrict__ engs) {
     const Eng& E = engs[blockIdx.y];
-    Ctl* c = E.ctl;
+    gp<Ctl> c = E.ctl;
     if (c->done) return;
     Stamp stamp(E, P_SEL_HIST);
     __shared__ uint32_t lh[NBIN];
@@ -691,8 +753,8 @@
     uint64_t kmin;
     uint32_t shift;
     fresh_binning(c, b, kmin, shift);
-    const uint64_t* __restrict__ keys = E.open_key[b];
-    const uint32_t* __restrict__ ids = E.open_id[b];
+    gp<const uint64_t> __restrict__ keys = E.open_key[b];
+    gp<const uint32_t> __restrict__ ids = E.open_id[b];
     constexpr uint32_t ITEMS = 8, TILE = 256 * ITEMS;
     uint64_t fmn = ~0ull, fmx = 0, bmn = ~0ull, bmx = 0;
     const uint32_t ntiles = (n + TILE - 1) / TILE;
@@ -769,7 +831,7 @@
 
 __global__ __launch_bounds__(1024) void k_sel_scan(const Eng* __restrict__ engs, int rebased) {
     const Eng& E = engs[blockIdx.y];
-    Ctl* c = E.ctl;
+    gp<Ctl> c = E.ctl;
     __shared__ uint32_t pre[NBIN + 1];
     __shared__ uint32_t wsum[16];
     __shared__ uint32_t s_spill, s_bstar, s_maxbin, s_giant, s_nbig, s_sp, s_hbin;
@@ -836,7 +898,7 @@
     for (int i = NBIN + t; i < kSegs; i += 1024) E.fill[i] = 0;
     if (t == 1023) E.pre[NBIN] = pre[NBIN];
     __syncthreads();
-    const bool giant = E.coop && !*E.coop_off && want != 0 && pre[s_bstar + 1] - pre[s_bstar] > kGiantBin;
+    const bool giant = E.coop && !coop_is_off(E) && want != 0 && pre[s_bstar + 1] - pre[s_bstar] > kGiantBin;
     if (giant)
         for (int i = t; i < kMaxLevels * kSub; i += 1024) E.subhist[i] = 0;
     for (int k = 0; k < kBinsPerThread; k++) {
@@ -972,7 +1034,7 @@
 };
 
 enum { BAR_FAIL = 0, BAR_PASS = 1, BAR_BROKEN = 2 };
-__device__ __forceinline__ int collect_grid_barrier(const Eng& E, Ctl* c, CollectLds& L, uint32_t target, bool first) {
+__device__ __forceinline__ int collect_grid_barrier(const Eng& E, gp<Ctl> c, CollectLds& L, uint32_t target, bool first) {
     asm volatile("s_waitcnt vmcnt(0)" ::: "memory");
     __syncthreads();
     if (threadIdx.x == 0) {
@@ -1022,14 +1084,14 @@
     return (int)L.ok;
 }
 
-__device__ __noinline__ int collect_giant(const Eng& E, Ctl* c, CollectLds& L, const SelParams P) {
+__device__ __forceinline__ int collect_giant(const Eng& E, gp<Ctl> c, CollectLds& L, const SelParams P) {
     const uint32_t t = threadIdx.x, lane = t & 63, wv = t >> 6;
     const uint32_t n = P.n;
     const uint64_t bkmin = P.kmin;
     const uint32_t shift = P.shift, bstar = P.bstar, want = P.want;
     const uint32_t pre_b = P.pre_b;
-    uint64_t* __restrict__ keys = E.open_key[P.b];
-    const uint32_t* __restrict__ ids = E.open_id[P.b];
+    gp<uint64_t> __restrict__ keys = E.open_key[P.b];
+    gp<const uint32_t> __restrict__ ids = E.open_id[P.b];
     constexpr uint32_t ITEMS = 8, TILE = 256 * ITEMS;
     const uint32_t ntiles = (n + TILE - 1) / TILE;
     uint32_t phase = 0;
@@ -1119,7 +1181,7 @@
             }
         }
         __syncthreads();
-        uint32_t* gh = E.subhist + (size_t)lvl * kSub;
+        gp<uint32_t> gh = E.subhist + (size_t)lvl * kSub;
         for (uint32_t i = t; i < (uint32_t)kSub; i += 256)
             if (lh[i]) atomicAdd(&gh[i], lh[i]);
         if (collect_grid_barrier(E, c, L, ++phase * gridDim.x, false) != BAR_PASS) return BAR_FAIL;
@@ -1292,7 +1354,7 @@
 template <bool FUSED>
 __global__ __launch_bounds__(256) void k_sel_collect(const Eng* __restrict__ engs) {
     const Eng& E = engs[blockIdx.y];
-    Ctl* c = E.ctl;
+    gp<Ctl> c = E.ctl;
     if (c->done) return;
     Stamp stamp(E, P_SEL_COLLECT);
     extern __shared__ __attribute__((aligned(16))) uint8_t collect_lds[];
@@ -1353,7 +1415,7 @@
         P.bstar = L.bstar;
         P.pre_b = L.pre[P.bstar];
         P.cn_star = L.pre[P.bstar + 1] - P.pre_b;
-        P.giant = E.coop && !*E.coop_off && P.cn_star > kGiantBin;
+        P.giant = E.coop && !coop_is_off(E) && P.cn_star > kGiantBin;
         if (blockIdx.x == 0) {
             for (uint32_t i = t; i <= (uint32_t)NBIN; i += 256) E.pre[i] = L.pre[i];
             if (t == 0) {
@@ -1420,8 +1482,8 @@
     const uint32_t n = P.n;
     const uint64_t kmin = P.kmin;
     const uint32_t shift = P.shift, bstar = P.bstar;
-    uint64_t* __restrict__ keys = E.open_key[P.b];
-    const uint32_t* __restrict__ ids = E.open_id[P.b];
+    gp<uint64_t> __restrict__ keys = E.open_key[P.b];
+    gp<const uint32_t> __restrict__ ids = E.open_id[P.b];
     constexpr uint32_t ITEMS = 8, TILE = 256 * ITEMS;
     const uint32_t ntiles = (n + TILE - 1) / TILE;
     uint64_t* st_key = L.u.n.st_key;
@@ -1534,7 +1596,7 @@
     RankItem stack[kRankStack];
 };
 
-__device__ __forceinline__ void emit_pop(const Eng& E, Ctl* c, uint32_t rank, uint64_t key, uint32_t id) {
+__device__ __forceinline__ void emit_pop(const Eng& E, gp<Ctl> c, uint32_t rank, uint64_t key, uint32_t id) {
     E.pop_key[rank] = key;
     E.pop_id[rank] = id;
     if (id & ID_SOLVED) {
@@ -1544,7 +1606,7 @@
             atomicMin(&c->first_solved, rank);
     }
 }
-__device__ __forceinline__ void emit_ranked(const Eng& E, Ctl* c, uint32_t nf, bool live, uint32_t rank, uint32_t want,
+__device__ __forceinline__ void emit_ranked(const Eng& E, gp<Ctl> c, uint32_t nf, bool live, uint32_t rank, uint32_t want,
                                             uint64_t key, uint32_t id) {
     if (live && rank < want) emit_pop(E, c, rank, key, id);
     const bool back = live && rank >= want;
@@ -1561,7 +1623,7 @@
         E.open_id[nf][slot] = id;
     }
 }
-__device__ __forceinline__ void ret_begin(Ctl* c, RankShared& S, uint32_t nf, uint32_t count) {
+__device__ __forceinline__ void ret_begin(gp<Ctl> c, RankShared& S, uint32_t nf, uint32_t count) {
     __syncthreads();
     if (threadIdx.x == 0) {
         S.ret_base = count ? atomicAdd(&c->ret_n.v, count) : 0u;
@@ -1570,7 +1632,7 @@
     __syncthreads();
 }
 struct RetAcc {};
-__device__ __forceinline__ void ret_put(const Eng& E, Ctl* c, RankShared& S, uint32_t nf, bool pred, uint64_t key,
+__device__ __forceinline__ void ret_put(const Eng& E, gp<Ctl> c, RankShared& S, uint32_t nf, bool pred, uint64_t key,
                                         uint32_t id, RetAcc& acc) {
     const unsigned long long mask = __ballot(pred);
     if (mask == 0) return;
@@ -1585,7 +1647,7 @@
         E.open_id[nf][slot] = id;
     }
 }
-__device__ __forceinline__ void ret_end(Ctl* c, uint32_t nf, RetAcc acc) {}
+__device__ __forceinline__ void ret_end(gp<Ctl> c, uint32_t nf, RetAcc acc) {}
 template <int NJ>
 __device__ __forceinline__ void ret_put_many(const Eng& E, RankShared& S, uint32_t nf, uint32_t n_ord, uint32_t preds,
                                              const uint64_t* key, const uint32_t* id) {
@@ -1616,7 +1678,7 @@
         }
 }
 
-__device__ __forceinline__ void rank_small_entries(const Eng& E, Ctl* c, RankShared& S, uint64_t* LK, uint32_t* LI,
+__device__ __forceinline__ void rank_small_entries(const Eng& E, gp<Ctl> c, RankShared& S, uint64_t* LK, uint32_t* LI,
                                                    uint32_t nf, uint32_t p0, uint32_t n_ord, uint32_t want) {
     const uint32_t t = threadIdx.x;
     const uint32_t plast = (p0 + RT - 1 < n_ord ? p0 + RT - 1 : n_ord - 1);
@@ -1775,7 +1837,7 @@
     }
 }
 
-__device__ __noinline__ void rank_item(const Eng& E, Ctl* c, RankShared& S, uint64_t* LK, uint32_t* LI, uint32_t nf,
+__device__ __forceinline__ void rank_item(const Eng& E, gp<Ctl> c, RankShared& S, uint64_t* LK, uint32_t* LI, uint32_t nf,
                                        uint32_t want, RankItem it) {
     const uint32_t t = threadIdx.x;
     const uint64_t* __restrict__ K = (it.src ? E.ord_key : E.tmp_key) + it.off;
@@ -2038,7 +2100,7 @@
 
 __global__ __launch_bounds__(RT) void k_rank(const Eng* __restrict__ engs) {
     const Eng& E = engs[blockIdx.y];
-    Ctl* c = E.ctl;
+    gp<Ctl> c = E.ctl;
     if (c->done) return;
     Stamp stamp(E, P_RANK);
     __shared__ RankShared S;
@@ -2089,7 +2151,7 @@
     }
 }
 
-__device__ __forceinline__ void close_pop(const Eng& E, Ctl* c, const IterState& S0, uint32_t it, uint32_t want,
+__device__ __forceinline__ void close_pop(const Eng& E, gp<Ctl> c, const IterState& S0, uint32_t it, uint32_t want,
                                           uint32_t npop, uint32_t base, bool fail) {
     IterState N = S0;
     if (E.sem == DCA_SEM_PY) {
@@ -2185,7 +2247,7 @@
     using TL = Tile<ENV, DIM, kEngTile>;
     constexpr int kTileParents = kEngTile;
     constexpr int TP = kEngTile;
-    Ctl* c = E.ctl;
+    gp<Ctl> c = E.ctl;
     if (c->done) return;
     Stamp stamp(E, P_EXPAND);
     extern __shared__ __attribute__((aligned(16))) uint8_t smem[];
@@ -2231,10 +2293,10 @@
             l_g[r] = (uint32_t)E.g[pid];
         }
         if (r < np && w < WPR) {
-            const uint8_t* row = E.state + (size_t)(E.pop_id[r0 + r] & ID_MASK) * EV::D;
+            gp<const uint8_t> row = E.state + (size_t)(E.pop_id[r0 + r] & ID_MASK) * EV::D;
             uint32_t v = 0;
             if (4 * w + 4 <= EV::D) {
-                __builtin_memcpy(&v, row + 4 * w, 4);
+                v = load_word(row + 4 * w);
             } else {
                 for (int b = 0; 4 * w + b < EV::D; b++) v |= (uint32_t)row[4 * w + b] << (8 * b);
             }
@@ -2260,7 +2322,7 @@
             constexpr uint32_t EPC = 16 / OH;
             const uint32_t te = nchild * ROW;
             const uint32_t one16 = E.oh_dtype == DCA_DT_F16 ? 0x3C00u : 0x3F80u;
-            uint8_t* goh = E.onehot + (size_t)j0 * ROW * OH;
+            gp<uint8_t> goh = E.onehot + (size_t)j0 * ROW * OH;
             const uint32_t nch = (te + EPC - 1) / EPC;
             auto staged_nnet = [&](uint32_t i) -> uint32_t {
                 const uint32_t b = lst[i];
@@ -2412,13 +2474,13 @@
                                 paused = true;
                                 break;
                             }
-                            const uint8_t* rrow = E.state + (size_t)rep * EV::D;
+                            gp<const uint8_t> rrow = E.state + (size_t)rep * EV::D;
                             uint32_t diff = 0;
 #pragma unroll
                             for (int k = 0; k < NWD; k++) {
                                 uint32_t v = 0;
                                 if (4 * k + 4 <= EV::D) {
-                                    __builtin_memcpy(&v, rrow + 4 * k, 4);
+                                    v = load_word(rrow + 4 * k);
                                 } else {
                                     for (int b = 0; 4 * k + b < EV::D; b++) v |= (uint32_t)rrow[4 * k + b] << (8 * b);
                                 }
@@ -2448,11 +2510,11 @@
                     const uint32_t rrel = l_qrep[itc] - base;
                     const uint32_t rk = rrel / (uint32_t)EV::A, a2 = rrel - rk * (uint32_t)EV::A;
                     const uint32_t ppid = E.pop_id[rk] & ID_MASK;
-                    const uint8_t* prow = E.state + (size_t)ppid * EV::D;
+                    gp<const uint8_t> prow = E.state + (size_t)ppid * EV::D;
                     uint32_t pw = 0;
                     if (w < (uint32_t)NWD) {
                         if (4 * w + 4 <= (uint32_t)EV::D) {
-                            __builtin_memcpy(&pw, prow + 4 * w, 4);
+                            pw = load_word(prow + 4 * w);
                         } else {
                             for (uint32_t b = 0; 4 * w + b < (uint32_t)EV::D; b++) pw |= (uint32_t)prow[4 * w + b] << (8 * b);
                         }
@@ -2504,15 +2566,16 @@
     __syncthreads();
     if (!write_nn) {
         const uint32_t tb = nchild * EV::D;
-        uint8_t* gpool = E.state + ((size_t)base + j0) * EV::D;
+        gp<uint8_t> gpool = E.state + ((size_t)base + j0) * EV::D;
         const uint32_t nfull = tb >> 4;
         for (uint32_t q = threadIdx.x; q < nfull; q += kThreads)
             reinterpret_cast<uint4*>(gpool)[q] = reinterpret_cast<const uint4*>(lst)[q];
+#pragma unroll 1
         for (uint32_t bq = (nfull << 4) + threadIdx.x; bq < tb; bq += kThreads) gpool[bq] = lst[bq];
     } else {
         const uint32_t tb = nchild * EV::D;
-        uint8_t* gpool = E.state + ((size_t)base + j0) * EV::D;
-        uint8_t* gnn = E.nnet_in + (size_t)j0 * EV::D;
+        gp<uint8_t> gpool = E.state + ((size_t)base + j0) * EV::D;
+        gp<uint8_t> gnn = E.nnet_in + (size_t)j0 * EV::D;
         const uint32_t nfull = tb >> 4;
         for (uint32_t q = threadIdx.x; q < nfull; q += kThreads) {
             const uint4 v = reinterpret_cast<const uint4*>(lst)[q];
@@ -2528,6 +2591,7 @@
                 reinterpret_cast<uint4*>(gnn)[q] = v;
             }
         }
+#pragma unroll 1
         for (uint32_t bq = (nfull << 4) + threadIdx.x; bq < tb; bq += kThreads) {
             const uint32_t b = lst[bq];
             gpool[bq] = (uint8_t)b;
@@ -2568,11 +2632,11 @@
 
 __global__ __launch_bounds__(256) void k_decide(const Eng* __restrict__ engs) {
     const Eng& E = engs[blockIdx.y];
-    Ctl* c = E.ctl;
+    gp<Ctl> c = E.ctl;
     if (c->done) return;
     Stamp stamp(E, P_DECIDE);
     const uint32_t j = blockIdx.x * 256 + threadIdx.x;
-    const IterState& S1 = st_next(c);
+    gr<const IterState> S1 = st_next(c);
     const uint32_t m = S1.m, base = S1.base;
     if (j >= m) return;
     const uint32_t slot = E.child_slot[j];
@@ -2587,7 +2651,7 @@
 __global__ __launch_bounds__(256) void k_pack(const Eng* __restrict__ engs) {
     const Eng& E = engs[blockIdx.y];
     using EV = EnvT<ENV, DIM>;
-    Ctl* c = E.ctl;
+    gp<Ctl> c = E.ctl;
     if (c->done) {
         if (blockIdx.x == 0 && threadIdx.x == 0) {
             atomicAdd(&E.pk_n[1], 1u);
@@ -2632,7 +2696,7 @@
         lrow[q] = (uint8_t)(ENV == DCA_ENV_CUBE3 ? (v * 57u) >> 9 : v);
     }
     __syncthreads();
-    uint8_t* gnn = E.pk_nnet + (size_t)gbase * EV::D;
+    gp<uint8_t> gnn = E.pk_nnet + (size_t)gbase * EV::D;
     for (uint32_t q = threadIdx.x; q < tb; q += 256) gnn[q] = lrow[q];
     if constexpr (OH != 0) {
         constexpr uint32_t ROW = EV::D * EV::DEPTH, EPC = 16 / OH;
@@ -2663,7 +2727,7 @@
     }
 }
 
-__device__ __forceinline__ void commit_ticket(const Eng& E, Ctl* c) {
+__device__ __forceinline__ void commit_ticket(const Eng& E, gp<Ctl> c) {
     __syncthreads();
     if (threadIdx.x == 0) {
         uint32_t t = atomicAdd(&c->ticket_a.v, 1u);
@@ -2693,13 +2757,13 @@
 template <bool FUSED>
 __global__ __launch_bounds__(1024) void k_commit(const Eng* __restrict__ engs, int packed) {
     const Eng& E = engs[blockIdx.y];
-    Ctl* c = E.ctl;
+    gp<Ctl> c = E.ctl;
     if (c->done) return;
     Stamp stamp(E, P_COMMIT);
     __shared__ uint32_t sh[3 * 16 + 3];
     __shared__ uint32_t lh[NBIN];
     __shared__ uint64_t red[4][16];
-    const IterState& S1 = st_next(c);
+    gr<const IterState> S1 = st_next(c);
     const uint32_t m = S1.m, base = S1.base;
     const uint32_t fb = c->cur_f, bb = c->cur_b;
     const uint64_t T = c->T;
@@ -2783,7 +2847,7 @@
         if (f < hbin) atomicAdd(&lh[f], 1u);
     }
     const uint32_t cnt[3] = {tof ? 1u : 0u, tob ? 1u : 0u, is_new ? 1u : 0u};
-    uint32_t* const ctr[3] = {&c->open_n[fb].v, &c->open_n[bb].v, &c->closed_n.v};
+    const gp<uint32_t> ctr[3] = {&c->open_n[fb].v, &c->open_n[bb].v, &c->closed_n.v};
     uint32_t pos[3];
     block_reserveK<1024, 3>(cnt, ctr, pos, sh);
     static_assert(kBinsPerThread % 2 == 0, "bins are flushed in aligned pairs");
@@ -2857,14 +2921,14 @@
 __global__ __launch_bounds__(256) void k_gather_popped(const Eng* __restrict__ engs, uint8_t* __restrict__ out_states,
                                                        uint8_t* __restrict__ out_flags) {
     const Eng& E = engs[blockIdx.y];
-    const Ctl* c = E.ctl;
+    gp<const Ctl> c = E.ctl;
     const uint32_t B = (uint32_t)E.B, D = (uint32_t)E.D;
     const uint32_t npop = c->done ? 0u : st_next(c).npop;
     for (uint32_t r = blockIdx.x; r < B; r += gridDim.x) {
         uint8_t* dst = out_states + ((size_t)blockIdx.y * B + r) * D;
         if (r < npop) {
             const uint32_t idf = E.pop_id[r];
-            const uint8_t* src = E.state + (size_t)(idf & ID_MASK) * D;
+            gp<const uint8_t> src = E.state + (size_t)(idf & ID_MASK) * D;
             for (uint32_t b = threadIdx.x; b < D; b += blockDim.x) dst[b] = src[b];
             if (threadIdx.x == 0) out_flags[(size_t)blockIdx.y * B + r] = (idf & ID_SOLVED) ? 2 : 1;
         } else {
@@ -2874,7 +2938,7 @@
     }
 }
 
-__global__ void k_solution(Eng E, int32_t* out , double* path_cost) {
+__global__ void k_solution(EngH E, int32_t* out , double* path_cost) {
     if (threadIdx.x != 0 || blockIdx.x != 0) return;
     Ctl* c = E.ctl;
     out[0] = -1;
@@ -2885,8 +2949,8 @@
         n = c->goal_id;
         *path_cost = (double)E.g[n];
     } else {
-        if (!st_cur(c).has_best) return;
-        n = st_cur(c).best_id;
+        if (!st_cur((gp<const Ctl>)c).has_best) return;
+        n = st_cur((gp<const Ctl>)c).best_id;
     }
     int len = 0;
     while ((E.sem == DCA_SEM_PY ? E.parent[n] != NIL : E.g[n] > 0) && len < kMaxMoves - 1) {
@@ -2913,7 +2977,7 @@
 
 struct dca_engine {
     int K;
-    Eng E[kMaxInstances];
+    EngH E[kMaxInstances];
     Eng* d_engs;
     uint8_t* nnet_all;
     uint8_t* onehot_all;
@@ -2978,7 +3042,7 @@
 template <int ENV, int DIM>
 int launch_expand_env(const dca_engine* e, int heur_id, bool want_oh, bool want_nn, hipStream_t s) {
     using TL = Tile<ENV, DIM, kEngTile>;
-    const Eng& E = e->E[0];
+    const EngH& E = e->E[0];
     dim3 g = gxy((E.B + kEngTile - 1) / kEngTile, e), b(kThreads);
     const size_t lds = TL::LDS_BYTES + ((kEngTile * EnvT<ENV, DIM>::A * EnvT<ENV, DIM>::D + 15) / 16) * 16 + 64;
     const int wnn = want_nn && heur_id < 0 ? 1 : 0;
@@ -2992,7 +3056,7 @@
 }
 
 int launch_expand(const dca_engine* e, int heur_id, bool want_oh, bool want_nn, hipStream_t s) {
-    const Eng& E = e->E[0];
+    const EngH& E = e->E[0];
     if (E.env == DCA_ENV_CUBE3) return launch_expand_env<DCA_ENV_CUBE3, 0>(e, heur_id, want_oh, want_nn, s);
     if (E.env == DCA_ENV_LIGHTSOUT) return launch_expand_env<DCA_ENV_LIGHTSOUT, 7>(e, heur_id, want_oh, want_nn, s);
     switch (E.dim) {
@@ -3006,7 +3070,7 @@
 
 template <int ENV, int DIM>
 int launch_pack_env(const dca_engine* e, hipStream_t s) {
-    const Eng& E = e->E[0];
+    const EngH& E = e->E[0];
     const dim3 g = gxy((E.M + 255) / 256, e), b(256);
     if (E.pk_onehot == nullptr)
         hipLaunchKernelGGL((k_pack<ENV, DIM, 0>), g, b, 0, s, e->d_engs);
@@ -3018,7 +3082,7 @@
 }
 
 int launch_pack(const dca_engine* e, hipStream_t s) {
-    const Eng& E = e->E[0];
+    const EngH& E = e->E[0];
     if (E.env == DCA_ENV_CUBE3) return launch_pack_env<DCA_ENV_CUBE3, 0>(e, s);
     if (E.env == DCA_ENV_LIGHTSOUT) return launch_pack_env<DCA_ENV_LIGHTSOUT, 7>(e, s);
     switch (E.dim) {
@@ -3050,7 +3114,7 @@
 }
 
 int enqueue_commit(dca_engine* e, bool packed, hipStream_t s) {
-    const Eng& E = e->E[0];
+    const EngH& E = e->E[0];
     const dim3 g = gxy((E.M + 1023) / 1024, e);
     if (packed)
         hipLaunchKernelGGL(k_commit<false>, g, dim3(1024), 0, s, e->d_engs, 1);
@@ -3076,8 +3140,8 @@
 int pull_dev_weights(dca_engine* e) {
     if (!e->w_dev) return 0;
     DCA_HIP(hipDeviceSynchronize());
-    std::vector<Eng> tmp((size_t)e->K);
-    DCA_HIP(hipMemcpy(tmp.data(), e->d_engs, sizeof(Eng) * (size_t)e->K, hipMemcpyDeviceToHost));
+    std::vector<EngH> tmp((size_t)e->K);
+    DCA_HIP(hipMemcpy(tmp.data(), e->d_engs, sizeof(EngH) * (size_t)e->K, hipMemcpyDeviceToHost));
     for (int i = 0; i < e->K; i++) {
         e->E[i].w = tmp[(size_t)i].w;
         e->E[i].wf = tmp[(size_t)i].wf;
@@ -3088,7 +3152,7 @@
 
 int upload_engs(dca_engine* e) {
     if (int rc = pull_dev_weights(e)) return rc;
-    DCA_HIP(hipMemcpy(e->d_engs, e->E, sizeof(Eng) * (size_t)e->K, hipMemcpyHostToDevice));
+    DCA_HIP(hipMemcpy(e->d_engs, e->E, sizeof(EngH) * (size_t)e->K, hipMemcpyHostToDevice));
     return 0;
 }
 
@@ -3155,7 +3219,7 @@
     if (!rc) rc = dev_alloc(e, &e->d_engs, K);
     if (!rc) rc = dev_alloc(e, &e->d_cost, 1);
     for (size_t i = 0; i < K && !rc; i++) {
-        Eng& E = e->E[i];
+        EngH& E = e->E[i];
         E.env = env;
         E.dim = dim;
         E.D = D;
@@ -3297,7 +3361,7 @@
     DCA_INST(e, inst);
     DCA_ARG(root != nullptr);
     hipStream_t s = (hipStream_t)stream;
-    Eng& E = e->E[inst];
+    EngH& E = e->E[inst];
     for (int i = 0; i < E.D; i++) DCA_ARG(root[i] < (E.env == DCA_ENV_CUBE3 ? 54 : E.env == DCA_ENV_LIGHTSOUT ? 2 : E.D));
     DCA_HIP(hipStreamSynchronize(s));
     memcpy(e->h_stage, root, (size_t)E.D);
@@ -3375,7 +3439,7 @@
         set_error("dca_engine_enable_packed called twice");
         return DCA_E_STATE;
     }
-    const Eng& E0 = e->E[0];
+    const EngH& E0 = e->E[0];
     const int64_t row = (int64_t)E0.D * E0.depth;
     const int esz = onehot_dtype == DCA_DT_F32 ? 4 : 2;
     if (onehot_dtype >= 0) DCA_ARG(onehot_row_stride >= row && (onehot_row_stride * esz) % 16 == 0 && onehot_row_stride < (1 << 20));
@@ -3391,7 +3455,7 @@
     }
     DCA_HIP(hipHostMalloc((void**)&e->h_pk_n, 64, hipHostMallocDefault));
     for (int i = 0; i < e->K; i++) {
-        Eng& E = e->E[i];
+        EngH& E = e->E[i];
         if (int rc = dev_alloc(e, &E.kept_pos, (size_t)E.M)) return rc;
         E.pk_n = e->pk_n;
         E.pk_src = e->pk_src;
@@ -3669,7 +3733,7 @@
     if (e->phase != 0)
         for (int i = 0; i < e->K; i++) e->tab_cleared[i] = 0;
     for (int i = 0; i < e->K; i++) {
-        Eng& E = e->E[i];
+        EngH& E = e->E[i];
         if (i >= n) {
             DCA_HIP(hipMemsetD32Async((hipDeviceptr_t)&E.ctl->done, 1, 1, s));
             continue;
@@ -3714,7 +3778,7 @@
         set_error("dca_engine_last_popped outside an iteration (call it between pop_expand and commit)");
         return DCA_E_STATE;
     }
-    const Eng& E = e->E[0];
+    const EngH& E = e->E[0];
     const unsigned gx = (unsigned)(E.B < 1024 ? E.B : 1024);
     hipLaunchKernelGGL(k_gather_popped, gxy(gx, e), dim3(64), 0, (hipStream_t)stream, e->d_engs, states, flags);
     return launch_check("k_gather_popped");
@@ -3809,7 +3873,7 @@
     DCA_INST(e, inst);
     DCA_ARG(len != nullptr && cap >= 0 && (cap == 0 || moves != nullptr));
     hipStream_t s = (hipStream_t)stream;
-    const Eng& E = e->E[inst];
+    const EngH& E = e->E[inst];
     hipLaunchKernelGGL(k_solution, dim3(1), dim3(64), 0, s, E, E.d_moves, e->d_cost);
     if (int rc = launch_check("k_solution")) return rc;
     DCA_HIP(hipMemcpyAsync(e->h_moves, E.d_moves, kMaxMoves * sizeof(int32_t), hipMemcpyDeviceToHost, s));
```
